# dohlee/diffab-pytorch

Measured on AMD Instinct MI355X. Metric: CDR-residue denoise-steps/sec (K=128 patch), higher is better.
Workload: dtype f32 (bf16x6 / fp16x3 split-precision products on the 16-bit matrix cores, fp32 accumulate; fp32-accurate, DESIGN section 4)

## Files before the change

diffab-pytorch_amd/csrc/api.hip:

```cpp
#include <atomic>
#include <cstring>
#include <mutex>
#include <vector>

#include "common.h"
#include "denoiser_internal.h"
#include "mlp_chain_tile.h"

namespace diffab {

static thread_local char g_err[512] = "";

void set_error(const char* fmt, ...) {
  va_list ap;
  va_start(ap, fmt);
  vsnprintf(g_err, sizeof(g_err), fmt, ap);
  va_end(ap);
}

namespace {
struct OrderState {
  std::recursive_mutex mu;
  hipStream_t last = nullptr;
  bool have = false;
// ... 20 lines not shown
  o.have = true;
}
StreamOrder::~StreamOrder() {
  if (dev_ < 0) return;
  OrderState& o = g_order[dev_ & 31];
  --o.depth;
  o.mu.unlock();
}
void set_stream_order(bool on) { g_order_on.store(on); }

struct KernelTimer {
  bool on = false;
  std::vector<hipEvent_t> ev;
  size_t used = 0;
};
static KernelTimer g_timer;

void timer_begin(hipStream_t st) {
  if (!g_timer.on) return;
  if (g_timer.used + 2 > g_timer.ev.size()) {
    for (int i = 0; i < 2; ++i) {
      hipEvent_t e;
      if (hipEventCreate(&e) != hipSuccess) return;
      g_timer.ev.push_back(e);
    }
  }
  (void)hipEventRecord(g_timer.ev[g_timer.used], st);
}
bool kernel_timer_enabled() { return g_timer.on; }
void timer_end(hipStream_t st) {
  if (!g_timer.on || g_timer.used + 2 > g_timer.ev.size()) return;
  (void)hipEventRecord(g_timer.ev[g_timer.used + 1], st);
  g_timer.used += 2;
}

static int check_dims(const diffab_dims* d, const char* who) {
  DIFFAB_REQUIRE(d != nullptr, DIFFAB_ERR_ARG, "%s: dims is null", who);
  DIFFAB_REQUIRE(d->B > 0 && d->K > 0 && d->D > 0 && d->C >= 0 && d->H > 0 && d->DS > 0 && d->PQ > 0 && d->PV > 0 && d->NL >= 0 && d->V > 0,
                 DIFFAB_ERR_ARG, "%s: non-positive dimension (B=%d K=%d D=%d C=%d H=%d DS=%d PQ=%d PV=%d NL=%d V=%d)", who, d->B, d->K, d->D,
                 d->C, d->H, d->DS, d->PQ, d->PV, d->NL, d->V);
  DIFFAB_REQUIRE(static_cast<int64_t>(d->B) * d->K < (1ll << 31), DIFFAB_ERR_UNSUPPORTED, "%s: B*K must be < 2^31", who);
  return DIFFAB_OK;
}

struct StepBuffers {
  float *cat2, *h1, *hA, *hB, *cat3, *t1, *t2, *vbuf, *logits, *ipa, *emb_tab, *beta_tab;
  char* planes;
  float* pair;
  size_t bytes;
};
static size_t mlp_planes_bytes() { return (rowgemm128_b6_scratch_bytes(128) + 255) & ~static_cast<size_t>(255); }

static StepBuffers carve_step(const diffab_dims* d, void* ws, int n_pair = 0) {
  Carver c(ws);
  const size_t rows = static_cast<size_t>(d->B) * d->K;
  StepBuffers b;
  b.cat2 = c.take<float>(rows * 2 * d->D);
  b.h1 = c.take<float>(rows * d->D);
  b.hA = c.take<float>(rows * d->D);
  b.hB = c.take<float>(rows * d->D);
  b.cat3 = c.take<float>(rows * (d->D + 3));
  b.t1 = c.take<float>(rows * d->D);
  b.t2 = c.take<float>(rows * d->D);
  b.vbuf = c.take<float>(rows * 3);
  b.logits = c.take<float>(rows * d->V);
  b.emb_tab = c.take<float>(static_cast<size_t>(25) * d->D);
  b.beta_tab = c.take<float>(static_cast<size_t>(3) * d->B * d->D);
  size_t ipa_floats = ipa_generic_workspace_floats(d);
  if (fast_path_supported(d)) ipa_floats = ipa_floats > ipa_fast_workspace_floats(d) ? ipa_floats : ipa_fast_workspace_floats(d);
  b.ipa = c.take<float>(ipa_floats);
  b.planes = fast_path_supported(d) ? c.take<char>(d->NL * ipa_layer_planes_bytes() + 11 * mlp_planes_bytes()) : nullptr;
  b.pair = pair_planes_supported(d) ? c.take<float>(pair_planes_floats(d, n_pair)) : nullptr;
  b.bytes = c.bytes();
  return b;
}

static bool ipa_layer_weights_ok(const diffab_dims* d, const diffab_ipa_layer_weights* w) {
  return w && w->gamma && w->wq_s && w->wk_s && w->wv_s && (w->w_bias || d->C == 0) && w->wq_p && w->wk_p && w->wv_p && w->w_out && w->b_out;
}

static int ipa_layer_dispatch(const diffab_dims* d, const diffab_ipa_layer_weights* w, const float* x, const float* e, const float* R,
                              const float* t, float* y, float* ws, uint32_t flags, hipStream_t st, float* sp_keep = nullptr,
                              float* d2_keep = nullptr, const void* planes = nullptr, const float* pair_planes = nullptr,
                              bool taped = false,
                              const unsigned char* tile_needed = nullptr, const int* ctx_of_row = nullptr, int n_ctx = 0) {
  DIFFAB_REQUIRE(ipa_layer_weights_ok(d, w), DIFFAB_ERR_ARG, "ipa layer: null weight pointer");
  if (!(flags & DIFFAB_FLAG_FORCE_GENERIC) && fast_path_supported(d))
    return ipa_layer_fast(d, w, x, e, R, t, y, ws, st, sp_keep, d2_keep, planes, pair_planes, (flags & DIFFAB_FLAG_FP32_GEMM) != 0,
                          taped, tile_needed, ctx_of_row, n_ctx);
  return ipa_layer_generic(d, w, x, e, R, t, y, ws, st, ctx_of_row);
}

static int check_denoiser_weights(const diffab_dims* d, const diffab_denoiser_weights* w) {
  DIFFAB_REQUIRE(w && w->seq_emb && w->res_w0 && w->res_b0 && w->res_w2 && w->res_b2 && (d->NL == 0 || w->layers), DIFFAB_ERR_ARG,
                 "denoiser: null weight pointer");
  DIFFAB_REQUIRE(d->C > 0, DIFFAB_ERR_ARG, "denoiser: C must be positive (the Denoiser's IPA layers use the pair bias, :478-492)");
  for (const diffab_mlp3_weights* h : {&w->coord, &w->orient, &w->seq})
    DIFFAB_REQUIRE(h->w0 && h->b0 && h->w2 && h->b2 && h->w4 && h->b4, DIFFAB_ERR_ARG, "denoiser head: null weight pointer");
  for (int l = 0; l < d->NL; ++l)
    DIFFAB_REQUIRE(ipa_layer_weights_ok(d, &w->layers[l]), DIFFAB_ERR_ARG, "denoiser: null weight pointer in IPA layer %d", l);
  return DIFFAB_OK;
}

static bool use_pair_planes(const diffab_dims* d, uint32_t flags, const float* pair_ctx, const StepBuffers& b) {
  const uint32_t other = DIFFAB_FLAG_FORCE_GENERIC | DIFFAB_FLAG_PAIR_F32;
  return (flags & DIFFAB_FLAG_PAIR_PLANES) && !(flags & other) && b.pair != nullptr && pair_planes_supported(d) &&
         (reinterpret_cast<uintptr_t>(pair_ctx) & 15) == 0;
}

static bool module_launch_fills_chip(const diffab_dims* d) {
  if (!ipa_module_persistent_supported(d)) return false;
  int dev = 0, ncu = 256;
  if (hipGetDevice(&dev) == hipSuccess) (void)hipDeviceGetAttribute(&ncu, hipDeviceAttributeMultiprocessorCount, dev);
  const int rounds = (d->B + ncu - 1) / ncu;
  return d->K == 128 && d->B >= ncu && static_cast<double>(d->B) >= 0.85 * rounds * ncu;
}

struct ForwardPlan {
  uint32_t flags;
  bool fold;
  bool b6;
  bool chain;
  bool persistent, fused_mlps;
  const float* pair_planes;
  const int* ctx_of_row;
  int n_ctx;
  const unsigned char* last_layer_tiles;
  float* res_emb;
};

static ForwardPlan plan_forward(const diffab_dims* d, uint32_t flags, const StepBuffers& b, const float* res_ctx, const float* pair_ctx,
                                float* res_emb, bool loop, const int* ctx_of_row = nullptr, int n_ctx = 0, unsigned char* tiles = nullptr) {
  const int rows = d->B * d->K, D = d->D;
  if (loop && !(flags & DIFFAB_FLAG_PAIR_F32)) flags |= DIFFAB_FLAG_PAIR_PLANES;
  ForwardPlan p{};
  p.flags = flags;
  p.fold = !(flags & DIFFAB_FLAG_FORCE_GENERIC) && fast_path_supported(d) && rowgemm128_ok(res_ctx, D, b.h1, D, rows, D);
  p.b6 = p.fold && use_b6_gemm(flags) && rowgemm128_b6_ok(res_ctx, D, b.h1, D, rows, D);
  p.chain = p.b6 && d->V <= 128;
  p.pair_planes = use_pair_planes(d, flags, pair_ctx, b) ? b.pair : nullptr;
  p.ctx_of_row = ctx_of_row;
  p.n_ctx = n_ctx;
  p.last_layer_tiles = (flags & DIFFAB_FLAG_SKIP_UNUSED_ROWS) && p.fold && d->K % 16 == 0 ? tiles : nullptr;
  p.res_emb = res_emb;
  p.persistent = p.b6 && p.pair_planes != nullptr && ipa_module_persistent_supported(d) && p.last_layer_tiles == nullptr &&
                 ((flags & DIFFAB_FLAG_PERSISTENT_MODULE) || (loop && !(flags & DIFFAB_FLAG_MULTI_LAUNCH) && module_launch_fills_chip(d)));
  p.fused_mlps = p.persistent && p.chain && D == 128 && res_emb == nullptr;
  return p;
}

struct StepBias {
  const float* beta;
  const float* sched_beta;
  int t;
  const int* t_dev;
  float* beta_traj;
  int traj_rows;
};

static int prepare_forward(const diffab_dims* d, const diffab_denoiser_weights* w, const ForwardPlan& p, const StepBuffers& b,
                           const float* pair_ctx, const StepBias& bias, hipStream_t st) {
  if (p.fold)
    if (int rc = launch_fold_embed_table(d, w, b.emb_tab, st)) return rc;
  if (p.b6) {
    const int D = d->D;
    for (int l = 0; l < d->NL; ++l)
      if (int rc = ipa_layer_split_weights(&w->layers[l], b.planes + l * ipa_layer_planes_bytes(), st)) return rc;
    char* mlp = b.planes + d->NL * ipa_layer_planes_bytes();
    const diffab_mlp3_weights* hw[3] = {&w->coord, &w->orient, &w->seq};
    if (int rc = launch_wsplit128(w->res_w0, 2 * D, D, mlp, st)) return rc;
    if (int rc = launch_wsplit128(w->res_w2, D, D, mlp + mlp_planes_bytes(), st)) return rc;
    for (int hd = 0; hd < 3; ++hd) {
      if (int rc = launch_wsplit128(hw[hd]->w0, D + 3, D, mlp + (2 + 2 * hd) * mlp_planes_bytes(), st)) return rc;
      if (int rc = launch_wsplit128(hw[hd]->w2, D, D, mlp + (3 + 2 * hd) * mlp_planes_bytes(), st)) return rc;
      const int nout = hd == 2 ? d->V : 3;
      if (int rc = launch_wsplit128(hw[hd]->w4, D, D, mlp + (8 + hd) * mlp_planes_bytes(), st, nout)) return rc;
    }
  }
  if (p.pair_planes)
    if (int rc = launch_pair_split(d, pair_ctx, b.pair, st, p.n_ctx)) return rc;
  if (bias.beta_traj) {
    diffab_dims dt = *d;
    dt.B = bias.traj_rows;
    if (int rc = launch_fold_beta_table(&dt, w, bias.sched_beta, bias.beta_traj, st)) return rc;
  }
  return DIFFAB_OK;
}

static int denoise_step(const diffab_dims* d, const diffab_denoiser_weights* w, const ForwardPlan& p, const StepBias& bias,
                        const int64_t* seq_t, const float* x_t, const float* O_t, const float* res_ctx, const float* pair_ctx, float* out_eps,
                        float* out_O0, float* out_post, float* out_logits, const StepBuffers& b, hipStream_t st) {
  const int rows = d->B * d->K, D = d->D;
  if (p.fold && bias.beta_traj == nullptr)
    if (int rc = launch_fold_beta_table(d, w, bias.beta, b.beta_tab, st, bias.sched_beta, bias.t, bias.t_dev)) return rc;
  const char* mlp = p.b6 ? b.planes + d->NL * ipa_layer_planes_bytes() : nullptr;
  auto dense128 = [&](int slot, const float* X, const float* W, int ldw, const float* bvec, const int64_t* bias_idx, int bias_div, float* Y,
                      bool relu) -> int {
    if (p.b6) return launch_rowgemm128_b6p(X, D, mlp + slot * mlp_planes_bytes(), bvec, bias_idx, bias_div, Y, D, rows, D, relu, st);
    return launch_rowgemm128(X, D, W, ldw, bvec, bias_idx, bias_div, Y, D, rows, D, relu, st);
  };
  float* logits = out_logits ? out_logits : b.logits;
  MlpChainSet emb_set{}, head_set{};
  if (p.chain) {
    const void* pl[3] = {mlp, mlp + mlp_planes_bytes(), nullptr};
    const float* bs[3] = {b.emb_tab, w->res_b2, nullptr};
    float* ys[1] = {b.hA};
    const int nout1[1] = {D};
    if (int rc = make_mlp_chain_set(&emb_set, 1, pl, bs, seq_t, 0, 2, nout1, ys, nout1)) return rc;
    if (!p.fused_mlps)
      if (int rc = launch_mlp_chain_b6(res_ctx, D, pl, bs, seq_t, 0, 2, D, b.hA, D, rows, st)) return rc;
  } else if (p.fold) {
    if (int rc = dense128(0, res_ctx, w->res_w0, 2 * D, b.emb_tab, seq_t, 0, b.h1, true)) return rc;
    if (int rc = dense128(1, b.h1, w->res_w2, D, w->res_b2, nullptr, 0, b.hA, false)) return rc;
  } else {
    if (int rc = launch_embed_concat(res_ctx, w->seq_emb, seq_t, D, rows, b.cat2, st)) return rc;
    if (int rc = launch_linear(b.cat2, 2 * D, w->res_w0, w->res_b0, b.h1, D, rows, D, 2 * D, true, st)) return rc;
    if (int rc = launch_linear(b.h1, D, w->res_w2, w->res_b2, b.hA, D, rows, D, D, false, st)) return rc;
  }
  float *cur = b.hA, *nxt = b.hB;
  const diffab_mlp3_weights* hw[3] = {&w->coord, &w->orient, &w->seq};
  float* outs[3] = {out_eps, b.vbuf, logits};
  const int nout[3] = {3, 3, d->V};
  const void* hpl[9];
  const float* hbs[9];
  const int head_div = bias.beta_traj ? rows : d->K;
  if (p.chain) {
    for (int hd = 0; hd < 3; ++hd) {
      hpl[3 * hd] = mlp + (2 + 2 * hd) * mlp_planes_bytes();
      hpl[3 * hd + 1] = mlp + (3 + 2 * hd) * mlp_planes_bytes();
      hpl[3 * hd + 2] = mlp + (8 + hd) * mlp_planes_bytes();
      hbs[3 * hd] = bias.beta_traj ? bias.beta_traj + (static_cast<size_t>(hd) * bias.traj_rows + bias.t) * D
                                   : b.beta_tab + static_cast<size_t>(hd) * d->B * D;
      hbs[3 * hd + 1] = hw[hd]->b2;
      hbs[3 * hd + 2] = hw[hd]->b4;
    }
    if (int rc = make_mlp_chain_set(&head_set, 3, hpl, hbs, nullptr, head_div, 3, nout, outs, nout)) return rc;
  }
  if (p.persistent) {
    if (int rc = launch_ipa_module_persistent(d, b.hA, b.hB, O_t, x_t, b.ipa, b.planes, p.pair_planes, st, p.fused_mlps ? res_ctx : nullptr,
                                              &emb_set, &head_set, p.ctx_of_row, p.n_ctx))
      return rc;
    cur = (d->NL & 1) ? b.hB : b.hA;
  }
  for (int l = 0; l < d->NL && !p.persistent; ++l) {
    const void* planes = p.b6 ? b.planes + l * ipa_layer_planes_bytes() : nullptr;
    if (int rc = ipa_layer_dispatch(d, &w->layers[l], cur, pair_ctx, O_t, x_t, nxt, b.ipa, p.flags, st, nullptr, nullptr, planes, p.pair_planes,
                                    false, l == d->NL - 1 ? p.last_layer_tiles : nullptr, p.ctx_of_row, p.n_ctx))
      return rc;
    float* tmp = cur; cur = nxt; nxt = tmp;
  }
  if (p.res_emb) DIFFAB_HIP_CHECK(hipMemcpyAsync(p.res_emb, cur, sizeof(float) * rows * D, hipMemcpyDeviceToDevice, st));
  if (p.chain) {
    if (!p.fused_mlps)
      if (int rc = launch_mlp_chains_b6(cur, D, 3, hpl, hbs, nullptr, head_div, 3, nout, outs, nout, rows, st)) return rc;
  } else if (p.fold) {
    for (int hd = 0; hd < 3; ++hd) {
      if (int rc = dense128(2 + 2 * hd, cur, hw[hd]->w0, D + 3, b.beta_tab + static_cast<size_t>(hd) * d->B * D, nullptr, d->K, b.t1, true))
        return rc;
      if (int rc = dense128(3 + 2 * hd, b.t1, hw[hd]->w2, D, hw[hd]->b2, nullptr, 0, b.t2, true)) return rc;
      if (int rc = launch_linear(b.t2, D, hw[hd]->w4, hw[hd]->b4, outs[hd], nout[hd], rows, nout[hd], D, false, st)) return rc;
    }
  } else {
    if (int rc = launch_beta_concat(cur, bias.beta, D, d->K, rows, b.cat3, st)) return rc;
    for (int hd = 0; hd < 3; ++hd) {
      if (int rc = launch_linear(b.cat3, D + 3, hw[hd]->w0, hw[hd]->b0, b.t1, D, rows, D, D + 3, true, st)) return rc;
      if (int rc = launch_linear(b.t1, D, hw[hd]->w2, hw[hd]->b2, b.t2, D, rows, D, D, true, st)) return rc;
      if (int rc = launch_linear(b.t2, D, hw[hd]->w4, hw[hd]->b4, outs[hd], nout[hd], rows, nout[hd], D, false, st)) return rc;
    }
  }
  if (out_O0 == nullptr) return DIFFAB_OK;
  return launch_heads_finish(b.vbuf, O_t, logits, d->V, rows, out_O0, out_post, st);
}

static uint32_t taped_flags(uint32_t flags) { return flags & ~(DIFFAB_FLAG_FORCE_GENERIC | DIFFAB_FLAG_PAIR_PLANES); }

static int denoise_step_taped(const diffab_dims* d, const diffab_denoiser_weights* w, const int64_t* seq_t, const float* x_t,
                              const float* O_t, const float* res_ctx, const float* pair_ctx, const float* beta, float* out_eps,
                              float* out_O0, float* out_post, const TrainTape& tp, uint32_t flags, hipStream_t st) {
  const int rows = d->B * d->K, D = d->D;
  if (int rc = launch_embed_concat(res_ctx, w->seq_emb, seq_t, D, rows, tp.cat2, st)) return rc;
  if (int rc = launch_linear(tp.cat2, 2 * D, w->res_w0, w->res_b0, tp.h1, D, rows, D, 2 * D, true, st)) return rc;
  if (int rc = launch_linear(tp.h1, D, w->res_w2, w->res_b2, tp.x[0], D, rows, D, D, false, st)) return rc;
  const bool b6 = tp.planes && use_b6_gemm(flags) && fast_path_supported(d);
  for (int l = 0; l < d->NL; ++l) {
    if (b6)
      if (int rc = ipa_layer_split_weights(&w->layers[l], tp.planes, st)) return rc;
    if (int rc = ipa_layer_dispatch(d, &w->layers[l], tp.x[l], pair_ctx, O_t, x_t, tp.x[l + 1], tp.ipa_ws[l], flags, st, tp.sp[l], tp.d2[l],
                                    b6 ? tp.planes : nullptr, nullptr, true))
      return rc;
  }
  if (int rc = launch_beta_concat(tp.x[d->NL], beta, D, d->K, rows, tp.cat3, st)) return rc;
  const diffab_mlp3_weights* hw[3] = {&w->coord, &w->orient, &w->seq};
  float* outs[3] = {out_eps, tp.vbuf, tp.logits};
  const int nout[3] = {3, 3, d->V};
  for (int hd = 0; hd < 3; ++hd) {
    if (int rc = launch_linear(tp.cat3, D + 3, hw[hd]->w0, hw[hd]->b0, tp.t1[hd], D, rows, D, D + 3, true, st)) return rc;
    if (int rc = launch_linear(tp.t1[hd], D, hw[hd]->w2, hw[hd]->b2, tp.t2[hd], D, rows, D, D, true, st)) return rc;
    if (int rc = launch_linear(tp.t2[hd], D, hw[hd]->w4, hw[hd]->b4, outs[hd], nout[hd], rows, nout[hd], D, false, st)) return rc;
  }
  return launch_heads_finish(tp.vbuf, O_t, tp.logits, d->V, rows, out_O0, out_post, st);
}

constexpr int kTrajRows = 1025;
struct SampleBuffers {
  float *beta, *eps, *O0, *post;
  int* t_dev;
  unsigned char* tiles;
  float* beta_traj;
  int* ctx_of_row;
  float* res_ctx;
  void* step;
  size_t bytes;
};

static SampleBuffers carve_sample(const diffab_dims* d, void* ws, int n_pair = 0, bool mapped = false) {
  Carver c(ws);
  const size_t rows = static_cast<size_t>(d->B) * d->K;
  SampleBuffers s;
  s.beta = c.take<float>(d->B);
  s.eps = c.take<float>(rows * 3);
  s.O0 = c.take<float>(rows * 9);
  s.post = c.take<float>(rows * d->V);
  s.t_dev = c.take<int>(64);
  s.tiles = c.take<unsigned char>(static_cast<size_t>(d->B) * ((d->K + 15) / 16));
  s.beta_traj = c.take<float>(static_cast<size_t>(3) * kTrajRows * d->D);
  s.ctx_of_row = mapped ? c.take<int>(d->B) : nullptr;
  s.res_ctx = mapped ? c.take<float>(rows * d->D) : nullptr;
  const size_t step_bytes = carve_step(d, nullptr, n_pair).bytes;
  s.step = c.take<char>(step_bytes);
  s.bytes = c.bytes();
  return s;
}

struct ScoreBuffers {
  int* t_list;
  float* beta;
  int* ctx_of_row;
  int64_t* seq_t;
  float *x_t, *O_t, *eps, *eps_hat;
  float* res_ctx;
  void* step;
  size_t bytes;
};
static ScoreBuffers carve_score(const diffab_dims* d, void* ws, int n_ctx) {
  Carver c(ws);
  const size_t rows = static_cast<size_t>(d->B) * d->K;
  ScoreBuffers s;
  s.t_list = c.take<int>(kTrajRows);
  s.beta = c.take<float>(d->B);
  s.ctx_of_row = c.take<int>(d->B);
  s.seq_t = c.take<int64_t>(rows);
  s.x_t = c.take<float>(rows * 3);
  s.O_t = c.take<float>(rows * 9);
  s.eps = c.take<float>(rows * 3);
  s.eps_hat = c.take<float>(rows * 3);
  s.res_ctx = c.take<float>(rows * d->D);
  s.step = c.take<char>(carve_step(d, nullptr, n_ctx).bytes);
  s.bytes = c.bytes();
  return s;
}

}

using namespace diffab;

extern "C" {

const char* diffab_version(void) { return "diffab_hip 0.1.0 (gfx950)"; }
const char* diffab_last_error(void) { return g_err; }

int diffab_device_ok(void) {
  int n = 0;
  if (hipGetDeviceCount(&n) != hipSuccess || n <= 0) return 0;
  hipDeviceProp_t p;
  int dev = 0;
  if (hipGetDevice(&dev) != hipSuccess || hipGetDeviceProperties(&p, dev) != hipSuccess) return 0;
  return std::strncmp(p.gcnArchName, "gfx950", 6) == 0 ? 1 : 0;
}

int diffab_debug_linear128(const float* X, const float* W, const float* bias, float* Y, int64_t M, int32_t Kd, int32_t mode, void* scratch,
                           size_t scratch_bytes, void* stream) {
  StreamOrder order_(stream);
  DIFFAB_REQUIRE(X && W && Y && M >= 1 && M < (1LL << 31) && Kd >= 32 && Kd % 32 == 0, DIFFAB_ERR_ARG, "debug_linear128: bad operands");
  hipStream_t st = as_stream(stream);
  if (mode == 0) return launch_linear(X, Kd, W, bias, Y, 128, static_cast<int>(M), 128, Kd, false, st);
  if (mode == 2) {
    const size_t pb = (rowgemm128_h3_planes_bytes(Kd) + 255) & ~static_cast<size_t>(255);
    DIFFAB_REQUIRE(Kd % 64 == 0, DIFFAB_ERR_ARG, "debug_linear128: mode 2 (fp16 x 3) needs Kd %% 64 == 0 (its chunks of 32 k are joined in pairs)");
    DIFFAB_REQUIRE(scratch && scratch_bytes >= pb + 512 && rowgemm128_b6_ok(X, Kd, Y, 128, static_cast<int>(M), Kd) &&
                       (reinterpret_cast<uintptr_t>(scratch) & 15) == 0,
                   DIFFAB_ERR_ARG, "debug_linear128: mode 2 needs 16-byte aligned operands and %zu bytes of scratch", pb + 512);
    float* wis = reinterpret_cast<float*>(static_cast<char*>(scratch) + pb);
    if (int rc = launch_wsplit128_h3(W, Kd, Kd, scratch, wis, st)) return rc;
    return launch_rowgemm128_h3p(X, Kd, scratch, wis, bias, nullptr, 0, Y, 128, static_cast<int>(M), Kd, false, st, nullptr);
  }
  DIFFAB_REQUIRE(mode == 1 && scratch && scratch_bytes >= rowgemm128_b6_scratch_bytes(Kd) && rowgemm128_b6_ok(X, Kd, Y, 128, static_cast<int>(M), Kd),
                 DIFFAB_ERR_ARG, "debug_linear128: mode 1 needs 16-byte aligned operands and %zu bytes of scratch", rowgemm128_b6_scratch_bytes(Kd));
  return launch_rowgemm128_b6(X, Kd, W, Kd, bias, nullptr, 0, Y, 128, static_cast<int>(M), Kd, false, scratch, st);
}

int diffab_debug_xstat128(const float* X, const float* W, float* Y, int64_t M, int32_t N, int32_t mode, void* scratch, size_t scratch_bytes,
                          void* stream) {
  StreamOrder order_(stream);
  DIFFAB_REQUIRE(X && W && Y && scratch && M >= 1 && M < (1LL << 31) && N >= 1 && (mode == 1 || mode == 2), DIFFAB_ERR_ARG,
                 "debug_xstat128: bad operands");
  const size_t need = mode == 1 ? xstat_b6_scratch_bytes(N) : xstat_h3_scratch_bytes(N);
  DIFFAB_REQUIRE(scratch_bytes >= need && (reinterpret_cast<uintptr_t>(scratch) & 15) == 0 && (reinterpret_cast<uintptr_t>(X) & 15) == 0,
                 DIFFAB_ERR_ARG, "debug_xstat128: needs 16-byte aligned X / scratch and %zu bytes of scratch", need);
  hipStream_t st = as_stream(stream);
  if (mode == 1) return launch_xstat_b6(X, W, 1, N, Y, N, static_cast<int>(M), N, scratch, st);
  return launch_xstat_h3(X, W, 1, N, Y, N, static_cast<int>(M), N, scratch, st);
}

int diffab_debug_gemm_tn(const float* A, const float* B, float* C, float* db, int64_t M, int32_t N1, int32_t N2, int32_t mode, void* stream) {
  StreamOrder order_(stream);
  DIFFAB_REQUIRE(A && B && C && M >= 1 && M < (1LL << 31) && N1 >= 1 && N2 >= 1 && (mode == 1 || mode == 2), DIFFAB_ERR_ARG,
                 "debug_gemm_tn: bad operands");
  hipStream_t st = as_stream(stream);
  if (mode == 1) return launch_gemm_tn_b6(A, N1, B, N2, C, N2, static_cast<int>(M), N1, N2, db, nullptr, nullptr, 0, st);
  return launch_gemm_tn_h3(A, N1, B, N2, C, N2, static_cast<int>(M), N1, N2, db, nullptr, nullptr, 0, st);
}

int diffab_set_stream_guard(int on) {
  set_stream_order(on != 0);
  return DIFFAB_OK;
}

int diffab_debug_set_module_stagger(int32_t ticks_10ns, int32_t classes) {
  set_module_stagger(ticks_10ns, classes);
  return DIFFAB_OK;
}

int diffab_debug_set_module_stamps(void* device_buffer) {
  set_module_stamps(device_buffer);
  return DIFFAB_OK;
}

int diffab_debug_set_attn_variant(int32_t v) { return set_attn_variant(v); }

int diffab_debug_set_attn_stamps(void* device_buffer) {
  set_attn_stamps(device_buffer);
  return DIFFAB_OK;
}

int diffab_kernel_timer_enable(int on) {
  g_timer.on = on != 0;
  g_timer.used = 0;
  return DIFFAB_OK;
}

int diffab_kernel_timer_read(int64_t* launches, double* total_ms) {
  DIFFAB_REQUIRE(launches && total_ms, DIFFAB_ERR_ARG, "kernel_timer_read: null pointer");
  double tot = 0.0;
  for (size_t i = 0; i + 1 < g_timer.used; i += 2) {
    DIFFAB_HIP_CHECK(hipEventSynchronize(g_timer.ev[i + 1]));
    float ms = 0.f;
    DIFFAB_HIP_CHECK(hipEventElapsedTime(&ms, g_timer.ev[i], g_timer.ev[i + 1]));
    tot += ms;
  }
  *launches = static_cast<int64_t>(g_timer.used / 2);
  *total_ms = tot;
  g_timer.used = 0;
  return DIFFAB_OK;
}

size_t diffab_denoise_workspace_bytes(const diffab_dims* d) {
  if (check_dims(d, "denoise_workspace_bytes")) return 0;
  return carve_step(d, nullptr).bytes;
}

size_t diffab_sample_workspace_bytes(const diffab_dims* d) {
  if (check_dims(d, "sample_workspace_bytes")) return 0;
  return carve_sample(d, nullptr).bytes;
}

size_t diffab_sample_shared_workspace_bytes(const diffab_dims* d, int32_t n_ctx) {
  if (check_dims(d, "sample_shared_workspace_bytes")) return 0;
  if (n_ctx < 1 || static_cast<int64_t>(n_ctx) * d->K >= (1ll << 31)) {
    set_error("sample_shared_workspace_bytes: need 1 <= n_ctx and n_ctx*K < 2^31 (n_ctx=%d)", n_ctx);
    return 0;
  }
  return carve_sample(d, nullptr, n_ctx, true).bytes;
}

int diffab_ipa_layer_fwd(const diffab_dims* d, const diffab_ipa_layer_weights* w, const float* x, const float* e, const float* R,
                         const float* t, float* y, void* workspace, size_t workspace_bytes, uint32_t flags, void* stream) {
  StreamOrder order_(stream);
  if (int rc = check_dims(d, "ipa_layer_fwd")) return rc;
  DIFFAB_REQUIRE(x && (e || d->C == 0) && R && t && y && workspace, DIFFAB_ERR_ARG, "ipa_layer_fwd: null pointer");
  const StepBuffers b = carve_step(d, workspace);
  DIFFAB_REQUIRE(workspace_bytes >= b.bytes, DIFFAB_ERR_WORKSPACE, "ipa_layer_fwd: workspace %zu < %zu bytes", workspace_bytes, b.bytes);
  const float* pair_planes = nullptr;
  if (use_pair_planes(d, flags, e, b)) {
    if (int rc = launch_pair_split(d, e, b.pair, as_stream(stream))) return rc;
    pair_planes = b.pair;
  }
  return ipa_layer_dispatch(d, w, x, e, R, t, y, b.ipa, flags, as_stream(stream), nullptr, nullptr, nullptr, pair_planes);
}

int diffab_denoise_step_fwd(const diffab_dims* d, const diffab_denoiser_weights* w, const int64_t* seq_t, const float* x_t, const float* O_t,
                            const float* res_ctx, const float* pair_ctx, const float* beta, float* out_eps, float* out_O0,
                            float* out_posterior, float* out_logits, float* out_res_emb, void* workspace, size_t workspace_bytes,
                            uint32_t flags, void* stream) {
  StreamOrder order_(stream);
  if (int rc = check_dims(d, "denoise_step_fwd")) return rc;
  if (int rc = check_denoiser_weights(d, w)) return rc;
  DIFFAB_REQUIRE(seq_t && x_t && O_t && res_ctx && pair_ctx && beta && out_eps && out_O0 && out_posterior && workspace, DIFFAB_ERR_ARG,
                 "denoise_step_fwd: null pointer");
  const StepBuffers b = carve_step(d, workspace);
  DIFFAB_REQUIRE(workspace_bytes >= b.bytes, DIFFAB_ERR_WORKSPACE, "denoise_step_fwd: workspace %zu < %zu bytes", workspace_bytes, b.bytes);
  hipStream_t st = as_stream(stream);
  const ForwardPlan p = plan_forward(d, flags, b, res_ctx, pair_ctx, out_res_emb, false);
  const StepBias bias{beta};
  if (int rc = prepare_forward(d, w, p, b, pair_ctx, bias, st)) return rc;
  return denoise_step(d, w, p, bias, seq_t, x_t, O_t, res_ctx, pair_ctx, out_eps, out_O0, out_posterior, out_logits, b, st);
}

size_t diffab_train_tape_bytes(const diffab_dims* d) {
  if (check_dims(d, "train_tape_bytes") || d->NL > kMaxLayers) return 0;
  return train_tape_floats(d) * sizeof(float);
}

size_t diffab_train_workspace_bytes(const diffab_dims* d) {
  if (check_dims(d, "train_workspace_bytes")) return 0;
  return train_bwd_workspace_floats(d) * sizeof(float);
}

int diffab_train_step_fwd(const diffab_dims* d, const diffab_denoiser_weights* w, const int64_t* seq_t, const float* x_t, const float* O_t,
                          const float* res_ctx, const float* pair_ctx, const float* beta, const float* true_post, const float* true_eps,
                          const float* true_O0, const uint8_t* gen_mask, const uint8_t* res_mask, float* out_eps, float* out_O0,
                          float* out_posterior, float* losses3, void* tape, size_t tape_bytes, uint32_t flags, void* stream) {
  StreamOrder order_(stream);
  if (int rc = check_dims(d, "train_step_fwd")) return rc;
  if (int rc = check_denoiser_weights(d, w)) return rc;
  DIFFAB_REQUIRE(d->NL <= kMaxLayers, DIFFAB_ERR_UNSUPPORTED, "train_step_fwd: at most %d IPA layers", kMaxLayers);
  DIFFAB_REQUIRE(seq_t && x_t && O_t && res_ctx && pair_ctx && beta && true_post && true_eps && true_O0 && gen_mask && res_mask && out_eps &&
                     out_O0 && out_posterior && losses3 && tape,
                 DIFFAB_ERR_ARG, "train_step_fwd: null pointer");
  DIFFAB_REQUIRE(tape_bytes >= train_tape_floats(d) * sizeof(float), DIFFAB_ERR_WORKSPACE, "train_step_fwd: tape %zu < %zu bytes", tape_bytes,
                 train_tape_floats(d) * sizeof(float));
  const TrainTape tp = carve_tape(d, static_cast<float*>(tape));
  hipStream_t st = as_stream(stream);
  flags = taped_flags(flags);
  if (int rc = denoise_step_taped(d, w, seq_t, x_t, O_t, res_ctx, pair_ctx, beta, out_eps, out_O0, out_posterior, tp, flags, st)) return rc;
  return launch_losses_fwd(out_posterior, true_post, out_eps, true_eps, out_O0, true_O0, gen_mask, res_mask, d->B, d->K, d->V, losses3, st,
                           tp.scratch);
}

int diffab_train_step_bwd(const diffab_dims* d, const diffab_denoiser_weights* w, const diffab_denoiser_weights* grads,
                          const int64_t* seq_t, const float* x_t, const float* O_t, const float* pair_ctx, const float* out_eps,
                          const float* out_O0, const float* out_posterior, const float* true_post, const float* true_eps,
                          const float* true_O0, const uint8_t* gen_mask, const uint8_t* res_mask, const float* upstream3, float* d_res_ctx,
                          float* d_pair_ctx, const void* tape, size_t tape_bytes, void* workspace, size_t workspace_bytes, void* stream) {
  StreamOrder order_(stream);
  if (int rc = check_dims(d, "train_step_bwd")) return rc;
  if (int rc = check_denoiser_weights(d, w)) return rc;
  if (int rc = check_denoiser_weights(d, grads)) return rc;
  DIFFAB_REQUIRE(d->NL <= kMaxLayers, DIFFAB_ERR_UNSUPPORTED, "train_step_bwd: at most %d IPA layers", kMaxLayers);
  DIFFAB_REQUIRE(seq_t && x_t && O_t && pair_ctx && out_eps && out_O0 && out_posterior && true_post && true_eps && true_O0 && gen_mask &&
                     res_mask && upstream3 && tape && workspace,
                 DIFFAB_ERR_ARG, "train_step_bwd: null pointer");
  DIFFAB_REQUIRE(tape_bytes >= train_tape_floats(d) * sizeof(float), DIFFAB_ERR_WORKSPACE, "train_step_bwd: tape too small");
  DIFFAB_REQUIRE(workspace_bytes >= train_bwd_workspace_floats(d) * sizeof(float), DIFFAB_ERR_WORKSPACE, "train_step_bwd: workspace %zu < %zu",
                 workspace_bytes, train_bwd_workspace_floats(d) * sizeof(float));
  const TrainTape tp = carve_tape(d, static_cast<float*>(const_cast<void*>(tape)));
  return train_step_bwd(d, w, grads, tp, seq_t, x_t, O_t, pair_ctx, out_eps, out_O0, out_posterior, true_post, true_eps, true_O0, gen_mask,
                        res_mask, upstream3, d_res_ctx, d_pair_ctx, static_cast<float*>(workspace), as_stream(stream));
}

int diffab_denoise_step_fwd_taped(const diffab_dims* d, const diffab_denoiser_weights* w, const int64_t* seq_t, const float* x_t,
                                  const float* O_t, const float* res_ctx, const float* pair_ctx, const float* beta, float* out_eps,
                                  float* out_O0, float* out_posterior, void* tape, size_t tape_bytes, uint32_t flags, void* stream) {
  StreamOrder order_(stream);
  if (int rc = check_dims(d, "denoise_step_fwd_taped")) return rc;
  if (int rc = check_denoiser_weights(d, w)) return rc;
  DIFFAB_REQUIRE(d->NL <= kMaxLayers, DIFFAB_ERR_UNSUPPORTED, "denoise_step_fwd_taped: at most %d IPA layers", kMaxLayers);
  DIFFAB_REQUIRE(seq_t && x_t && O_t && res_ctx && pair_ctx && beta && out_eps && out_O0 && out_posterior && tape, DIFFAB_ERR_ARG,
                 "denoise_step_fwd_taped: null pointer");
  DIFFAB_REQUIRE(tape_bytes >= train_tape_floats(d) * sizeof(float), DIFFAB_ERR_WORKSPACE, "denoise_step_fwd_taped: tape %zu < %zu bytes",
                 tape_bytes, train_tape_floats(d) * sizeof(float));
  const TrainTape tp = carve_tape(d, static_cast<float*>(tape));
  return denoise_step_taped(d, w, seq_t, x_t, O_t, res_ctx, pair_ctx, beta, out_eps, out_O0, out_posterior, tp, taped_flags(flags), as_stream(stream));
}

int diffab_denoise_step_bwd(const diffab_dims* d, const diffab_denoiser_weights* w, const diffab_denoiser_weights* grads,
                            const int64_t* seq_t, const float* x_t, const float* O_t, const float* pair_ctx, const float* out_posterior,
                            const float* d_eps, const float* d_O0, const float* d_posterior, float* d_res_ctx, float* d_pair_ctx,
                            float* d_x_t, float* d_O_t, const void* tape, size_t tape_bytes, void* workspace, size_t workspace_bytes,
                            void* stream) {
  StreamOrder order_(stream);
  if (int rc = check_dims(d, "denoise_step_bwd")) return rc;
  if (int rc = check_denoiser_weights(d, w)) return rc;
  if (int rc = check_denoiser_weights(d, grads)) return rc;
  DIFFAB_REQUIRE(d->NL <= kMaxLayers, DIFFAB_ERR_UNSUPPORTED, "denoise_step_bwd: at most %d IPA layers", kMaxLayers);
  DIFFAB_REQUIRE(seq_t && x_t && O_t && pair_ctx && out_posterior && d_res_ctx && tape && workspace, DIFFAB_ERR_ARG,
                 "denoise_step_bwd: null pointer");
  DIFFAB_REQUIRE(tape_bytes >= train_tape_floats(d) * sizeof(float), DIFFAB_ERR_WORKSPACE, "denoise_step_bwd: tape too small");
  DIFFAB_REQUIRE(workspace_bytes >= train_bwd_workspace_floats(d) * sizeof(float), DIFFAB_ERR_WORKSPACE, "denoise_step_bwd: workspace %zu < %zu",
                 workspace_bytes, train_bwd_workspace_floats(d) * sizeof(float));
  const TrainTape tp = carve_tape(d, static_cast<float*>(const_cast<void*>(tape)));
  return denoise_step_bwd(d, w, grads, tp, seq_t, x_t, O_t, pair_ctx, out_posterior, d_eps, d_O0, d_posterior, d_res_ctx, d_pair_ctx,
                          static_cast<float*>(workspace), as_stream(stream), d_x_t, d_O_t);
}

static diffab_dims one_layer(const diffab_dims* d) {
  diffab_dims d1 = *d;
  d1.NL = 1;
  return d1;
}
size_t diffab_ipa_layer_tape_bytes(const diffab_dims* d) {
  if (check_dims(d, "ipa_layer_tape_bytes")) return 0;
  const diffab_dims d1 = one_layer(d);
  return train_tape_floats(&d1) * sizeof(float);
}
size_t diffab_ipa_layer_bwd_workspace_bytes(const diffab_dims* d) {
  if (check_dims(d, "ipa_layer_bwd_workspace_bytes")) return 0;
  const diffab_dims d1 = one_layer(d);
  return train_bwd_workspace_floats(&d1) * sizeof(float);
}

int diffab_ipa_layer_fwd_taped(const diffab_dims* d, const diffab_ipa_layer_weights* w, const float* x, const float* e, const float* R,
                               const float* t, float* y, void* tape, size_t tape_bytes, uint32_t flags, void* stream) {
  StreamOrder order_(stream);
  if (int rc = check_dims(d, "ipa_layer_fwd_taped")) return rc;
  DIFFAB_REQUIRE(x && (e || d->C == 0) && R && t && y && tape, DIFFAB_ERR_ARG, "ipa_layer_fwd_taped: null pointer");
  const diffab_dims d1 = one_layer(d);
  DIFFAB_REQUIRE(tape_bytes >= train_tape_floats(&d1) * sizeof(float), DIFFAB_ERR_WORKSPACE, "ipa_layer_fwd_taped: tape %zu < %zu bytes", tape_bytes,
                 train_tape_floats(&d1) * sizeof(float));
  const TrainTape tp = carve_tape(&d1, static_cast<float*>(tape));
  hipStream_t st = as_stream(stream);
  const size_t nb = sizeof(float) * static_cast<size_t>(d->B) * d->K * d->D;
  DIFFAB_HIP_CHECK(hipMemcpyAsync(tp.x[0], x, nb, hipMemcpyDeviceToDevice, st));
  flags = taped_flags(flags);
  const bool b6 = tp.planes && use_b6_gemm(flags) && fast_path_supported(&d1);
  if (b6)
    if (int rc = ipa_layer_split_weights(w, tp.planes, st)) return rc;
  if (int rc = ipa_layer_dispatch(&d1, w, tp.x[0], e, R, t, tp.x[1], tp.ipa_ws[0], flags, st, tp.sp[0], tp.d2[0], b6 ? tp.planes : nullptr,
                                  nullptr, true))
    return rc;
  DIFFAB_HIP_CHECK(hipMemcpyAsync(y, tp.x[1], nb, hipMemcpyDeviceToDevice, st));
  return DIFFAB_OK;
}

int diffab_ipa_layer_bwd(const diffab_dims* d, const diffab_ipa_layer_weights* w, const diffab_ipa_layer_weights* grads, const float* e,
                         const float* R, const float* t, const float* dy, float* dx, float* d_e, float* d_R, float* d_t, const void* tape,
                         size_t tape_bytes, void* workspace, size_t workspace_bytes, void* stream) {
  StreamOrder order_(stream);
  if (int rc = check_dims(d, "ipa_layer_bwd")) return rc;
  DIFFAB_REQUIRE(w && grads && (e || d->C == 0) && R && t && dy && dx && tape && workspace, DIFFAB_ERR_ARG, "ipa_layer_bwd: null pointer");
  const diffab_dims d1 = one_layer(d);
  DIFFAB_REQUIRE(tape_bytes >= train_tape_floats(&d1) * sizeof(float), DIFFAB_ERR_WORKSPACE, "ipa_layer_bwd: tape too small");
  DIFFAB_REQUIRE(workspace_bytes >= train_bwd_workspace_floats(&d1) * sizeof(float), DIFFAB_ERR_WORKSPACE, "ipa_layer_bwd: workspace %zu < %zu",
                 workspace_bytes, train_bwd_workspace_floats(&d1) * sizeof(float));
  const TrainTape tp = carve_tape(&d1, static_cast<float*>(const_cast<void*>(tape)));
  return ipa_layer_bwd(&d1, w, grads, tp, R, t, e, dy, dx, d_e, static_cast<float*>(workspace), as_stream(stream), d_R, d_t);
}

int diffab_sample_loop(const diffab_dims* d, const diffab_denoiser_weights* w, const diffab_sched* s, const diffab_igso3* rev_tab,
                       int64_t* seq, float* x, float* O, const float* res_ctx, const float* pair_ctx, const uint8_t* gen_mask, uint64_t seed,
                       int64_t first_patch, int32_t t_start, int32_t t_stop, void* workspace, size_t workspace_bytes, uint32_t flags,
                       void* stream) {
  if (int rc = check_dims(d, "sample_loop")) return rc;
  return diffab_sample_loop_shared(d, w, s, rev_tab, seq, x, O, res_ctx, pair_ctx, d->B, nullptr, gen_mask, seed, first_patch, t_start, t_stop,
                                   workspace, workspace_bytes, flags, stream);
}

int diffab_sample_loop_shared(const diffab_dims* d, const diffab_denoiser_weights* w, const diffab_sched* s, const diffab_igso3* rev_tab,
                              int64_t* seq, float* x, float* O, const float* res_ctx, const float* pair_ctx, int32_t n_ctx,
                              const int32_t* ctx_of_row, const uint8_t* gen_mask, uint64_t seed, int64_t first_patch, int32_t t_start,
                              int32_t t_stop, void* workspace, size_t workspace_bytes, uint32_t flags, void* stream) {
  return diffab_sample_loop_aa(d, w, s, rev_tab, seq, x, O, res_ctx, pair_ctx, n_ctx, ctx_of_row, gen_mask, seed, first_patch, t_start, t_stop,
                               workspace, workspace_bytes, flags, nullptr, stream);
}

int diffab_sample_loop_aa(const diffab_dims* d, const diffab_denoiser_weights* w, const diffab_sched* s, const diffab_igso3* rev_tab,
                          int64_t* seq, float* x, float* O, const float* res_ctx, const float* pair_ctx, int32_t n_ctx, const int32_t* ctx_of_row,
                          const uint8_t* gen_mask, uint64_t seed, int64_t first_patch, int32_t t_start, int32_t t_stop, void* workspace,
                          size_t workspace_bytes, uint32_t flags, const uint32_t* allowed, void* stream) {
  return diffab_sample_loop_rec(d, w, s, rev_tab, seq, x, O, res_ctx, pair_ctx, n_ctx, ctx_of_row, gen_mask, seed, first_patch, t_start, t_stop,
                                workspace, workspace_bytes, flags, allowed, nullptr, stream);
}

int diffab_sample_loop_rec(const diffab_dims* d, const diffab_denoiser_weights* w, const diffab_sched* s, const diffab_igso3* rev_tab,
                           int64_t* seq, float* x, float* O, const float* res_ctx, const float* pair_ctx, int32_t n_ctx,
                           const int32_t* ctx_of_row, const uint8_t* gen_mask, uint64_t seed, int64_t first_patch, int32_t t_start,
                           int32_t t_stop, void* workspace, size_t workspace_bytes, uint32_t flags, const uint32_t* allowed,
                           const diffab_sample_record* rec, void* stream) {
  StreamOrder order_(stream);
  if (int rc = check_dims(d, "sample_loop")) return rc;
  if (int rc = check_denoiser_weights(d, w)) return rc;
  DIFFAB_REQUIRE(s && s->T > 0 && s->alpha && s->beta && s->one_minus_alpha_bar_sqrt, DIFFAB_ERR_ARG, "sample_loop: bad schedule");
  DIFFAB_REQUIRE(rev_tab && rev_tab->sigmas && rev_tab->cdf && rev_tab->n_sigmas >= s->T + 1 && rev_tab->n_bins > 0, DIFFAB_ERR_ARG,
                 "sample_loop: reverse IGSO3 table must have T+1 rows");
  DIFFAB_REQUIRE(seq && x && O && res_ctx && pair_ctx && gen_mask && workspace, DIFFAB_ERR_ARG, "sample_loop: null pointer");
  DIFFAB_REQUIRE(t_start <= s->T && t_stop >= 0 && t_stop <= t_start, DIFFAB_ERR_ARG, "sample_loop: need T >= t_start >= t_stop >= 0");
  const uint32_t keep = flags & (DIFFAB_FLAG_KEEP_STRUCTURE | DIFFAB_FLAG_KEEP_SEQUENCE);
  DIFFAB_REQUIRE(keep != (DIFFAB_FLAG_KEEP_STRUCTURE | DIFFAB_FLAG_KEEP_SEQUENCE), DIFFAB_ERR_ARG,
                 "sample_loop: DIFFAB_FLAG_KEEP_STRUCTURE and DIFFAB_FLAG_KEEP_SEQUENCE together leave nothing to sample");
  flags &= ~keep;
  DIFFAB_REQUIRE(!(allowed && (keep & DIFFAB_FLAG_KEEP_SEQUENCE)), DIFFAB_ERR_ARG,
                 "sample_loop: allowed classes constrain a sequence that DIFFAB_FLAG_KEEP_SEQUENCE does not sample");
  DIFFAB_REQUIRE(!allowed || d->V <= 32, DIFFAB_ERR_ARG, "sample_loop: allowed classes are one 32-bit word per residue; V = %d > 32", d->V);
  SampleRecordDev rdev;
  if (rec != nullptr) {
    DIFFAB_REQUIRE(rec->n_slots >= 1, DIFFAB_ERR_ARG, "sample_loop: record n_slots = %d < 1", rec->n_slots);
    DIFFAB_REQUIRE(rec->slot_of_step && rec->slot_dev && rec->seq && rec->x && rec->O, DIFFAB_ERR_ARG,
                   "sample_loop: record needs slot_of_step, slot_dev, seq, x and O");
    const int n_pred = (rec->pred_x != nullptr) + (rec->pred_O != nullptr) + (rec->seq_probs != nullptr);
    DIFFAB_REQUIRE(n_pred == 0 || n_pred == 3, DIFFAB_ERR_ARG, "sample_loop: record predictions are pred_x, pred_O and seq_probs, all or none");
    DIFFAB_REQUIRE(n_pred == 0 || s->alpha_bar_sqrt, DIFFAB_ERR_ARG, "sample_loop: record predictions need the schedule's alpha_bar_sqrt");
    std::vector<int> used(rec->n_slots, 0);
    for (int t = 0; t <= s->T; ++t) {
      const int j = rec->slot_of_step[t];
      if (j == -1) continue;
      DIFFAB_REQUIRE(j >= 0 && j < rec->n_slots, DIFFAB_ERR_ARG, "sample_loop: record slot_of_step[%d] = %d outside -1, [0, %d)", t, j,
                     rec->n_slots);
      DIFFAB_REQUIRE(t > t_stop && t <= t_start, DIFFAB_ERR_ARG,
                     "sample_loop: record slot_of_step[%d] = %d, but the call runs steps [%d, %d] only (the slot would never be written)", t, j,
                     t_stop + 1, t_start);
      DIFFAB_REQUIRE(used[j]++ == 0, DIFFAB_ERR_ARG, "sample_loop: record slot %d is given to two steps", j);
    }
// ... 162 lines not shown
```

diffab-pytorch_amd/csrc/denoiser_fast.hip:

```cpp
#include <cstdlib>
#include <type_traits>

#include "common.h"
#include "denoiser_internal.h"
#include "rowgemm_b6_tile.h"
#include "ipa_attn_tile.h"

namespace diffab {


constexpr int LBM = 128, LBK = 32, LLD = LBK + 4;

struct LinearSegs {
  const float* W[6];
  int n_end[6];
  int nseg;
};

template <int BN, bool RELU, bool VEC>
__global__ __launch_bounds__(256) void linear_mfma_kernel(const float* __restrict__ X, int ldx, LinearSegs segs,
                                                          const float* __restrict__ bias, float* __restrict__ Y, int ldy, int M, int N,
                                                          int Kd) {
  __shared__ __attribute__((aligned(16))) float As[LBM * LLD];
  __shared__ __attribute__((aligned(16))) float Bs[BN * LLD];
// ... 197 lines not shown
  };

  load_w(0);
  load_a(aA, 0);
  store_w(0);
  __syncthreads();
  for (int ch = 0; ch < nchunk; ch += 2 * AW) {
    load_a(aB, ch / AW + 1);
#pragma unroll
    for (int p = 0; p < AW; ++p) {
      load_w(ch + p + 1);
      MEM_FENCE();
      compute(aA, p, p & 1);
      store_w((p + 1) & 1);
      __syncthreads();
    }
    load_a(aA, ch / AW + 2);
#pragma unroll
    for (int p = 0; p < AW; ++p) {
      load_w(ch + AW + p + 1);
      MEM_FENCE();
      compute(aB, p, (AW + p) & 1);
      store_w((AW + p + 1) & 1);
      __syncthreads();
    }
  }
  const int col = 64 * cw + 4 * l15;
  const bool table = bias_idx != nullptr || bias_div > 0;
  f32x4 bv = {0.f, 0.f, 0.f, 0.f};
  if (bias && !table) bv = *reinterpret_cast<const f32x4*>(bias + col);
#pragma unroll
  for (int mt = 0; mt < MT; ++mt)
#pragma unroll
    for (int r = 0; r < 4; ++r) {
      const int row = m0 + 16 * MT * rw + 16 * mt + 4 * g + r;
      if (row >= M) continue;
      if (table) {
        const int64_t bi = bias_idx ? bias_idx[row] : row / bias_div;
        bv = *reinterpret_cast<const f32x4*>(bias + bi * 128 + col);
      }
      f32x4 o = {acc[mt][0][r] + bv[0], acc[mt][1][r] + bv[1], acc[mt][2][r] + bv[2], acc[mt][3][r] + bv[3]};
      if (RELU) { o[0] = fmaxf(o[0], 0.f); o[1] = fmaxf(o[1], 0.f); o[2] = fmaxf(o[2], 0.f); o[3] = fmaxf(o[3], 0.f); }
      *reinterpret_cast<f32x4*>(Y + static_cast<int64_t>(row) * ldy + col) = o;
    }
}

bool rowgemm128_ok(const float* X, int ldx, const float* Y, int ldy, int M, int Kd) {
  return Kd % (2 * RG_KC) == 0 && ldx % 4 == 0 && ldy % 4 == 0 && aligned16(X) && aligned16(Y) && M >= RG_ROWS;
}
int launch_rowgemm128(const float* X, int ldx, const float* W, int ldw, const float* bias, const int64_t* bias_idx, int bias_div, float* Y,
                      int ldy, int M, int Kd, bool relu, hipStream_t st) {
  DIFFAB_REQUIRE(rowgemm128_ok(X, ldx, Y, ldy, M, Kd) && (!bias || aligned16(bias)), DIFFAB_ERR_ARG, "rowgemm128: unsupported operands");
  const dim3 grid((M + RG_ROWS - 1) / RG_ROWS);
#define RG_LAUNCH(R, AW_) \
  hipLaunchKernelGGL((rowgemm128_kernel<R, AW_>), grid, dim3(512), 0, st, X, ldx, W, ldw, bias, bias_idx, bias_div, Y, ldy, M, Kd)
  if (RG_DEEP_A && Kd % (4 * RG_KC) == 0) { if (relu) RG_LAUNCH(true, 2); else RG_LAUNCH(false, 2); }
  else                                    { if (relu) RG_LAUNCH(true, 1); else RG_LAUNCH(false, 1); }
#undef RG_LAUNCH
  DIFFAB_LAUNCH_CHECK();
  return DIFFAB_OK;
}

int launch_linear(const float* X, int ldx, const float* W, const float* bias, float* Y, int ldy, int M, int N, int Kd, bool relu,
                  hipStream_t st) {
  LinearSegs segs{};
  segs.W[0] = W;
  segs.n_end[0] = N;
  segs.nseg = 1;
  const bool vec = (ldx % 4 == 0) && (Kd % 4 == 0) && aligned16(X) && aligned16(W);
  if (N == 128 && vec && rowgemm128_ok(X, ldx, Y, ldy, M, Kd) && (!bias || aligned16(bias)))
    return launch_rowgemm128(X, ldx, W, Kd, bias, nullptr, 0, Y, ldy, M, Kd, relu, st);
  if (N > 64) return launch_linear_bn<128>(X, ldx, segs, bias, Y, ldy, M, N, Kd, relu, vec, st);
  return launch_linear_bn<64>(X, ldx, segs, bias, Y, ldy, M, N, Kd, relu, vec, st);
}

template <int NT, bool MULTI, bool PLANES = false, bool TAPE = false>
__global__ __launch_bounds__(512) void ipa_attn_fast_kernel(const float* __restrict__ proj, const float* __restrict__ e,
                                                            const float* __restrict__ R, const float* __restrict__ t,
                                                            const float* __restrict__ Wb, const float* __restrict__ gamma,
                                                            float* __restrict__ feat, int B, int NC_arg,
                                                            unsigned long long* __restrict__ stamps, const float* __restrict__ esc = nullptr,
                                                            float* __restrict__ tape_p = nullptr, float* __restrict__ tape_d2 = nullptr,
                                                            const unsigned char* __restrict__ tile_needed = nullptr,
                                                            const int* __restrict__ ctx_of_row = nullptr) {
  extern __shared__ __attribute__((aligned(16))) float S[];
  const int ntile = (MULTI ? NC_arg : 1) * NT;
  int b, tile;
  const unsigned bid = blockIdx.x;
  if ((B & 7) == 0) {
    const int xcd = bid & 7, slot = bid >> 3;
    b = (slot / ntile) * 8 + xcd;
    tile = slot % ntile;
  } else {
    b = bid / ntile;
    tile = bid % ntile;
  }
  if (tile_needed != nullptr && !tile_needed[b * ntile + tile]) return;
  ipa_attn_tile<NT, MULTI, PLANES, TAPE>(S, b, tile, bid, proj, e, R, t, Wb, gamma, feat, NC_arg, stamps, esc, tape_p, tape_d2, ctx_of_row);
}

static unsigned long long* g_attn_stamps = nullptr;
static bool g_pair_chain_off = false;
void set_pair_embed_fused(bool on);
int set_attn_variant(int v) {
  DIFFAB_REQUIRE((v & ~(4 | 64)) == 0, DIFFAB_ERR_ARG, "debug_set_attn_variant: %d has bits other than 4 and 64", v);
  set_pair_embed_fused(!(v & 4));
  g_pair_chain_off = (v & 64) != 0;
  return DIFFAB_OK;
}
bool pair_chain_bwd_enabled() { return !g_pair_chain_off; }
void set_attn_stamps(void* p) {
  g_attn_stamps = static_cast<unsigned long long*>(p);
}

__global__ void points_to_global_fast_kernel(float* __restrict__ proj, const float* __restrict__ R, const float* __restrict__ t, int rows) {
  const int gid = blockIdx.x * blockDim.x + threadIdx.x;
  if (gid >= rows * 192) return;
  const int r = gid / 192, p = gid % 192;
  float* qv = proj + static_cast<int64_t>(r) * ANP + OFF_GQ + p * 3;
  const float* Rr = R + static_cast<int64_t>(r) * 9;
  const float x = qv[0], y = qv[1], z = qv[2];
  qv[0] = (x * Rr[0] + y * Rr[3] + z * Rr[6]) + t[r * 3 + 0];
  qv[1] = (x * Rr[1] + y * Rr[4] + z * Rr[7]) + t[r * 3 + 1];
  qv[2] = (x * Rr[2] + y * Rr[5] + z * Rr[8]) + t[r * 3 + 2];
}

__global__ __launch_bounds__(64) void fold_embed_table_kernel(const float* __restrict__ emb, const float* __restrict__ W0,
                                                              const float* __restrict__ b0, int D, int n_types, float* __restrict__ tab) {
  const int s_ = blockIdx.x, n0 = blockIdx.y * 8, lane = threadIdx.x;
  if (s_ >= n_types) return;
  float acc[8];
#pragma unroll
  for (int i = 0; i < 8; ++i) {
    acc[i] = 0.f;
    const int n = n0 + i;
    if (n < D)
      for (int k = lane; k < D; k += 64) acc[i] += emb[s_ * D + k] * W0[n * 2 * D + D + k];
  }
#pragma unroll
  for (int i = 0; i < 8; ++i) {
    for (int o = 32; o > 0; o >>= 1) acc[i] += __shfl_xor(acc[i], o);
    if (lane == 0 && n0 + i < D) tab[s_ * D + n0 + i] = acc[i] + b0[n0 + i];
  }
}
__global__ void fold_beta_table_kernel(const float* __restrict__ beta, const float* __restrict__ Wa, const float* __restrict__ ba,
                                       const float* __restrict__ Wb_, const float* __restrict__ bb, const float* __restrict__ Wc,
                                       const float* __restrict__ bc, int D, int B, float* __restrict__ tab,
                                       const float* __restrict__ sched_beta, int t, const int* __restrict__ t_dev) {
  const int b = blockIdx.x, hd = blockIdx.y, n = threadIdx.x;
  if (b >= B || n >= D) return;
  const float* W = hd == 0 ? Wa : (hd == 1 ? Wb_ : Wc);
  const float* bias = hd == 0 ? ba : (hd == 1 ? bb : bc);
  const float be = sched_beta ? sched_beta[t_dev ? *t_dev : t] : beta[b];
  const float* wr = W + n * (D + 3) + D;
  tab[(static_cast<int64_t>(hd) * B + b) * D + n] = ((be * wr[0] + sinf(be) * wr[1]) + cosf(be) * wr[2]) + bias[n];
}
int launch_fold_embed_table(const diffab_dims* d, const diffab_denoiser_weights* w, float* emb_tab, hipStream_t st) {
  hipLaunchKernelGGL(fold_embed_table_kernel, dim3(25, (d->D + 7) / 8), dim3(64), 0, st, w->seq_emb, w->res_w0, w->res_b0, d->D, 25, emb_tab);
  DIFFAB_LAUNCH_CHECK();
  return DIFFAB_OK;
}
int launch_fold_beta_table(const diffab_dims* d, const diffab_denoiser_weights* w, const float* beta, float* beta_tab, hipStream_t st,
                           const float* sched_beta, int t, const int* t_dev) {
  hipLaunchKernelGGL(fold_beta_table_kernel, dim3(d->B, 3), dim3(d->D), 0, st, beta, w->coord.w0, w->coord.b0, w->orient.w0, w->orient.b0,
                     w->seq.w0, w->seq.b0, d->D, d->B, beta_tab, sched_beta, t, t_dev);
  DIFFAB_LAUNCH_CHECK();
  return DIFFAB_OK;
}

bool fast_path_supported(const diffab_dims* d) {
  return d->D == 128 && d->C == AC && d->H == AH && d->DS == ADS && d->PQ == AP && d->PV == AP && d->K % 64 == 0 && d->K >= 64 &&
         d->K <= 1024;
}

__global__ __launch_bounds__(256) void pair_rowscale_kernel(const float* __restrict__ e, int row_f4, float* __restrict__ rs) {
  const int64_t row = blockIdx.x;
  const f32x4* p = reinterpret_cast<const f32x4*>(e) + row * row_f4;
  float m = 0.f;
  for (int i = threadIdx.x; i < row_f4; i += 256) {
    const f32x4 v = p[i];
    m = fmaxf(fmaxf(m, fmaxf(fabsf(v[0]), fabsf(v[1]))), fmaxf(fabsf(v[2]), fabsf(v[3])));
  }
#pragma unroll
  for (int o = 1; o < 64; o <<= 1) m = fmaxf(m, __shfl_xor(m, o));
  __shared__ float wm[4];
  if ((threadIdx.x & 63) == 0) wm[threadIdx.x >> 6] = m;
  __syncthreads();
  if (threadIdx.x == 0) {
    const unsigned b = __float_as_uint(fmaxf(fmaxf(wm[0], wm[1]), fmaxf(wm[2], wm[3])));
    const int ex = static_cast<int>((b >> 23) & 255u);
    const bool ok = ex >= 8 && ex < 231 && b < 0x7f800000u;
    rs[2 * row] = ok ? __uint_as_float(static_cast<unsigned>(127 + 7 + 127 - ex) << 23) : 1.0f;
    rs[2 * row + 1] = ok ? __uint_as_float(static_cast<unsigned>(ex - 7) << 23) : 1.0f;
  }
}
__global__ void pair_split_kernel(const float* __restrict__ e, const float* __restrict__ rs, int K, int64_t n_groups,
                                  _Float16* __restrict__ out) {
  const int64_t gid = blockIdx.x * static_cast<int64_t>(blockDim.x) + threadIdx.x;
  if (gid >= n_groups) return;
  const int cg = static_cast<int>(gid & 7);
  const int64_t rj = gid >> 3;
  const int j = static_cast<int>(rj % K);
  const int64_t row = rj / K;
  const float s = rs[2 * row];
  const f32x4 v0 = reinterpret_cast<const f32x4*>(e)[gid * 2], v1 = reinterpret_cast<const f32x4*>(e)[gid * 2 + 1];
  f16x8 h1, h2;
#pragma unroll
  for (int c = 0; c < 8; ++c) {
    const float x = (c < 4 ? v0[c & 3] : v1[c & 3]) * s;
    const _Float16 a = static_cast<_Float16>(x);
    h1[c] = a;
    h2[c] = static_cast<_Float16>(x - static_cast<float>(a));
  }
  const int jt = j >> 4, l15 = j & 15, ks = cg >> 2, g = cg & 3;
  _Float16* base = out + (row * K) * 128 + static_cast<int64_t>(jt) * 2048 + ks * 512 + (l15 + 16 * g) * 8;
  *reinterpret_cast<f16x8*>(base) = h1;
  *reinterpret_cast<f16x8*>(base + 1024) = h2;
}
bool pair_planes_supported(const diffab_dims* d) { return fast_path_supported(d); }
static size_t pair_patches(const diffab_dims* d, int n_pair) { return static_cast<size_t>(n_pair > 0 ? n_pair : d->B); }
size_t pair_planes_floats(const diffab_dims* d, int n_pair) {
  const size_t np = pair_patches(d, n_pair);
  return pair_planes_supported(d) ? np * d->K * d->K * AC + 64 + 2 * np * d->K + 64 : 0;
}
const float* pair_row_scales(const diffab_dims* d, const float* planes, int n_pair) {
  return planes + 64 + pair_patches(d, n_pair) * d->K * d->K * AC;
}
int launch_pair_split(const diffab_dims* d, const float* e, float* planes, hipStream_t st, int n_pair) {
  DIFFAB_REQUIRE(pair_planes_supported(d) && e && planes && (reinterpret_cast<uintptr_t>(planes) & 15) == 0 &&
                     (reinterpret_cast<uintptr_t>(e) & 15) == 0,
                 DIFFAB_ERR_ARG, "pair_split: unsupported operands");
  const int64_t np = static_cast<int64_t>(pair_patches(d, n_pair));
  const int64_t n = np * d->K * d->K * AC;
  float* rs = const_cast<float*>(pair_row_scales(d, planes, n_pair));
  hipLaunchKernelGGL(pair_rowscale_kernel, dim3(static_cast<unsigned>(np * d->K)), dim3(256), 0, st, e, d->K * AC / 4, rs);
  hipLaunchKernelGGL(pair_split_kernel, dim3(static_cast<unsigned>((n / 8 + 255) / 256)), dim3(256), 0, st, e, rs, d->K, n / 8,
                     reinterpret_cast<_Float16*>(planes + 64));
  DIFFAB_LAUNCH_CHECK();
  return DIFFAB_OK;
}


bool use_b6_gemm(uint32_t flags) { return !(flags & DIFFAB_FLAG_FP32_GEMM); }
static size_t round256(size_t b) { return (b + 255) & ~static_cast<size_t>(255); }
constexpr size_t kLayerSmallFloats = AH * AC + 64 + 128;
size_t ipa_layer_small_offset() { return 0; }
size_t ipa_layer_h3_pj_offset() { return ipa_layer_small_offset() + round256(kLayerSmallFloats * sizeof(float)); }
size_t ipa_layer_h3_out_offset() { return ipa_layer_h3_pj_offset() + round256(proj_frames_h3_planes_bytes()); }
size_t ipa_layer_h3_wis_offset() { return ipa_layer_h3_out_offset() + round256(rowgemm128_h3_planes_bytes(AF)); }
size_t ipa_layer_planes_bytes() { return ipa_layer_h3_wis_offset() + round256((ANP + 128) * sizeof(float)); }
__global__ void layer_small_copy_kernel(const float* __restrict__ w_bias, const float* __restrict__ gamma, const float* __restrict__ b_out,
                                        float* __restrict__ out) {
  const int i = blockIdx.x * blockDim.x + threadIdx.x;
  if (i < AH * AC) out[i] = w_bias[i];
  else if (i < AH * AC + 64) out[i] = i - AH * AC < AH ? gamma[i - AH * AC] : 0.0f;
  else if (i < static_cast<int>(kLayerSmallFloats)) out[i] = b_out[i - AH * AC - 64];
}
int ipa_layer_split_weights(const diffab_ipa_layer_weights* w, void* planes, hipStream_t st) {
  DIFFAB_REQUIRE(w && w->wq_s && w->wk_s && w->wv_s && w->wq_p && w->wk_p && w->wv_p && w->w_out, DIFFAB_ERR_ARG, "ipa layer: null weight pointer");
  const float* W6[6] = {w->wq_s, w->wk_s, w->wv_s, w->wq_p, w->wk_p, w->wv_p};
  if (w->w_bias && w->gamma && w->b_out) {
    hipLaunchKernelGGL(layer_small_copy_kernel, dim3((kLayerSmallFloats + 255) / 256), dim3(256), 0, st, w->w_bias, w->gamma, w->b_out,
                       reinterpret_cast<float*>(static_cast<char*>(planes) + ipa_layer_small_offset()));
    DIFFAB_LAUNCH_CHECK();
  }
  char* pl = static_cast<char*>(planes);
  float* wis = reinterpret_cast<float*>(pl + ipa_layer_h3_wis_offset());
  if (int rc = launch_pjsplit_h3(W6, pl + ipa_layer_h3_pj_offset(), wis, st)) return rc;
  return launch_wsplit128_h3(w->w_out, AF, AF, pl + ipa_layer_h3_out_offset(), wis + ANP, st);
}
static size_t b6_scratch_floats() { return (ipa_layer_planes_bytes() + 256) / sizeof(float); }

static size_t ipa_ws_parts_offset(const diffab_dims* d) {
  const size_t rows = static_cast<size_t>(d->B) * d->K;
  const size_t o = rows * (ANP + AF) + 128 + (attention_split_supported(d) ? attention_split_workspace_floats(d) : 0) + b6_scratch_floats();
  return (o + 63) & ~static_cast<size_t>(63);
}
size_t ipa_fast_workspace_floats(const diffab_dims* d) { return ipa_ws_parts_offset(d) + rowgemm128_h3_parts_floats(d->B * d->K, AF) + 64; }

int ipa_layer_fast(const diffab_dims* d, const diffab_ipa_layer_weights* w, const float* x, const float* e, const float* R, const float* t,
                   float* y, float* ws, hipStream_t st, float* sp_keep, float* d2_keep, const void* planes, const float* pair_planes,
                   bool fp32_gemm, bool taped, const unsigned char* tile_needed, const int* ctx_of_row, int n_ctx) {
  const int rows = d->B * d->K, D = d->D;
  DIFFAB_REQUIRE(ctx_of_row == nullptr || sp_keep == nullptr, DIFFAB_ERR_ARG, "ipa_layer_fast: shared contexts are an inference form");
  float* proj = ws;
  float* feat = ws + static_cast<size_t>(rows) * ANP;
  const bool h3 = use_b6_gemm(fp32_gemm ? DIFFAB_FLAG_FP32_GEMM : 0u) && (planes != nullptr || sp_keep == nullptr);
  if (h3 && planes == nullptr) {
    float* tail = ws + static_cast<size_t>(rows) * (ANP + AF) + 128 + (attention_split_supported(d) ? attention_split_workspace_floats(d) : 0);
    void* own = reinterpret_cast<void*>((reinterpret_cast<uintptr_t>(tail) + 255) & ~static_cast<uintptr_t>(255));
    if (int rc = ipa_layer_split_weights(w, own, st)) return rc;
    planes = own;
  }
  const char* plc = static_cast<const char*>(planes);
  const float* wis = h3 ? reinterpret_cast<const float*>(plc + ipa_layer_h3_wis_offset()) : nullptr;
  auto to_out = [&]() -> int {
    if (h3 && rowgemm128_b6_ok(feat, AF, y, D, rows, AF))
      return launch_rowgemm128_h3p(feat, AF, plc + ipa_layer_h3_out_offset(), wis + ANP, w->b_out, nullptr, 0, y, D, rows, AF, false, st,
                                   taped ? nullptr : ws + ipa_ws_parts_offset(d));
    return launch_linear(feat, AF, w->w_out, w->b_out, y, D, rows, D, AF, false, st);
  };
  LinearSegs segs{};
  segs.W[0] = w->wq_s; segs.W[1] = w->wk_s; segs.W[2] = w->wv_s; segs.W[3] = w->wq_p; segs.W[4] = w->wk_p; segs.W[5] = w->wv_p;
  segs.n_end[0] = 256; segs.n_end[1] = 512; segs.n_end[2] = 768; segs.n_end[3] = 960; segs.n_end[4] = 1152; segs.n_end[5] = 1344;
  segs.nseg = 6;
  bool vec = aligned16(x);
  for (int s = 0; s < 6; ++s) vec = vec && aligned16(segs.W[s]);
  DIFFAB_REQUIRE(vec, DIFFAB_ERR_ARG, "ipa_layer_fast: x and the projection weights must be 16-byte aligned");
  if (h3) {
    if (int rc = launch_proj_frames_h3p(x, plc + ipa_layer_h3_pj_offset(), wis, R, t, proj, rows, st)) return rc;
  } else {
    if (int rc = launch_proj_frames_f32(x, segs.W, R, t, proj, rows, st)) return rc;
  }
  if (sp_keep != nullptr && attention_split_supported(d) && !(d->K == 128 && d2_keep != nullptr)) {
    if (int rc = launch_attention_split(d, proj, e, R, t, w->w_bias, w->gamma, feat, sp_keep, st, d2_keep)) return rc;
    return to_out();
  }
  const bool tape = sp_keep != nullptr && attention_split_supported(d);
  const int nt = (d->K % 128 == 0) ? 8 : 4;
  const int nc = d->K / (16 * nt);
  const size_t lds = ipa_attn_lds_bytes(nt);
  const dim3 grid(d->B * (d->K / TI));
  const bool use_planes = pair_planes != nullptr && pair_planes_supported(d);
  const float* e_arg = use_planes ? pair_planes + 64 : e;
  const float* esc = use_planes ? pair_row_scales(d, pair_planes, n_ctx) : nullptr;
#define ATTN_LAUNCH(NT_, MULTI_, PLANES_)                                                                                             \
  do {                                                                                                                                \
    DIFFAB_HIP_CHECK(hipFuncSetAttribute(reinterpret_cast<const void*>(ipa_attn_fast_kernel<NT_, MULTI_, PLANES_>),                   \
                                         hipFuncAttributeMaxDynamicSharedMemorySize, static_cast<int>(lds)));                         \
    timer_begin(st);                                                                                                                  \
    hipLaunchKernelGGL((ipa_attn_fast_kernel<NT_, MULTI_, PLANES_>), grid, dim3(512), lds, st, proj, e_arg, R, t, w->w_bias, w->gamma, \
                       feat, d->B, nc, g_attn_stamps, esc, nullptr, nullptr, tile_needed, ctx_of_row);                                \
    timer_end(st);                                                                                                                    \
  } while (0)
  if (tape) {
    DIFFAB_HIP_CHECK(hipFuncSetAttribute(reinterpret_cast<const void*>(ipa_attn_fast_kernel<8, false, false, true>),
                                         hipFuncAttributeMaxDynamicSharedMemorySize, static_cast<int>(lds)));
    hipLaunchKernelGGL((ipa_attn_fast_kernel<8, false, false, true>), grid, dim3(512), lds, st, proj, e, R, t, w->w_bias, w->gamma, feat,
                       d->B, nc, nullptr, nullptr, sp_keep, d2_keep);
  } else if (use_planes) {
    if (nt == 8 && nc == 1) ATTN_LAUNCH(8, false, true);
    else if (nt == 8) ATTN_LAUNCH(8, true, true);
    else if (nc == 1) ATTN_LAUNCH(4, false, true);
    else ATTN_LAUNCH(4, true, true);
  } else if (nt == 8 && nc == 1) ATTN_LAUNCH(8, false, false);
  else if (nt == 8) ATTN_LAUNCH(8, true, false);
  else if (nc == 1) ATTN_LAUNCH(4, false, false);
  else ATTN_LAUNCH(4, true, false);
#undef ATTN_LAUNCH
  DIFFAB_LAUNCH_CHECK();
  return to_out();
}

}
```

diffab-pytorch_amd/csrc/denoiser_internal.h:

```cpp
#pragma once
#include "common.h"

namespace diffab {

int launch_linear_generic(const float* X, int ldx, const float* W, const float* bias, float* Y, int ldy, int M, int N, int Kd, bool relu,
                          hipStream_t st);
size_t ipa_generic_workspace_floats(const diffab_dims* d);
int ipa_layer_generic(const diffab_dims* d, const diffab_ipa_layer_weights* w, const float* x, const float* e, const float* R, const float* t,
                      float* y, float* ws, hipStream_t st, const int* ctx_of_row = nullptr);
int launch_embed_concat(const float* res_ctx, const float* emb, const int64_t* seq, int D, int64_t rows, float* out, hipStream_t st);
int launch_beta_concat(const float* h, const float* beta, int D, int K, int64_t rows, float* out, hipStream_t st);
int launch_heads_finish(const float* v, const float* O_t, const float* logits, int V, int64_t rows, float* O0, float* post, hipStream_t st);
int launch_proj_frames_f32(const float* x, const float* const* W6, const float* R, const float* t, float* proj, int rows, hipStream_t st);
int launch_losses_bwd(const float* post, const float* tpost, const float* eps, const float* teps, const float* O0, const float* tO,
                      const float* O_t, const float* v, const uint8_t* gm, const uint8_t* rm, const float* count, const float* up, int V,
                      int64_t rows, float* d_logits, float* d_eps, float* d_v, hipStream_t st);
int launch_heads_cotangent(const float* post, const float* c_post, const float* c_eps, const float* c_O0, const float* O_t, const float* v,
                           int V, int64_t rows, float* d_logits, float* d_eps, float* d_v, float* d_Ot, hipStream_t st);
int launch_ipa_frames_bwd(const float* proj, const float* dproj, int NP, int pt_col0, int n_pts, const float* feat, const float* dfeat, int F,
                          int ol_col0, int on_col0, int n_vpts, const float* R, const float* t, float* dR, float* dt, int rows,
                          hipStream_t st);

bool fast_path_supported(const diffab_dims* d);
size_t ipa_fast_workspace_floats(const diffab_dims* d);
int ipa_layer_fast(const diffab_dims* d, const diffab_ipa_layer_weights* w, const float* x, const float* e, const float* R, const float* t,
                   float* y, float* ws, hipStream_t st,
                   float* sp_keep = nullptr, float* d2_keep = nullptr,
                   const void* planes = nullptr,
                   const float* pair_planes = nullptr,
                   bool fp32_gemm = false,
                   bool taped = false,
                   const unsigned char* tile_needed = nullptr,
                   const int* ctx_of_row = nullptr, int n_ctx = 0);
bool pair_planes_supported(const diffab_dims* d);
size_t pair_planes_floats(const diffab_dims* d, int n_pair = 0);
int launch_pair_split(const diffab_dims* d, const float* e, float* planes, hipStream_t st, int n_pair = 0);
const float* pair_row_scales(const diffab_dims* d, const float* planes, int n_pair = 0);
int launch_linear(const float* X, int ldx, const float* W, const float* bias, float* Y, int ldy, int M, int N, int Kd, bool relu,
                  hipStream_t st);

bool rowgemm128_ok(const float* X, int ldx, const float* Y, int ldy, int M, int Kd);
int launch_rowgemm128(const float* X, int ldx, const float* W, int ldw, const float* bias, const int64_t* bias_idx, int bias_div, float* Y,
                      int ldy, int M, int Kd, bool relu, hipStream_t st);
size_t rowgemm128_b6_scratch_bytes(int Kd);
bool rowgemm128_b6_ok(const float* X, int ldx, const float* Y, int ldy, int M, int Kd);
int launch_wsplit128(const float* W, int ldw, int Kd, void* planes, hipStream_t st, int nrows = 128);
int launch_mlp_chains_b6(const float* X, int ldx, int nchains, const void* const* planes, const float* const* bias, const int64_t* bias_idx0,
                         int bias_div0, int nlayers, const int* n_out, float* const* Y, const int* ldy, int M, hipStream_t st);
struct MlpChainSet;
int make_mlp_chain_set(MlpChainSet* out, int nchains, const void* const* planes, const float* const* bias, const int64_t* bias_idx0,
                       int bias_div0, int nlayers, const int* n_out, float* const* Y, const int* ldy);
int launch_mlp_chain_b6(const float* X, int ldx, const void* const* planes, const float* const* bias, const int64_t* bias_idx0, int bias_div0,
                        int nlayers, int n_out, float* Y, int ldy, int M, hipStream_t st);
int launch_wsplit128_strided(const float* W, int64_t sn, int64_t sk, int kseg, int k0, void* planes, hipStream_t st);
int launch_wsplit128_segs(const float* const* W, const int* k_end, int nseg, void* planes, hipStream_t st);
int launch_rowgemm128_b6p(const float* X, int ldx, const void* planes, const float* bias, const int64_t* bias_idx, int bias_div, float* Y,
                          int ldy, int M, int Kd, bool relu, hipStream_t st, float* parts = nullptr);
size_t rowgemm128_b6_parts_floats(int M, int Kd);
size_t rowgemm128_h3_parts_floats(int M, int Kd);
int launch_rowgemm128_b6(const float* X, int ldx, const float* W, int ldw, const float* bias, const int64_t* bias_idx, int bias_div, float* Y,
                         int ldy, int M, int Kd, bool relu, void* scratch, hipStream_t st);
bool use_b6_gemm(uint32_t flags = 0);
size_t xstat_b6_scratch_bytes(int N);
int launch_gemm_tn_h3(const float* A, int lda, const float* B, int ldb, float* C, int ldc, int M, int N1, int N2, float* db,
                      float* const* seg_ptrs, const int* seg_ends, int nseg, hipStream_t st);
size_t xstat_h3_scratch_bytes(int N);
int launch_xstat_h3(const float* X, const float* W, int64_t sn, int64_t sk, float* Y, int ldy, int rows, int N, void* scratch, hipStream_t st);
int launch_xstat_b6(const float* X, const float* W, int64_t sn, int64_t sk, float* Y, int ldy, int rows, int N, void* scratch, hipStream_t st);
bool gemm_tn_b6_ok(const float* A, int lda, const float* B, int ldb, int M, int N1, int N2);
int launch_gemm_tn_b6(const float* A, int lda, const float* B, int ldb, float* C, int ldc, int M, int N1, int N2, float* db,
                      float* const* seg_ptrs, const int* seg_ends, int nseg, hipStream_t st);
size_t ipa_layer_planes_bytes();
size_t ipa_layer_small_offset();
size_t ipa_layer_h3_pj_offset();
size_t ipa_layer_h3_out_offset();
size_t ipa_layer_h3_wis_offset();
size_t rowgemm128_h3_planes_bytes(int Kd);
size_t proj_frames_h3_planes_bytes();
int launch_wsplit128_h3(const float* W, int ldw, int Kd, void* planes, float* wis, hipStream_t st, int nrows = 128);
int launch_pjsplit_h3(const float* const* W6, void* planes, float* wis, hipStream_t st);
int launch_rowgemm128_h3p(const float* X, int ldx, const void* planes, const float* wis, const float* bias, const int64_t* bias_idx, int bias_div,
                          float* Y, int ldy, int M, int Kd, bool relu, hipStream_t st, float* parts = nullptr);
int launch_proj_frames_h3p(const float* x, const void* planes, const float* wis, const float* R, const float* t, float* proj, int rows,
                           hipStream_t st);
int ipa_layer_split_weights(const diffab_ipa_layer_weights* w, void* planes, hipStream_t st);
bool ipa_module_persistent_supported(const diffab_dims* d);
int launch_ipa_module_persistent(const diffab_dims* d, float* xa, float* xb, const float* R, const float* t, float* ws, const void* planes,
                                 const float* pair_planes, hipStream_t st, const float* emb_X = nullptr, const MlpChainSet* emb = nullptr,
                                 const MlpChainSet* heads = nullptr, const int* ctx_of_row = nullptr, int n_ctx = 0);
void set_module_stagger(int ticks, int classes);
void set_module_stamps(void* device_buffer);
int launch_fold_embed_table(const diffab_dims* d, const diffab_denoiser_weights* w, float* emb_tab, hipStream_t st);
int launch_fold_beta_table(const diffab_dims* d, const diffab_denoiser_weights* w, const float* beta, float* beta_tab, hipStream_t st,
                           const float* sched_beta = nullptr, int t = 0, const int* t_dev = nullptr);

bool pair_embed_fused_supported(const diffab_ctx_dims* d);
size_t pair_embed_fused_prep_floats(const diffab_ctx_dims* d);
int launch_pair_embed_fused(const diffab_ctx_dims* d, const diffab_pair_emb_weights* w, const int64_t* seq_idx, const float* distmat,
                            const float* xyz, const float* pairwise_dihedrals, const int64_t* residue_idx, int32_t residue_idx_batch_stride,
                            const int64_t* chain_idx, const float* atom_mask, const uint8_t* sequence_context_mask, float* out, float* prep,
                            float* tape_h1, float* tape_df, float* tape_m1, float* tape_m2, int64_t row0, int64_t nrows, hipStream_t st,
                            const float** coef_sp_out = nullptr);
int launch_softplus_table(const float* coefw, int n, float* out, hipStream_t st);

bool attention_split_supported(const diffab_dims* d);
size_t attention_split_workspace_floats(const diffab_dims* d);
int launch_ipa_logits(const diffab_dims* d, const float* proj, const float* gamma, float* SP, hipStream_t st);
int launch_attention_probs(const diffab_dims* d, const float* proj, const float* e, const float* Wb, const float* gamma, float* P,
                           float* D2, hipStream_t st);
constexpr int kDeLayersMax = 6;
int launch_pair_de_layers(const diffab_dims* d, int nl, const float* const* P, const float* const* G, const float* const* doe,
                          const float* const* Wb, float* de, hipStream_t st);
int launch_pair_stream_bwd(const diffab_dims* d, const float* e, const float* P, float* G , const float* D2,
                           const float* dfeat, float* wb_part, const float* Wb, float* de ,
                           hipStream_t st);
int launch_attention_split(const diffab_dims* d, const float* proj, const float* e, const float* R, const float* t, const float* Wb,
                           const float* gamma, float* feat, float* SP, hipStream_t st, float* D2 = nullptr);

void set_stream_order(bool on);
int set_attn_variant(int v);
// ... 107 lines not shown
```

diffab-pytorch_amd/csrc/ipa_attn_tile.h:

```cpp
#pragma once
#include <hip/hip_runtime.h>
#include <cmath>
#include <cstdint>

namespace diffab {

typedef float f32x4 __attribute__((ext_vector_type(4)));
typedef float f32x16 __attribute__((ext_vector_type(16)));
typedef float f32x2 __attribute__((ext_vector_type(2)));

#ifndef MEM_FENCE
#define MEM_FENCE() asm volatile("" ::: "memory")
#endif

constexpr int AH = 8, ADS = 32, AP = 8, AC = 64;
constexpr int ANP = 3 * AH * ADS + 3 * AH * AP * 3;
constexpr int AF = AH * ADS + AH * AC + AH * AP * 3 + AH * AP;
constexpr int OFF_QS = 0, OFF_KS = 256, OFF_VS = 512, OFF_GQ = 768, OFF_GK = 960, OFF_GV = 1152;
constexpr int FOFF_OS = 0, FOFF_OE = 256, FOFF_OL = 768, FOFF_ON = 960;
constexpr int TI = 16;


#define FAST_EXP(x) __expf(x)

typedef _Float16 f16x8 __attribute__((ext_vector_type(8)));
typedef short s16x4_t __attribute__((ext_vector_type(4)));
typedef short s16x8_t __attribute__((ext_vector_type(8)));
template <int SD>
struct AttnP1Pre {
  f32x4 st[SD][4];
  f32x4 qa[2];
  f32x4 gqr[2];
};
struct AttnLaneOff { int s, p0, p1; };
__device__ __forceinline__ AttnLaneOff attn_lane_off(const int lane) {
  const int g0 = lane, g1 = lane + 64 < 96 ? lane + 64 : 95;
  return AttnLaneOff{(lane >> 3) * ANP + 4 * (lane & 7), (g0 / 6) * ANP + 4 * (g0 % 6), (g1 / 6) * ANP + 4 * (g1 % 6)};
}
__device__ __forceinline__ void attn_tile_request(f32x4 (&dst)[4], const float* __restrict__ proj, const int64_t row0, const int off_s,
                                                  const int off_p, const AttnLaneOff lo, const int h) {
  const float* us = proj + row0 * ANP + (off_s + h * ADS);
  const float* up = proj + row0 * ANP + (off_p + h * 24);
  dst[0] = *reinterpret_cast<const f32x4*>(us + lo.s);
  dst[1] = *reinterpret_cast<const f32x4*>(us + 8 * ANP + lo.s);
  dst[2] = *reinterpret_cast<const f32x4*>(up + lo.p0);
  dst[3] = *reinterpret_cast<const f32x4*>(up + lo.p1);
}
template <int SD>
__device__ __forceinline__ void attn_p1_request(AttnP1Pre<SD>& pre, const int piece, const float* __restrict__ proj, const int64_t prow0,
                                                const int64_t krow0, const int i0, const int lane, const AttnLaneOff lo, const int h) {
  if (piece < SD) {
    attn_tile_request(pre.st[piece], proj, krow0 + 16 * piece, OFF_KS, OFF_GK, lo, h);
    return;
  }
  const int l15 = lane & 15, q = lane >> 4;
  const float* uq = proj + (prow0 + i0) * ANP + h * ADS;
  pre.qa[0] = *reinterpret_cast<const f32x4*>(uq + OFF_QS + l15 * ANP + 4 * q);
  pre.qa[1] = *reinterpret_cast<const f32x4*>(uq + OFF_QS + 16 + l15 * ANP + 4 * q);
  const float* ug = proj + (prow0 + i0) * ANP + (OFF_GQ + h * 24);
  pre.gqr[0] = *reinterpret_cast<const f32x4*>(ug + lo.p0);
  pre.gqr[1] = *reinterpret_cast<const f32x4*>(ug + lo.p1);
}

template <bool PLANES, typename FP>
__device__ __forceinline__ void attn_shift_pair_rows(FP& e, FP& esc, const int* __restrict__ ctx_of_row, const int b, const int K) {
  if (ctx_of_row == nullptr) return;
  int c;
  asm volatile("s_load_dword %0, %1, 0x0\n\ts_waitcnt lgkmcnt(0)" : "=s"(c) : "s"(ctx_of_row + b) : "memory");
  const int64_t shift = static_cast<int64_t>(c - b) * K;
  e += shift * K * AC;
  if constexpr (PLANES) esc += 2 * shift;
}

template <int NT, bool MULTI, bool PLANES = false, bool TAPE = false>
__device__ __forceinline__ void ipa_attn_tile(float* __restrict__ S, const int b, const int tile, const unsigned stamp_id,
                                              const float* __restrict__ proj, const float* __restrict__ e,
                                              const float* __restrict__ R, const float* __restrict__ t,
                                              const float* __restrict__ Wb, const float* __restrict__ gamma,
                                              float* __restrict__ feat, int NC_arg,
                                              unsigned long long* __restrict__ stamps, const float* __restrict__ esc = nullptr,
                                              float* __restrict__ tape_p = nullptr, float* __restrict__ tape_d2 = nullptr,
                                              const int* __restrict__ ctx_of_row = nullptr) {
  static_assert(!PLANES || NT % 2 == 0, "the o_e product takes key tiles in pairs");
  static_assert(!TAPE || (!MULTI && !PLANES), "the tape form is the single-chunk fp32-pair kernel");
  const int NC = MULTI ? NC_arg : 1;
  constexpr int KC = NT * 16;
  const int K = NC * KC;
  auto stamp = [&](int k) {
    if (stamps != nullptr) {
      __builtin_amdgcn_sched_barrier(0);
#ifdef AT_STAMP_REALTIME
      const unsigned long long tnow = __builtin_amdgcn_s_memrealtime();
#else
      const unsigned long long tnow = __builtin_amdgcn_s_memtime();
#endif
      if ((threadIdx.x & 63) == 0) stamps[(static_cast<size_t>(stamp_id) * 8 + (threadIdx.x >> 6)) * 8 + k] = tnow;
      __builtin_amdgcn_sched_barrier(0);
    }
  };
  stamp(0);
  const int i0 = tile * TI;
  const int tid = threadIdx.x, lane0 = tid & 63, wv = __builtin_amdgcn_readfirstlane(tid >> 6);
  constexpr int HS = KC + 8, IS = AH * (KC + 8) + 8;
  const int64_t prow0 = static_cast<int64_t>(b) * K;
  attn_shift_pair_rows<PLANES>(e, esc, ctx_of_row, b, K);
  const float scale_t = 0.57735026918962576f;

  constexpr int KLD = 40, GLD = 28;
  constexpr int P1_TILE = 16 * KLD + 16 * GLD;
  constexpr int ELD = 72;
  constexpr int SCR_FLOATS = 2 * 16 * ELD;
  constexpr int E_LAG = MULTI ? 2 : 0;
  constexpr int E_EARLY = MULTI ? 1 : 2;
  float* scr = S + TI * IS + wv * SCR_FLOATS;
  float* st_fac = S + TI * IS + 8 * SCR_FLOATS;
  float* st_inv = st_fac + TI * AH;
  float* wb_lds = st_inv + TI * AH;
  float* gq_lds = wb_lds + (PLANES ? 0 : 4 * 64 * 4) + wv * (TI * 24);
  if (wv == 0 && !PLANES) {
    const int l15_ = lane0 & 15, q_ = lane0 >> 4;
#pragma unroll
    for (int sg = 0; sg < 4; ++sg) {
      f32x4 v = *reinterpret_cast<const f32x4*>(Wb + (l15_ & 7) * AC + 16 * sg + 4 * q_);
#pragma unroll
      for (int s_ = 0; s_ < 4; ++s_) v[s_] = l15_ < 8 ? v[s_] : 0.0f;
      *reinterpret_cast<f32x4*>(wb_lds + (sg * 64 + lane0) * 4) = v;
    }
  }

  const float* erow[2];
  float Mrun[2], Lrun[2];
#pragma unroll
  for (int ii = 0; ii < 2; ++ii) {
    erow[ii] = e + ((prow0 + i0 + 2 * wv + ii) * K) * AC;
    Mrun[ii] = -INFINITY;
    Lrun[ii] = 0.f;
  }
  float inv_s2[2];
#pragma unroll
  for (int ii = 0; ii < 2; ++ii) inv_s2[ii] = 1.0f;
  if constexpr (PLANES) {
    const float* ep = esc + 2 * (prow0 + i0 + 2 * __builtin_amdgcn_readfirstlane(static_cast<int>(threadIdx.x >> 6)));
#pragma unroll
    for (int ii = 0; ii < 2; ++ii) inv_s2[ii] = ep[2 * ii + 1];
  }

#pragma unroll 1
  for (int c = 0; c < NC; ++c) {
    const bool last = c == NC - 1;
    const int64_t krow0 = prow0 + c * KC;
    int lane = lane0;
    asm volatile("" : "+v"(lane));
    const int l15 = lane & 15, q = lane >> 4;
    f32x4 ev[2][NT][4];
    f32x4 wv4[2][2];
    auto load_e_tile = [&](int ii, int cc_, int jt) {
      if constexpr (PLANES) {
        const f32x4* ep = reinterpret_cast<const f32x4*>(erow[ii]) + (cc_ * NT + jt) * 256 + lane;
#pragma unroll
        for (int r = 0; r < 4; ++r) ev[ii][jt][r] = __builtin_nontemporal_load(ep + r * 64);
      } else {
        const f32x4* ep = reinterpret_cast<const f32x4*>(erow[ii] + (cc_ * KC + jt * 16 + 4 * q) * AC + 4 * l15);
#pragma unroll
        for (int r = 0; r < 4; ++r) ev[ii][jt][r] = __builtin_nontemporal_load(ep + r * (AC / 4));
      }
    };
    {
      const int h = wv;
      const float scale_s = 0.17677669529663687f;
      const float coef_p = -0.5f * 0.16666666666666666f * gamma[h];
      const int ks_dst = (lane >> 3) * KLD + 4 * (lane & 7);
      const int g0 = lane, g1 = lane + 64;
      const int gk_dst0 = 16 * KLD + (g0 / 6) * GLD + 4 * (g0 % 6), gk_dst1 = 16 * KLD + (g1 / 6) * GLD + 4 * (g1 % 6);
      constexpr int SD = MULTI ? 3 : 4;
      static_assert(E_EARLY <= SD, "the early pair tiles are requested in the last E_EARLY iterations, which must not request key tiles any more");
      AttnP1Pre<SD> pre;
      f32x4 (&st)[SD][4] = pre.st;
      const AttnLaneOff lo = attn_lane_off(lane);
      auto load_keys = [&](int sb, int jt) { attn_tile_request(st[sb], proj, krow0 + 16 * jt, OFF_KS, OFF_GK, lo, h); };
      auto stage_keys = [&](int sb, int lb) {
        float* t_ = scr + lb * P1_TILE;
        *reinterpret_cast<f32x4*>(t_ + ks_dst) = st[sb][0];
        *reinterpret_cast<f32x4*>(t_ + ks_dst + 8 * KLD) = st[sb][1];
        *reinterpret_cast<f32x4*>(t_ + gk_dst0) = st[sb][2];
        if (g1 < 96) *reinterpret_cast<f32x4*>(t_ + gk_dst1) = st[sb][3];
      };
      attn_p1_request<SD>(pre, SD, proj, prow0, krow0, i0, lane, lo, h);
#pragma unroll
      for (int piece = 0; piece < SD && piece < NT; ++piece) attn_p1_request<SD>(pre, piece, proj, prow0, krow0, i0, lane, lo, h);
      f32x4 (&qa)[2] = pre.qa;
      MEM_FENCE();
      *reinterpret_cast<f32x4*>(gq_lds + 4 * g0) = pre.gqr[0];
      if (g1 < 96) *reinterpret_cast<f32x4*>(gq_lds + 4 * g1) = pre.gqr[1];
      f32x4 gq[4][6];
#pragma unroll
      for (int r = 0; r < 4; ++r)
#pragma unroll
        for (int cc = 0; cc < 6; ++cc) gq[r][cc] = *reinterpret_cast<const f32x4*>(gq_lds + (4 * q + r) * 24 + 4 * cc);
      struct KeyFrag { f32x4 kb0, kb1, gk[6]; };
      auto read_frags = [&](int jt) {
        KeyFrag f;
        const float* t_ = scr + (jt & 1) * P1_TILE;
        f.kb0 = *reinterpret_cast<const f32x4*>(t_ + l15 * KLD + 4 * q);
        f.kb1 = *reinterpret_cast<const f32x4*>(t_ + l15 * KLD + 16 + 4 * q);
#pragma unroll
        for (int cc = 0; cc < 6; ++cc) f.gk[cc] = *reinterpret_cast<const f32x4*>(t_ + 16 * KLD + l15 * GLD + 4 * cc);
        return f;
      };
      stage_keys(0, 0);
      KeyFrag cur = read_frags(0);
      if (NT > 1) stage_keys(1 % SD, 1);
#pragma unroll
      for (int jt = 0; jt < NT; ++jt) {
        if (jt + 2 < NT) stage_keys((jt + 2) % SD, jt & 1);
        KeyFrag nxt = cur;
        if (jt + 1 < NT) nxt = read_frags(jt + 1);
        if (jt + SD < NT) {
          load_keys(jt % SD, jt + SD);
        } else if (jt + E_EARLY >= NT) {
          if constexpr (PLANES) {
            if (jt + E_EARLY == NT) {
              const int hh = lane & 7, qq = lane >> 4;
#pragma unroll
              for (int ks = 0; ks < 2; ++ks)
#pragma unroll
                for (int hf = 0; hf < 2; ++hf) wv4[ks][hf] = *reinterpret_cast<const f32x4*>(Wb + hh * AC + 32 * ks + 8 * qq + 4 * hf);
            }
          }
          load_e_tile(0, c, jt + E_EARLY - NT);
        }
        MEM_FENCE();
        const f32x4 kb0 = cur.kb0, kb1 = cur.kb1;
        f32x4 gk[6];
#pragma unroll
        for (int cc = 0; cc < 6; ++cc) gk[cc] = cur.gk[cc];
        cur = nxt;
        f32x4 acc = {0.f, 0.f, 0.f, 0.f};
#pragma unroll
        for (int s = 0; s < 4; ++s) acc = __builtin_amdgcn_mfma_f32_16x16x4f32(qa[0][s], kb0[s], acc, 0, 0, 0);
#pragma unroll
        for (int s = 0; s < 4; ++s) acc = __builtin_amdgcn_mfma_f32_16x16x4f32(qa[1][s], kb1[s], acc, 0, 0, 0);
#pragma unroll
        for (int r = 0; r < 4; ++r) {
          f32x2 d2v = {0.f, 0.f};
#pragma unroll
          for (int cc = 0; cc < 6; ++cc) {
            f32x2 dlo, dhi;
            asm("v_pk_add_f32 %0, %1, %2 neg_lo:[0,1] neg_hi:[0,1]"
                : "=v"(dlo)
                : "v"(__builtin_shufflevector(gq[r][cc], gq[r][cc], 0, 1)), "v"(__builtin_shufflevector(gk[cc], gk[cc], 0, 1)));
            asm("v_pk_add_f32 %0, %1, %2 neg_lo:[0,1] neg_hi:[0,1]"
                : "=v"(dhi)
                : "v"(__builtin_shufflevector(gq[r][cc], gq[r][cc], 2, 3)), "v"(__builtin_shufflevector(gk[cc], gk[cc], 2, 3)));
            d2v = __builtin_elementwise_fma(dlo, dlo, d2v);
            d2v = __builtin_elementwise_fma(dhi, dhi, d2v);
          }
          const float d2 = d2v[0] + d2v[1];
          S[(4 * q + r) * IS + h * HS + jt * 16 + l15] = scale_t * (acc[r] * scale_s + coef_p * d2);
          if constexpr (TAPE) tape_d2[((static_cast<int64_t>(b) * AH + h) * K + i0 + 4 * q + r) * K + jt * 16 + l15] = d2;
        }
        if (c == 0 && jt == 0) stamp(6);
        if (c == 0 && jt == 3) stamp(7);
      }
    }
    if (c == 0) stamp(1);
    {
      const int h = l15 & 7;
      constexpr int E_DEPTH_FP32 = 3;
      constexpr int RT = NT / 2;
      constexpr int E_DEPTH0 = PLANES ? RT : (E_DEPTH_FP32 < NT ? (E_DEPTH_FP32 > E_EARLY ? E_DEPTH_FP32 : E_EARLY) : NT);
      if constexpr (!PLANES) {
#pragma unroll
        for (int jt = E_EARLY; jt < E_DEPTH0; ++jt) load_e_tile(0, c, jt);
      }
      f32x4 wb[4];
      f16x8 wp[2][2];
      float bscale = scale_t, oscale = 1.0f;
      if constexpr (PLANES) {
        float wmax = 0.f;
#pragma unroll
        for (int ks = 0; ks < 2; ++ks)
#pragma unroll
          for (int hf = 0; hf < 2; ++hf)
#pragma unroll
            for (int s = 0; s < 4; ++s) wmax = fmaxf(wmax, fabsf(wv4[ks][hf][s]));
#pragma unroll
        for (int o = 1; o < 64; o <<= 1) wmax = fmaxf(wmax, __shfl_xor(wmax, o));
        const int ew = static_cast<int>((__float_as_uint(wmax) >> 23) & 255u);
        const float sw = (ew == 0 || ew > 230) ? 1.0f : __uint_as_float(static_cast<unsigned>(127 + 7 + 127 - ew) << 23);
        const float isw = (ew == 0 || ew > 230) ? 1.0f : __uint_as_float(static_cast<unsigned>(ew - 7) << 23);
#pragma unroll
        for (int ks = 0; ks < 2; ++ks)
#pragma unroll
          for (int c8 = 0; c8 < 8; ++c8) {
            const float x = l15 < 8 ? wv4[ks][c8 >> 2][c8 & 3] * sw : 0.0f;
            const _Float16 h1 = static_cast<_Float16>(x);
            wp[0][ks][c8] = h1;
            wp[1][ks][c8] = static_cast<_Float16>(x - static_cast<float>(h1));
          }
        bscale = scale_t * isw;
        oscale = 1.0f / 256.0f;
        asm volatile("" ::"v"(wp[0][0]), "v"(wp[1][0]), "v"(wp[0][1]), "v"(wp[1][1]));
#pragma unroll
        for (int jt = E_EARLY; jt < E_DEPTH0; ++jt) load_e_tile(0, c, jt);
      } else if constexpr (!MULTI) {
#pragma unroll
        for (int sg = 0; sg < 4; ++sg) {
          wb[sg] = *reinterpret_cast<const f32x4*>(Wb + h * AC + 16 * sg + 4 * q);
#pragma unroll
          for (int s = 0; s < 4; ++s) wb[sg][s] = l15 < 8 ? wb[sg][s] : 0.0f;
        }
      }
      MEM_FENCE();
      __syncthreads();
      if (c == 0) stamp(2);
      auto stage_e = [&](int ii, int jt) {
        float* t_ = scr + (jt & 1) * (16 * ELD) + 4 * q * ELD + 4 * l15;
#pragma unroll
        for (int r = 0; r < 4; ++r) *reinterpret_cast<f32x4*>(t_ + r * ELD) = ev[ii][jt][r];
      };

      if constexpr (PLANES) {
        char* trt = reinterpret_cast<char*>(scr);
        const int wr_off = l15 * 128 + 8 * ((2 * q) ^ (4 * ((l15 >> 1) & 3)) ^ (2 * (l15 & 1)));
        const int rrow = 4 * q + (l15 >> 2);
        const int rd_off = rrow * 128 + 8 * ((l15 & 3) ^ (4 * ((rrow >> 1) & 3)) ^ (2 * (rrow & 1)));
#pragma unroll
        for (int ii = 0; ii < 2; ++ii) {
          const int il = 2 * wv + ii;
          float* Srow = S + il * IS + h * HS;
          const float inv_s = inv_s2[ii];
          const float bscale_r = bscale * inv_s, oscale_r = oscale * inv_s;
          float m_run = -INFINITY, l_run = 0.f, m_hist[NT / 2];
          f32x4 oe[4];
#pragma unroll
          for (int ct = 0; ct < 4; ++ct) oe[ct] = f32x4{0.f, 0.f, 0.f, 0.f};
#pragma unroll
          for (int T = 0; T < NT / 2; ++T) {
            f32x4 acc[2][2];
#pragma unroll
            for (int tl = 0; tl < 2; ++tl)
#pragma unroll
              for (int ks = 0; ks < 2; ++ks) {
                const f16x8 a1 = __builtin_bit_cast(f16x8, ev[ii][2 * T + tl][ks]), a2 = __builtin_bit_cast(f16x8, ev[ii][2 * T + tl][2 + ks]);
                f32x4 a_ = {0.f, 0.f, 0.f, 0.f};
                a_ = __builtin_amdgcn_mfma_f32_16x16x32_f16(a2, wp[0][ks], a_, 0, 0, 0);
                a_ = __builtin_amdgcn_mfma_f32_16x16x32_f16(a1, wp[1][ks], a_, 0, 0, 0);
                a_ = __builtin_amdgcn_mfma_f32_16x16x32_f16(a1, wp[0][ks], a_, 0, 0, 0);
                acc[tl][ks] = a_;
              }
            float v[8], smax = -INFINITY;
#pragma unroll
            for (int tl = 0; tl < 2; ++tl) {
              const f32x4 sv = *reinterpret_cast<const f32x4*>(Srow + (2 * T + tl) * 16 + 4 * q);
#pragma unroll
              for (int r = 0; r < 4; ++r) {
                v[4 * tl + r] = sv[r] + bscale_r * (acc[tl][0][r] + acc[tl][1][r]);
                smax = fmaxf(smax, v[4 * tl + r]);
              }
            }
            smax = fmaxf(smax, __shfl_xor(smax, 16));
            smax = fmaxf(smax, __shfl_xor(smax, 32));
            const float m_new = fmaxf(m_run, smax);
            const float alpha = T == 0 ? 0.0f : FAST_EXP(m_run - m_new);
            m_run = m_new;
            m_hist[T] = m_new;
            float psum = 0.f;
#pragma unroll
            for (int tt = 0; tt < 8; ++tt) {
              v[tt] = FAST_EXP(v[tt] - m_new);
              psum += v[tt];
            }
            l_run = l_run * alpha + psum;
            if (T > 0) {
#pragma unroll
              for (int ct = 0; ct < 4; ++ct)
#pragma unroll
                for (int r = 0; r < 4; ++r) oe[ct][r] *= alpha;
            }
            f16x8 p1, p2;
#pragma unroll
            for (int tt = 0; tt < 8; ++tt) {
              const float x = 256.0f * v[tt];
              const _Float16 hh = static_cast<_Float16>(x);
              p1[tt] = hh;
              p2[tt] = static_cast<_Float16>(x - static_cast<float>(hh));
            }
#pragma unroll
            for (int tl = 0; tl < 2; ++tl) {
              if (l15 < 8) *reinterpret_cast<f32x4*>(Srow + (2 * T + tl) * 16 + 4 * q) = f32x4{v[4 * tl], v[4 * tl + 1], v[4 * tl + 2], v[4 * tl + 3]};
#pragma unroll
              for (int pl = 0; pl < 2; ++pl)
#pragma unroll
                for (int ks = 0; ks < 2; ++ks)
                  *reinterpret_cast<f32x4*>(trt + (tl * 2 + pl) * 2048 + (wr_off ^ (64 * ks))) = ev[ii][2 * T + tl][2 * pl + ks];
            }
            {
              constexpr int dummy_ = 0;
              (void)dummy_;
              const int nx = ii * NT + 2 * T + RT;
              if (nx < 2 * NT) {
                load_e_tile(nx / NT, c, nx % NT);
                load_e_tile((nx + 1) / NT, c, (nx + 1) % NT);
                MEM_FENCE();
              }
            }
            f16x8 a[2][4];
#pragma unroll
            for (int pl = 0; pl < 2; ++pl)
#pragma unroll
              for (int ct = 0; ct < 4; ++ct) {
                const int ro = rd_off ^ (32 * ct);
                const s16x4_t lo = __builtin_amdgcn_ds_read_tr16_b64_v4i16((s16x4_t __attribute__((address_space(3)))*)(trt + (0 * 2 + pl) * 2048 + ro));
                const s16x4_t hi = __builtin_amdgcn_ds_read_tr16_b64_v4i16((s16x4_t __attribute__((address_space(3)))*)(trt + (1 * 2 + pl) * 2048 + ro));
                const s16x8_t v8 = {lo[0], lo[1], lo[2], lo[3], hi[0], hi[1], hi[2], hi[3]};
                a[pl][ct] = __builtin_bit_cast(f16x8, v8);
              }
#pragma unroll
            for (int ct = 0; ct < 4; ++ct) oe[ct] = __builtin_amdgcn_mfma_f32_16x16x32_f16(a[1][ct], p1, oe[ct], 0, 0, 0);
#pragma unroll
            for (int ct = 0; ct < 4; ++ct) oe[ct] = __builtin_amdgcn_mfma_f32_16x16x32_f16(a[0][ct], p2, oe[ct], 0, 0, 0);
#pragma unroll
            for (int ct = 0; ct < 4; ++ct) oe[ct] = __builtin_amdgcn_mfma_f32_16x16x32_f16(a[0][ct], p1, oe[ct], 0, 0, 0);
          }
          l_run += __shfl_xor(l_run, 16);
          l_run += __shfl_xor(l_run, 32);
          const float Mnew = MULTI ? fmaxf(Mrun[ii], m_run) : m_run;
          const float fac = (!MULTI || c == 0) ? 0.0f : expf(Mrun[ii] - Mnew);
          const float cf = MULTI ? expf(m_run - Mnew) : 1.0f;
          Mrun[ii] = Mnew;
          Lrun[ii] = Lrun[ii] * fac + l_run * cf;
          const float inv = last ? 1.0f / Lrun[ii] : 1.0f;
#pragma unroll
          for (int T = 0; T < NT / 2 - (MULTI ? 0 : 1); ++T) {
            const float f = FAST_EXP(m_hist[T] - Mnew);
            if (l15 < 8) {
#pragma unroll
              for (int tl = 0; tl < 2; ++tl) {
                f32x4* sp = reinterpret_cast<f32x4*>(Srow + (2 * T + tl) * 16 + 4 * q);
                f32x4 pv = *sp;
#pragma unroll
                for (int r = 0; r < 4; ++r) pv[r] *= f;
                *sp = pv;
              }
            }
          }
          if (l15 < 8) {
            float* fo = feat + (prow0 + i0 + il) * AF + FOFF_OE + h * AC + 4 * q;
            const float sc = cf * oscale_r;
#pragma unroll
            for (int ct = 0; ct < 4; ++ct) {
              f32x4 o = oe[ct];
#pragma unroll
              for (int r = 0; r < 4; ++r) o[r] *= sc;
              if (MULTI && c > 0) {
                const f32x4 old = *reinterpret_cast<const f32x4*>(fo + 16 * ct);
#pragma unroll
                for (int r = 0; r < 4; ++r) o[r] += old[r] * fac;
              }
#pragma unroll
              for (int r = 0; r < 4; ++r) o[r] *= inv;
              *reinterpret_cast<f32x4*>(fo + 16 * ct) = o;
            }
            if (q == 0) {
              st_fac[il * AH + h] = fac;
              st_inv[il * AH + h] = inv;
            }
          }
        }
      } else {
#pragma unroll
      for (int ii = 0; ii < 2; ++ii) {
        const int il = 2 * wv + ii;
        float* Srow = S + il * IS + h * HS;
        float lg[NT][4];
        float mx = -INFINITY;
        stage_e(ii, 0);
#pragma unroll
        for (int jt = 0; jt < NT; ++jt) {
          f32x4 acc = {0.f, 0.f, 0.f, 0.f}, acc2 = {0.f, 0.f, 0.f, 0.f};
          {
            if (jt + 1 < NT) stage_e(ii, jt + 1);
            const float* t_ = scr + (jt & 1) * (16 * ELD) + l15 * ELD + 4 * q;
#pragma unroll
            for (int sg = 0; sg < 4; ++sg) {
              const f32x4 ea = *reinterpret_cast<const f32x4*>(t_ + 16 * sg);
              const f32x4 wbf = MULTI ? *reinterpret_cast<const f32x4*>(wb_lds + (sg * 64 + lane) * 4) : wb[sg];
#pragma unroll
              for (int s = 0; s < 4; ++s) {
                if (sg & 1) acc2 = __builtin_amdgcn_mfma_f32_16x16x4f32(ea[s], wbf[s], acc2, 0, 0, 0);
                else acc = __builtin_amdgcn_mfma_f32_16x16x4f32(ea[s], wbf[s], acc, 0, 0, 0);
              }
            }
          }
          if (ii == 0 && jt + E_DEPTH0 < NT) {
            load_e_tile(0, c, jt + E_DEPTH0);
            MEM_FENCE();
          }
          const f32x4 sv = *reinterpret_cast<const f32x4*>(Srow + jt * 16 + 4 * q);
#pragma unroll
          for (int r = 0; r < 4; ++r) {
            const float v = sv[r] + bscale * (acc[r] + acc2[r]);
            lg[jt][r] = v;
            mx = fmaxf(mx, v);
          }
        }
        mx = fmaxf(mx, __shfl_xor(mx, 16));
        mx = fmaxf(mx, __shfl_xor(mx, 32));
        const float Mnew = fmaxf(Mrun[ii], mx);
        const float fac = c == 0 ? 0.0f : expf(Mrun[ii] - Mnew);
        float sum = 0.f;
#pragma unroll
        for (int jt = 0; jt < NT; ++jt)
#pragma unroll
          for (int r = 0; r < 4; ++r) {
            const float p = FAST_EXP(lg[jt][r] - Mnew);
            lg[jt][r] = p;
            sum += p;
          }
        sum += __shfl_xor(sum, 16);
        sum += __shfl_xor(sum, 32);
        Mrun[ii] = Mnew;
        Lrun[ii] = Lrun[ii] * fac + sum;
        const float inv = last ? 1.0f / Lrun[ii] : 1.0f;
        f32x4 oe[4];
#pragma unroll
        for (int ct = 0; ct < 4; ++ct) oe[ct] = f32x4{0.f, 0.f, 0.f, 0.f};
#pragma unroll
        for (int jt = 0; jt < NT; ++jt) {
          const f32x4 pv = {lg[jt][0], lg[jt][1], lg[jt][2], lg[jt][3]};
          if (l15 < 8) *reinterpret_cast<f32x4*>(Srow + jt * 16 + 4 * q) = pv;
#pragma unroll
          for (int r = 0; r < 4; ++r)
#pragma unroll
            for (int ct = 0; ct < 4; ++ct)
              oe[ct] = __builtin_amdgcn_mfma_f32_16x16x4f32(ev[ii][jt][r][ct], pv[r], oe[ct], 0, 0, 0);
          if (ii == 0 && jt >= E_LAG) {
            load_e_tile(1, c, jt - E_LAG);
            MEM_FENCE();
          }
        }
        if (ii == 0) {
#pragma unroll
          for (int jt = NT - E_LAG; jt < NT; ++jt) load_e_tile(1, c, jt);
          MEM_FENCE();
        }
        if (l15 < 8) {
          float* fo = feat + (prow0 + i0 + il) * AF + FOFF_OE + h * AC + 16 * q;
#pragma unroll
          for (int r = 0; r < 4; ++r) {
            f32x4 v = {oe[0][r], oe[1][r], oe[2][r], oe[3][r]};
            if (c > 0) {
              const f32x4 old = *reinterpret_cast<const f32x4*>(fo + 4 * r);
#pragma unroll
              for (int s = 0; s < 4; ++s) v[s] += old[s] * fac;
            }
#pragma unroll
            for (int s = 0; s < 4; ++s) v[s] *= inv;
            *reinterpret_cast<f32x4*>(fo + 4 * r) = v;
          }
          if (q == 0) {
            st_fac[il * AH + h] = fac;
            st_inv[il * AH + h] = inv;
          }
        }
      }
      }
    }
    if (c == 0) stamp(3);

    {
      const int h = wv;
      const int pp = l15 & 7;
      const int xy = l15 >> 3;
      constexpr int SD3 = NT < 4 ? NT : 4;
      f32x4 sv[SD3][4];
      int lane3 = lane0;
      asm volatile("" : "+v"(lane3));
      const AttnLaneOff lo3 = attn_lane_off(lane3);
      auto load_vals = [&](int sb, int jt) { attn_tile_request(sv[sb], proj, krow0 + 16 * jt, OFF_VS, OFF_GV, lo3, h); };
      const int vs_dst = (lane >> 3) * KLD + 4 * (lane & 7);
      const int g0v = lane, g1v = lane + 64;
      const int gv_dst0 = 16 * KLD + (g0v / 6) * GLD + 4 * (g0v % 6), gv_dst1 = 16 * KLD + (g1v / 6) * GLD + 4 * (g1v % 6);
      auto stage_vals = [&](int sb, int lb) {
        float* t_ = scr + lb * P1_TILE;
// ... 105 lines not shown
```

diffab-pytorch_amd/csrc/ipa_persistent.hip:

```cpp
#include "common.h"
#include "denoiser_internal.h"
#define AT_STAMP_REALTIME 1
#include "ipa_attn_tile.h"
#include "proj_frames_h3_tile.h"
#include "rowgemm_h3_tile.h"
#include "mlp_chain_tile.h"

namespace diffab {

namespace {
constexpr size_t cmax(size_t a, size_t b) { return a > b ? a : b; }
constexpr size_t kModuleLdsBytes = cmax(cmax(ipa_attn_lds_bytes(8), static_cast<size_t>(kChainLdsBytes)),
                                        cmax(static_cast<size_t>(pjh3::PJ_LDS_BYTES), static_cast<size_t>(h3tile::lds_bytes<128>())));

struct ModuleArgs {
  float* xa;
  float* xb;
  float* proj;
  float* feat;
  const float* pair;
  const float* esc;
  const int* ctx_of_row;
  const float* R;
  const float* t;
  const char* planes;
  size_t layer_stride, pj_off, out_off, wis_off, small_off;
  unsigned long long* stamps;
  const float* emb_X;
  MlpChainSet emb, heads;
  int B, NL;
  int stagger_ticks, stagger_classes;
};
}

template <int KRES>
__global__ __launch_bounds__(512) void ipa_module_persistent_kernel(const ModuleArgs a) {
  extern __shared__ __attribute__((aligned(16))) float lds[];
  constexpr int K = KRES, NTILE = K / TI, DT = K / 128;
  static_assert(KRES == 128 || KRES == 256, "patch-resident module: K = 128 or 256");
  const int M = a.B * K;
  if (a.stagger_ticks > 0 && a.stagger_classes > 1) {
    const unsigned long long t0 = __builtin_amdgcn_s_memrealtime();
    const unsigned long long wait = static_cast<unsigned long long>((blockIdx.x >> 3) % a.stagger_classes) * a.stagger_ticks;
    while (__builtin_amdgcn_s_memrealtime() - t0 < wait) __builtin_amdgcn_s_sleep(32);
  }
  unsigned long long* pstamps = a.stamps ? a.stamps + static_cast<size_t>(a.B) * a.NL * NTILE * 64 : nullptr;
  auto pstamp = [&](int b, int l, int k) {
    if (pstamps != nullptr && threadIdx.x == 0) pstamps[(static_cast<size_t>(b) * a.NL + l) * 4 + k] = __builtin_amdgcn_s_memrealtime();
  };
#pragma unroll 1
  for (int b = blockIdx.x; b < a.B; b += gridDim.x) {
    if (a.emb_X != nullptr) {
#pragma unroll 1
      for (int dt = 0; dt < DT; ++dt) {
        int tid = threadIdx.x;
        asm volatile("" : "+v"(tid));
        chaintile::mlp_chain_tile(reinterpret_cast<__bf16*>(lds), tid, b * DT + dt, a.emb_X, 128, a.emb.c[0].planes[0], a.emb.c[0].planes[1],
                                  nullptr, a.emb.c[0].bias[0], a.emb.c[0].bias[1], nullptr, a.emb.c[0].bias_idx0, a.emb.c[0].bias_div0, 2, 128,
                                  a.xa, 128, M);
        asm volatile("s_waitcnt vmcnt(0)" ::: "memory");
        __syncthreads();
      }
    }
#pragma unroll 1
    for (int l = 0; l < a.NL; ++l) {
      const char* lp = a.planes + static_cast<size_t>(l) * a.layer_stride;
      const float* small = reinterpret_cast<const float*>(lp + a.small_off);
      const float* xin = (l & 1) ? a.xb : a.xa;
      float* xout = (l & 1) ? a.xa : a.xb;
      pstamp(b, l, 0);
#pragma unroll 1
      for (int dt = 0; dt < DT; ++dt) {
        int tid = threadIdx.x;
        asm volatile("" : "+v"(tid));
        pjh3::proj_frames_h3_tile<true, false>(reinterpret_cast<_Float16*>(lds), tid, b * DT + dt, 0, 1, xin,
                                               reinterpret_cast<const _Float16*>(lp + a.pj_off), reinterpret_cast<const float*>(lp + a.wis_off),
                                               a.R, a.t, a.proj, M);
        if (dt + 1 < DT) {
          asm volatile("s_waitcnt vmcnt(0)" ::: "memory");
          __syncthreads();
        }
      }
      asm volatile("s_waitcnt vmcnt(0)" ::: "memory");
      __syncthreads();
      pstamp(b, l, 1);
#pragma unroll 1
      for (int tile = 0; tile < NTILE; ++tile) {
        ipa_attn_tile<8, (KRES > 128), true>(lds, b, tile, static_cast<unsigned>((b * a.NL + l) * NTILE + tile), a.proj, a.pair, a.R, a.t, small,
                                             small + 512, a.feat, K / 128, a.stamps, a.esc, nullptr, nullptr, a.ctx_of_row);
        asm volatile("s_waitcnt vmcnt(0)" ::: "memory");
        __syncthreads();
      }
      pstamp(b, l, 2);
#pragma unroll 1
      for (int dt = 0; dt < DT; ++dt) {
        int tid = threadIdx.x;
        asm volatile("" : "+v"(tid));
        h3tile::rowgemm128_h3_tile<false, 128>(reinterpret_cast<_Float16*>(lds), tid, b * DT + dt, a.feat, AF,
                                               reinterpret_cast<const _Float16*>(lp + a.out_off),
                                               reinterpret_cast<const float*>(lp + a.wis_off) + ANP, small + 576, nullptr, 0, xout, 128, M, AF);
        if (dt + 1 < DT) {
          asm volatile("s_waitcnt vmcnt(0)" ::: "memory");
          __syncthreads();
        }
      }
      asm volatile("s_waitcnt vmcnt(0)" ::: "memory");
      __syncthreads();
      pstamp(b, l, 3);
    }
    if (a.emb_X != nullptr) {
      const float* xfin = (a.NL & 1) ? a.xb : a.xa;
#pragma unroll 1
      for (int hdt = 0; hdt < 3 * DT; ++hdt) {
        const int hd = hdt / DT, dt = hdt % DT;
        int tid = threadIdx.x;
        asm volatile("" : "+v"(tid));
#define HSEL(f) (hd == 0 ? a.heads.c[0].f : hd == 1 ? a.heads.c[1].f : a.heads.c[2].f)
        chaintile::mlp_chain_tile(reinterpret_cast<__bf16*>(lds), tid, b * DT + dt, xfin, 128, HSEL(planes[0]), HSEL(planes[1]), HSEL(planes[2]),
                                  HSEL(bias[0]), HSEL(bias[1]), HSEL(bias[2]), HSEL(bias_idx0), HSEL(bias_div0), 3, HSEL(n_out),
                                  hd == 0 ? a.heads.Y[0] : hd == 1 ? a.heads.Y[1] : a.heads.Y[2],
                                  hd == 0 ? a.heads.ldy[0] : hd == 1 ? a.heads.ldy[1] : a.heads.ldy[2], M);
#undef HSEL
        asm volatile("s_waitcnt vmcnt(0)" ::: "memory");
        __syncthreads();
      }
    }
  }
}

namespace {
int g_stagger_ticks = 1000, g_stagger_classes = 8;
unsigned long long* g_module_stamps = nullptr;
}
void set_module_stagger(int ticks, int classes) {
  g_stagger_ticks = ticks;
  g_stagger_classes = classes;
}
void set_module_stamps(void* p) { g_module_stamps = static_cast<unsigned long long*>(p); }

bool ipa_module_persistent_supported(const diffab_dims* d) {
  return fast_path_supported(d) && (d->K == 128 || d->K == 256) && d->NL >= 1;
}

int launch_ipa_module_persistent(const diffab_dims* d, float* xa, float* xb, const float* R, const float* t, float* ws, const void* planes,
                                 const float* pair_planes, hipStream_t st, const float* emb_X, const MlpChainSet* emb,
                                 const MlpChainSet* heads, const int* ctx_of_row, int n_ctx) {
  DIFFAB_REQUIRE(ipa_module_persistent_supported(d) && xa && xb && R && t && ws && planes && pair_planes, DIFFAB_ERR_ARG,
                 "ipa_module_persistent: unsupported operands");
  const size_t rows = static_cast<size_t>(d->B) * d->K;
  ModuleArgs a{};
  a.xa = xa;
  a.xb = xb;
  a.proj = ws;
  a.feat = ws + rows * ANP;
  a.pair = pair_planes + 64;
  a.esc = pair_row_scales(d, pair_planes, n_ctx);
  a.ctx_of_row = ctx_of_row;
  a.R = R;
  a.t = t;
  a.planes = static_cast<const char*>(planes);
  a.layer_stride = ipa_layer_planes_bytes();
  a.pj_off = ipa_layer_h3_pj_offset();
  a.out_off = ipa_layer_h3_out_offset();
  a.wis_off = ipa_layer_h3_wis_offset();
  a.small_off = ipa_layer_small_offset();
  a.stamps = g_module_stamps;
  if (emb_X != nullptr) {
    DIFFAB_REQUIRE(emb && heads && d->D == 128 && (reinterpret_cast<uintptr_t>(emb_X) & 15) == 0, DIFFAB_ERR_ARG,
                   "ipa_module_persistent: the fused MLP phases need both chain sets");
    a.emb_X = emb_X;
    a.emb = *emb;
    a.heads = *heads;
  }
  a.B = d->B;
  a.NL = d->NL;
  a.stagger_ticks = g_stagger_ticks;
  a.stagger_classes = g_stagger_classes;
  int dev = 0, ncu = 256;
  if (hipGetDevice(&dev) == hipSuccess) (void)hipDeviceGetAttribute(&ncu, hipDeviceAttributeMultiprocessorCount, dev);
  const int grid = d->B < ncu ? d->B : ncu;
#define MODULE_LAUNCH(K_)                                                                                                       \
  do {                                                                                                                            \
    DIFFAB_HIP_CHECK(hipFuncSetAttribute(reinterpret_cast<const void*>(ipa_module_persistent_kernel<K_>),                         \
                                         hipFuncAttributeMaxDynamicSharedMemorySize, static_cast<int>(kModuleLdsBytes)));        \
    timer_begin(st);                                                                                                              \
    hipLaunchKernelGGL((ipa_module_persistent_kernel<K_>), dim3(grid), dim3(512), kModuleLdsBytes, st, a);                        \
    timer_end(st);                                                                                                                \
  } while (0)
  if (d->K == 128) MODULE_LAUNCH(128);
  else MODULE_LAUNCH(256);
#undef MODULE_LAUNCH
  DIFFAB_LAUNCH_CHECK();
  return DIFFAB_OK;
}

}
```

diffab-pytorch_amd/diffab_pytorch/_hip.py:

```python
from __future__ import annotations

import ctypes as C
import os
from typing import Dict, Optional, Sequence

import torch

_HERE = os.path.dirname(os.path.abspath(__file__))
LIB_PATH = os.environ.get("DIFFAB_HIP_LIB") or os.path.join(os.path.dirname(_HERE), "lib", "libdiffab_hip.so")

FLAG_FORCE_GENERIC = 1
FLAG_PAIR_F32 = 64
FLAG_FP32_GEMM = 128
FLAG_PAIR_PLANES = 32
FLAG_GRAPH_SAMPLER = 16
FLAG_PERSISTENT_MODULE = 512
FLAG_MULTI_LAUNCH = 1024
FLAG_SKIP_UNUSED_ROWS = 256
FLAG_KEEP_STRUCTURE = 2048
FLAG_KEEP_SEQUENCE = 4096


class HipUnavailable(RuntimeError):
    pass


class DiffabHipError(RuntimeError):
    pass


class Dims(C.Structure):
    _fields_ = [(n, C.c_int32) for n in ("B", "K", "D", "C", "H", "DS", "PQ", "PV", "NL", "V")]


_fp = C.c_void_p


class IpaLayerWeights(C.Structure):
    _fields_ = [(n, _fp) for n in ("gamma", "wq_s", "wk_s", "wv_s", "w_bias", "wq_p", "wk_p", "wv_p", "w_out", "b_out")]


class Mlp3Weights(C.Structure):
    _fields_ = [(n, _fp) for n in ("w0", "b0", "w2", "b2", "w4", "b4")]


class DenoiserWeights(C.Structure):
    _fields_ = [
        ("seq_emb", _fp), ("res_w0", _fp), ("res_b0", _fp), ("res_w2", _fp), ("res_b2", _fp),
        ("layers", C.POINTER(IpaLayerWeights)),
        ("coord", Mlp3Weights), ("orient", Mlp3Weights), ("seq", Mlp3Weights),
    ]


class CtxDims(C.Structure):
    _fields_ = [(n, C.c_int32) for n in ("B", "K", "A", "D", "C", "max_dist")]


class ResidueEmbWeights(C.Structure):
    _fields_ = [(n, _fp) for n in ("aa_emb", "chain_emb", "w0", "b0", "w2", "b2", "w4", "b4", "w6", "b6")]


class PairEmbWeights(C.Structure):
    _fields_ = [(n, _fp) for n in ("aa_pair_emb", "relpos_emb", "pair2distcoef", "dw0", "db0", "dw2", "db2", "mw0", "mb0", "mw2", "mb2",
                                   "mw4", "mb4")]


class Sched(C.Structure):
    _fields_ = [("T", C.c_int32), ("alpha", _fp), ("alpha_bar", _fp), ("alpha_bar_sqrt", _fp),
                ("one_minus_alpha_bar_sqrt", _fp), ("beta", _fp)]


class Igso3(C.Structure):
    _fields_ = [("n_sigmas", C.c_int32), ("n_bins", C.c_int32), ("sigmas", _fp), ("cdf", _fp), ("sigma_threshold", C.c_float)]


class ScoreNoised(C.Structure):
    _fields_ = [(n, _fp) for n in ("seq_t", "x_t", "O_t", "eps")]


class SampleRecord(C.Structure):
    _fields_ = [("n_slots", C.c_int32), ("slot_of_step", C.POINTER(C.c_int32)), ("slot_dev", _fp)] + \
        [(n, _fp) for n in ("seq", "x", "O", "pred_x", "pred_O", "seq_probs")]


_i32, _i64, _u32, _u64, _sz = C.c_int32, C.c_int64, C.c_uint32, C.c_uint64, C.c_size_t
_PD, _PS, _PI = C.POINTER(Dims), C.POINTER(Sched), C.POINTER(Igso3)
SYMBOLS = {
    "diffab_version": (C.c_char_p, []),
    "diffab_last_error": (C.c_char_p, []),
    "diffab_device_ok": (C.c_int, []),
    "diffab_kernel_timer_enable": (C.c_int, [C.c_int]),
    "diffab_debug_set_attn_stamps": (C.c_int, [_fp]),
    "diffab_debug_set_attn_variant": (C.c_int, [_i32]),
    "diffab_debug_set_module_stagger": (C.c_int, [_i32, _i32]),
    "diffab_debug_set_module_stamps": (C.c_int, [_fp]),
    "diffab_set_stream_guard": (C.c_int, [C.c_int]),
    "diffab_debug_linear128": (C.c_int, [_fp, _fp, _fp, _fp, C.c_int64, C.c_int32, C.c_int32, _fp, C.c_size_t, _fp]),
    "diffab_debug_gemm_tn": (C.c_int, [_fp, _fp, _fp, _fp, C.c_int64, C.c_int32, C.c_int32, C.c_int32, _fp]),
    "diffab_debug_xstat128": (C.c_int, [_fp, _fp, _fp, C.c_int64, C.c_int32, C.c_int32, _fp, C.c_size_t, _fp]),
    "diffab_kernel_timer_read": (C.c_int, [C.POINTER(C.c_int64), C.POINTER(C.c_double)]),
    "diffab_so3_log": (C.c_int, [_fp, _fp, _i64, _fp]),
    "diffab_so3_exp": (C.c_int, [_fp, _fp, _i64, _fp]),
    "diffab_so3_matrix_to_rotvec": (C.c_int, [_fp, _fp, _i64, _fp]),
    "diffab_so3_rotvec_to_matrix": (C.c_int, [_fp, _fp, _i64, _fp]),
    "diffab_so3_scale_rot": (C.c_int, [_fp, _fp, _fp, _i64, _i64, _fp]),
    "diffab_igso3_table_build": (C.c_int, [_fp, _i32, _i32, _i32, _fp, _fp]),
    "diffab_igso3_table_build_accurate": (C.c_int, [_fp, _i32, _i32, _i32, _fp, _fp]),
    "diffab_igso3_cdf_build": (C.c_int, [_fp, _i32, _i32, _fp, _fp]),
    "diffab_igso3_sample": (C.c_int, [_PI, _fp, _i32, _i32, _fp, _fp, _fp, _fp, _fp, _fp]),
    "diffab_igso3_bins_without_replacement": (C.c_int, [_fp, _i32, _i32, _fp, _i32, _i32, _fp, _fp, _fp, C.c_float, _fp]),
    "diffab_igso3_sample_bins": (C.c_int, [_PI, _fp, _i32, _i32, _fp, _fp, _fp, _fp, _fp, _fp]),
    "diffab_weighted_multinomial": (C.c_int, [_fp, _fp, _fp, _fp, _i64, _i64, _fp, _fp]),
    "diffab_seq_forward_prob": (C.c_int, [_PS, C.c_int, _fp, _fp, _fp, _i32, _i32, _fp, _fp]),
    "diffab_seq_posterior": (C.c_int, [_PS, _fp, _fp, _fp, _fp, _i32, _i32, _fp, _fp]),
    "diffab_categorical_sample": (C.c_int, [_fp, _fp, _i64, _i32, _fp, _fp]),
    "diffab_coord_forward": (C.c_int, [_PS, _fp, _fp, _fp, _fp, _i32, _i32, _fp, _fp]),
    "diffab_orient_forward": (C.c_int, [_PS, _fp, _fp, _fp, _fp, _i32, _i32, _fp, _fp]),
    "diffab_philox_fill": (C.c_int, [_u64, _i64, _i32, _i32, _i32, _i32, C.c_int, _fp, _fp]),
    "diffab_denoise_workspace_bytes": (_sz, [_PD]),
    "diffab_sample_workspace_bytes": (_sz, [_PD]),
    "diffab_sample_shared_workspace_bytes": (_sz, [_PD, _i32]),
    "diffab_ipa_layer_fwd": (C.c_int, [_PD, C.POINTER(IpaLayerWeights), _fp, _fp, _fp, _fp, _fp, _fp, _sz, _u32, _fp]),
    "diffab_denoise_step_fwd": (C.c_int, [_PD, C.POINTER(DenoiserWeights), _fp, _fp, _fp, _fp, _fp, _fp, _fp, _fp, _fp, _fp, _fp,
                                          _fp, _sz, _u32, _fp]),
    "diffab_losses_fwd": (C.c_int, [_fp, _fp, _fp, _fp, _fp, _fp, _fp, _fp, _i32, _i32, _i32, _fp, _fp]),
    "diffab_train_tape_bytes": (_sz, [_PD]),
    "diffab_train_workspace_bytes": (_sz, [_PD]),
    "diffab_train_step_fwd": (C.c_int, [_PD, C.POINTER(DenoiserWeights)] + [_fp] * 16 + [_sz, _u32, _fp]),
    "diffab_train_step_bwd": (C.c_int, [_PD, C.POINTER(DenoiserWeights), C.POINTER(DenoiserWeights)] + [_fp] * 16 + [_sz, _fp, _sz, _fp]),
    "diffab_residue_embedding_workspace_bytes": (_sz, [C.POINTER(CtxDims)]),
    "diffab_residue_embedding_fwd": (C.c_int, [C.POINTER(CtxDims), C.POINTER(ResidueEmbWeights)] + [_fp] * 10 + [_sz, _fp]),
    "diffab_pair_embedding_workspace_bytes": (_sz, [C.POINTER(CtxDims)]),
    "diffab_pair_embedding_fwd": (C.c_int, [C.POINTER(CtxDims), C.POINTER(PairEmbWeights), _fp, _fp, _fp, _fp, _i32, _fp, _fp, _fp, _fp,
                                            _fp, _sz, _fp]),
    "diffab_pair_embedding_xyz_fwd": (C.c_int, [C.POINTER(CtxDims), C.POINTER(PairEmbWeights), _fp, _fp, _fp, _fp, _i32, _fp, _fp, _fp, _fp,
                                                _fp, _sz, _fp]),
    "diffab_residue_embedding_bwd_workspace_bytes": (_sz, [C.POINTER(CtxDims)]),
    "diffab_residue_embedding_bwd": (C.c_int, [C.POINTER(CtxDims), C.POINTER(ResidueEmbWeights), C.POINTER(ResidueEmbWeights)] + [_fp] * 10
                                     + [_sz, _fp]),
    "diffab_pair_embedding_bwd_workspace_bytes": (_sz, [C.POINTER(CtxDims)]),
    "diffab_pair_embedding_bwd": (C.c_int, [C.POINTER(CtxDims), C.POINTER(PairEmbWeights), C.POINTER(PairEmbWeights), _fp, _fp, _fp, _fp, _fp,
                                            _i32, _fp, _fp, _fp, _fp, _fp, _sz, _fp]),
    "diffab_pair_embedding_tape_bytes": (_sz, [C.POINTER(CtxDims)]),
    "diffab_pair_embedding_fwd_taped": (C.c_int, [C.POINTER(CtxDims), C.POINTER(PairEmbWeights), _fp, _fp, _fp, _fp, _fp, _i32, _fp, _fp, _fp,
                                                  _fp, _fp, _sz, _fp, _sz, _fp]),
    "diffab_pair_embedding_bwd_taped": (C.c_int, [C.POINTER(CtxDims), C.POINTER(PairEmbWeights), C.POINTER(PairEmbWeights), _fp, _fp, _fp, _fp,
                                                  _fp, _i32, _fp, _fp, _fp, _fp, _fp, _sz, _fp, _sz, _fp]),
    "diffab_featurize_xyz": (C.c_int, [_fp, _fp, _fp, _i32, _i32, _i32, _fp, _fp, _fp, _fp, _fp]),
    "diffab_orientation_loss": (C.c_int, [_fp, _fp, _i64, _fp, _fp, _fp]),
    "diffab_orientation_loss_bwd": (C.c_int, [_fp, _fp, _i64, _fp, _fp, _fp, _fp, _fp]),
    "diffab_frames_apply": (C.c_int, [_fp, _fp, _fp, _fp, _i32, _i32, _i32, _i32, _fp]),
    "diffab_frames_invert": (C.c_int, [_fp, _fp, _fp, _fp, _i32, _i32, _i32, _i32, _fp]),
    "diffab_frames_bwd": (C.c_int, [_fp, _fp, _fp, _fp, _i32, _fp, _fp, _i32, _i32, _i32, _i32, _fp]),
    "diffab_angular_encoding": (C.c_int, [_fp, _i64, _i32, _fp, _fp]),
    "diffab_angular_encoding_bwd": (C.c_int, [_fp, _fp, _i64, _i32, _fp, _fp]),
    "diffab_denoise_step_fwd_taped": (C.c_int, [_PD, C.POINTER(DenoiserWeights)] + [_fp] * 10 + [_sz, _u32, _fp]),
    "diffab_denoise_step_bwd": (C.c_int, [_PD, C.POINTER(DenoiserWeights), C.POINTER(DenoiserWeights)] + [_fp] * 13 + [_sz, _fp, _sz, _fp]),
    "diffab_ipa_layer_tape_bytes": (_sz, [_PD]),
    "diffab_ipa_layer_bwd_workspace_bytes": (_sz, [_PD]),
    "diffab_ipa_layer_fwd_taped": (C.c_int, [_PD, C.POINTER(IpaLayerWeights), _fp, _fp, _fp, _fp, _fp, _fp, _sz, _u32, _fp]),
    "diffab_ipa_layer_bwd": (C.c_int, [_PD, C.POINTER(IpaLayerWeights), C.POINTER(IpaLayerWeights), _fp, _fp, _fp, _fp, _fp, _fp, _fp, _fp, _fp,
                                       _sz, _fp, _sz, _fp]),
    "diffab_reverse_update": (C.c_int, [_PS, _i32, _fp, _fp, _fp, _fp, _fp, _fp, _fp, _fp, _fp, _fp, _i32, _i32, _i32, _fp]),
    "diffab_sample_loop": (C.c_int, [_PD, C.POINTER(DenoiserWeights), _PS, _PI, _fp, _fp, _fp, _fp, _fp, _fp, _u64, _i64, _i32,
                                     _i32, _fp, _sz, _u32, _fp]),
    "diffab_sample_loop_shared": (C.c_int, [_PD, C.POINTER(DenoiserWeights), _PS, _PI, _fp, _fp, _fp, _fp, _fp, _i32, C.POINTER(_i32), _fp,
                                            _u64, _i64, _i32, _i32, _fp, _sz, _u32, _fp]),
    "diffab_sample_init": (C.c_int, [_fp, _fp, _fp, _fp, _u64, _i64, _i32, _i32, _i32, _fp]),
    "diffab_sample_init_ex": (C.c_int, [_fp, _fp, _fp, _fp, _u64, _i64, _i32, _i32, _i32, _u32, _fp]),
    "diffab_sample_init_noised": (C.c_int, [_PS, _PI, _fp, _fp, _fp, _fp, _u64, _i64, _i32, _i32, _i32, _u32, _fp]),
    "diffab_sample_loop_aa": (C.c_int, [_PD, C.POINTER(DenoiserWeights), _PS, _PI, _fp, _fp, _fp, _fp, _fp, _i32, C.POINTER(_i32), _fp,
                                        _u64, _i64, _i32, _i32, _fp, _sz, _u32, _fp, _fp]),
    "diffab_sample_init_aa": (C.c_int, [_fp, _fp, _fp, _fp, _u64, _i64, _i32, _i32, _i32, _u32, _fp, _fp]),
    "diffab_sample_init_noised_aa": (C.c_int, [_PS, _PI, _fp, _fp, _fp, _fp, _u64, _i64, _i32, _i32, _i32, _u32, _fp, _fp]),
    "diffab_sample_loop_rec": (C.c_int, [_PD, C.POINTER(DenoiserWeights), _PS, _PI, _fp, _fp, _fp, _fp, _fp, _i32, C.POINTER(_i32), _fp,
                                         _u64, _i64, _i32, _i32, _fp, _sz, _u32, _fp, C.POINTER(SampleRecord), _fp]),
    "diffab_score_workspace_bytes": (_sz, [_PD, _i32]),
    "diffab_score_designs": (C.c_int, [_PD, C.POINTER(DenoiserWeights), _PS, _PI, _fp, _fp, _fp, _fp, _fp, _i32, _fp, _fp, _i32,
                                       C.POINTER(_i32), C.POINTER(_i32), _i32, _i32, _u64, _i64, _fp, _fp, C.POINTER(ScoreNoised), _fp, _sz,
                                       _u32, _fp]),
# ... 114 lines not shown
```

include/diffab_hip.h:

```cpp
#ifndef DIFFAB_HIP_H
#define DIFFAB_HIP_H

#include <stddef.h>
#include <stdint.h>

#ifdef __cplusplus
extern "C" {
#endif

#define DIFFAB_OK 0
#define DIFFAB_ERR_ARG (-1)
#define DIFFAB_ERR_UNSUPPORTED (-2)
#define DIFFAB_ERR_HIP (-3)
#define DIFFAB_ERR_WORKSPACE (-4)

#define DIFFAB_FLAG_FORCE_GENERIC 1u

#define DIFFAB_FLAG_PAIR_PLANES 32u

#define DIFFAB_FLAG_PAIR_F32 64u
#define DIFFAB_FLAG_FP32_GEMM 128u

#define DIFFAB_FLAG_GRAPH_SAMPLER 16u
#define DIFFAB_FLAG_PERSISTENT_MODULE 512u
#define DIFFAB_FLAG_MULTI_LAUNCH 1024u
#define DIFFAB_FLAG_SKIP_UNUSED_ROWS 256u
#define DIFFAB_FLAG_KEEP_STRUCTURE 2048u
#define DIFFAB_FLAG_KEEP_SEQUENCE 4096u

typedef struct {
  int32_t B;
  int32_t K;
  int32_t D;
  int32_t C;
  int32_t H;
  int32_t DS;
  int32_t PQ;
  int32_t PV;
  int32_t NL;
  int32_t V;
} diffab_dims;

typedef struct {
  const float* gamma;
  const float* wq_s;
  const float* wk_s;
  const float* wv_s;
  const float* w_bias;
  const float* wq_p;
  const float* wk_p;
  const float* wv_p;
  const float* w_out;
  const float* b_out;
} diffab_ipa_layer_weights;

typedef struct {
  const float *w0, *b0;
  const float *w2, *b2;
  const float *w4, *b4;
} diffab_mlp3_weights;

typedef struct {
  const float* seq_emb;
  const float *res_w0, *res_b0;
  const float *res_w2, *res_b2;
  const diffab_ipa_layer_weights* layers;
  diffab_mlp3_weights coord;
  diffab_mlp3_weights orient;
  diffab_mlp3_weights seq;
} diffab_denoiser_weights;

typedef struct {
  int32_t T;
  const float* alpha;
  const float* alpha_bar;
  const float* alpha_bar_sqrt;
  const float* one_minus_alpha_bar_sqrt;
  const float* beta;
} diffab_sched;

typedef struct {
  int32_t n_sigmas;
  int32_t n_bins;
  const float* sigmas;
  const float* cdf;
  float sigma_threshold;
} diffab_igso3;

const char* diffab_version(void);
const char* diffab_last_error(void);
int diffab_device_ok(void);

int diffab_kernel_timer_enable(int on);
int diffab_debug_set_attn_stamps(void* device_buffer);
int diffab_debug_set_attn_variant(int32_t v);
int diffab_debug_set_module_stagger(int32_t ticks_10ns, int32_t classes);
int diffab_debug_set_module_stamps(void* device_buffer);
int diffab_set_stream_guard(int on);
int diffab_debug_linear128(const float* X, const float* W, const float* bias, float* Y, int64_t M, int32_t Kd, int32_t mode, void* scratch,
                           size_t scratch_bytes, void* stream);
int diffab_debug_xstat128(const float* X, const float* W, float* Y, int64_t M, int32_t N, int32_t mode, void* scratch, size_t scratch_bytes,
                          void* stream);
int diffab_debug_gemm_tn(const float* A, const float* B, float* C, float* db, int64_t M, int32_t N1, int32_t N2, int32_t mode, void* stream);
int diffab_kernel_timer_read(int64_t* launches, double* total_ms);
int diffab_so3_log(const float* R, float* S, int64_t n, void* stream);
int diffab_so3_exp(const float* S, float* R, int64_t n, void* stream);
int diffab_so3_matrix_to_rotvec(const float* R, float* v, int64_t n, void* stream);
int diffab_so3_rotvec_to_matrix(const float* v, float* R, int64_t n, void* stream);
int diffab_so3_scale_rot(const float* R, const float* k, float* out, int64_t n, int64_t per_k, void* stream);

int diffab_igso3_table_build(const float* sigmas, int32_t n_sigmas, int32_t n_bins, int32_t num_iters, float* pdf, void* stream);
int diffab_igso3_table_build_accurate(const float* sigmas, int32_t n_sigmas, int32_t n_bins, int32_t num_iters, float* pdf,
                                      void* stream);
int diffab_igso3_cdf_build(const float* pdf, int32_t n_sigmas, int32_t n_bins, float* cdf, void* stream);
int diffab_igso3_sample(const diffab_igso3* tab, const int64_t* sigma_idx, int32_t B, int32_t K, const float* axis_raw,
                        const float* u_bin, const float* u_in, const float* z, float* rotvec, void* stream);

int diffab_igso3_bins_without_replacement(const float* pdf, int32_t n_sigmas, int32_t n_bins, const int64_t* sigma_idx, int32_t B,
                                          int32_t K, const float* race, int32_t* bins, const float* sigmas, float sigma_threshold,
                                          void* stream);
int diffab_igso3_sample_bins(const diffab_igso3* tab, const int64_t* sigma_idx, int32_t B, int32_t K, const float* axis_raw,
                             const int32_t* bins, const float* u_in, const float* z, float* rotvec, void* stream);

int diffab_weighted_multinomial(const float* p1, const float* p2, const float* w1, const float* w2, int64_t n, int64_t per_b,
                                float* out, void* stream);
int diffab_seq_forward_prob(const diffab_sched* s, int mode, const int64_t* seq, const int64_t* t, const uint8_t* mask,
                            int32_t B, int32_t K, float* prob , void* stream);
int diffab_seq_posterior(const diffab_sched* s, const int64_t* seq_t, const int64_t* seq_0, const int64_t* t,
                         const uint8_t* mask, int32_t B, int32_t K, float* post , void* stream);
int diffab_categorical_sample(const float* prob, const float* u, int64_t n_rows, int32_t V, int64_t* out, void* stream);
int diffab_coord_forward(const diffab_sched* s, const float* x0, const int64_t* t, const uint8_t* mask, const float* eps,
                         int32_t B, int32_t K, float* xt, void* stream);
int diffab_orient_forward(const diffab_sched* s, const float* O0, const uint8_t* mask, const int64_t* t,
                          const float* rotvec, int32_t B, int32_t K, float* Ot, void* stream);

int diffab_philox_fill(uint64_t seed, int64_t first_patch, int32_t B, int32_t K, int32_t step, int32_t stream_id, int kind,
                       float* out, void* stream);

size_t diffab_denoise_workspace_bytes(const diffab_dims* d);
size_t diffab_sample_workspace_bytes(const diffab_dims* d);
size_t diffab_sample_shared_workspace_bytes(const diffab_dims* d, int32_t n_ctx);
int diffab_ipa_layer_fwd(const diffab_dims* d, const diffab_ipa_layer_weights* w, const float* x ,
                         const float* e , const float* R , const float* t ,
                         float* y , void* workspace, size_t workspace_bytes, uint32_t flags, void* stream);
int diffab_denoise_step_fwd(const diffab_dims* d, const diffab_denoiser_weights* w, const int64_t* seq_t, const float* x_t,
                            const float* O_t, const float* res_ctx, const float* pair_ctx, const float* beta ,
                            float* out_eps, float* out_O0, float* out_posterior, float* out_logits, float* out_res_emb,
                            void* workspace, size_t workspace_bytes, uint32_t flags, void* stream);

int diffab_losses_fwd(const float* pred_post, const float* true_post, const float* pred_eps, const float* true_eps,
                      const float* pred_O0, const float* true_O0, const uint8_t* gen_mask, const uint8_t* res_mask,
                      int32_t B, int32_t K, int32_t V, float* losses3, void* stream);

size_t diffab_train_tape_bytes(const diffab_dims* d);
size_t diffab_train_workspace_bytes(const diffab_dims* d);
int diffab_train_step_fwd(const diffab_dims* d, const diffab_denoiser_weights* w, const int64_t* seq_t, const float* x_t,
                          const float* O_t, const float* res_ctx, const float* pair_ctx, const float* beta, const float* true_post,
                          const float* true_eps, const float* true_O0, const uint8_t* gen_mask, const uint8_t* res_mask,
                          float* out_eps, float* out_O0, float* out_posterior, float* losses3, void* tape, size_t tape_bytes,
                          uint32_t flags, void* stream);
int diffab_train_step_bwd(const diffab_dims* d, const diffab_denoiser_weights* w, const diffab_denoiser_weights* grads,
                          const int64_t* seq_t, const float* x_t, const float* O_t, const float* pair_ctx, const float* out_eps,
                          const float* out_O0, const float* out_posterior, const float* true_post, const float* true_eps,
                          const float* true_O0, const uint8_t* gen_mask, const uint8_t* res_mask, const float* upstream3,
                          float* d_res_ctx, float* d_pair_ctx, const void* tape, size_t tape_bytes, void* workspace,
                          size_t workspace_bytes, void* stream);

int diffab_orientation_loss(const float* pred, const float* target, int64_t n, float* elems, float* sum1, void* stream);
int diffab_orientation_loss_bwd(const float* pred, const float* target, int64_t n, const float* g_elems, const float* g_total,
                                float* d_pred, float* d_target, void* stream);

int diffab_frames_apply(const float* x, const float* R, const float* t, float* out, int32_t B, int32_t N, int32_t L, int32_t P, void* stream);
int diffab_frames_invert(const float* x, const float* R, const float* t, float* out, int32_t B, int32_t N, int32_t L, int32_t P, void* stream);
int diffab_frames_bwd(const float* x, const float* R, const float* t, const float* g_out, int32_t invert, float* dR, float* dt, int32_t B,
                      int32_t N, int32_t L, int32_t P, void* stream);
int diffab_angular_encoding(const float* x, int64_t n, int32_t num_funcs, float* out, void* stream);
int diffab_angular_encoding_bwd(const float* enc, const float* g_out, int64_t n, int32_t num_funcs, float* dx, void* stream);

int diffab_denoise_step_fwd_taped(const diffab_dims* d, const diffab_denoiser_weights* w, const int64_t* seq_t, const float* x_t,
                                  const float* O_t, const float* res_ctx, const float* pair_ctx, const float* beta, float* out_eps,
                                  float* out_O0, float* out_posterior, void* tape, size_t tape_bytes, uint32_t flags, void* stream);
int diffab_denoise_step_bwd(const diffab_dims* d, const diffab_denoiser_weights* w, const diffab_denoiser_weights* grads,
                            const int64_t* seq_t, const float* x_t, const float* O_t, const float* pair_ctx, const float* out_posterior,
// ... 142 lines not shown
```

Measured before the change: 13.07 million.

## Precompute per-layer pair bias once per context and restructure pair-plane layout

```diff
diff --git a/diffab-pytorch_amd/csrc/api.hip b/diffab-pytorch_amd/csrc/api.hip
--- a/diffab-pytorch_amd/csrc/api.hip
+++ b/diffab-pytorch_amd/csrc/api.hip
@@ -126,11 +126,12 @@
 static int ipa_layer_dispatch(const diffab_dims* d, const diffab_ipa_layer_weights* w, const float* x, const float* e, const float* R,
                               const float* t, float* y, float* ws, uint32_t flags, hipStream_t st, float* sp_keep = nullptr,
                               float* d2_keep = nullptr, const void* planes = nullptr, const float* pair_planes = nullptr,
+                              const float* pair_bias = nullptr,
                               bool taped = false,
                               const unsigned char* tile_needed = nullptr, const int* ctx_of_row = nullptr, int n_ctx = 0) {
   DIFFAB_REQUIRE(ipa_layer_weights_ok(d, w), DIFFAB_ERR_ARG, "ipa layer: null weight pointer");
   if (!(flags & DIFFAB_FLAG_FORCE_GENERIC) && fast_path_supported(d))
-    return ipa_layer_fast(d, w, x, e, R, t, y, ws, st, sp_keep, d2_keep, planes, pair_planes, (flags & DIFFAB_FLAG_FP32_GEMM) != 0,
+    return ipa_layer_fast(d, w, x, e, R, t, y, ws, st, sp_keep, d2_keep, planes, pair_planes, pair_bias, (flags & DIFFAB_FLAG_FP32_GEMM) != 0,
                           taped, tile_needed, ctx_of_row, n_ctx);
   return ipa_layer_generic(d, w, x, e, R, t, y, ws, st, ctx_of_row);
 }
@@ -202,6 +203,14 @@
   int traj_rows;
 };
 
+static int build_pair_operands(const diffab_dims* d, const float* pair_ctx, const diffab_ipa_layer_weights* layers, int nl, float* pair,
+                               hipStream_t st, int n_pair) {
+  if (int rc = launch_pair_split(d, pair_ctx, pair, st, n_pair)) return rc;
+  std::vector<const float*> wb(nl);
+  for (int l = 0; l < nl; ++l) wb[l] = layers[l].w_bias;
+  return launch_pair_bias(d, pair_ctx, wb.data(), nl, const_cast<float*>(pair_bias_of_layer(d, pair, n_pair, 0)), st, n_pair);
+}
+
 static int prepare_forward(const diffab_dims* d, const diffab_denoiser_weights* w, const ForwardPlan& p, const StepBuffers& b,
                            const float* pair_ctx, const StepBias& bias, hipStream_t st) {
   if (p.fold)
@@ -222,7 +231,7 @@
     }
   }
   if (p.pair_planes)
-    if (int rc = launch_pair_split(d, pair_ctx, b.pair, st, p.n_ctx)) return rc;
+    if (int rc = build_pair_operands(d, pair_ctx, w->layers, d->NL, b.pair, st, p.n_ctx)) return rc;
   if (bias.beta_traj) {
     diffab_dims dt = *d;
     dt.B = bias.traj_rows;
@@ -288,8 +297,9 @@
   }
   for (int l = 0; l < d->NL && !p.persistent; ++l) {
     const void* planes = p.b6 ? b.planes + l * ipa_layer_planes_bytes() : nullptr;
+    const float* pair_bias = p.pair_planes ? pair_bias_of_layer(d, p.pair_planes, p.n_ctx, l) : nullptr;
     if (int rc = ipa_layer_dispatch(d, &w->layers[l], cur, pair_ctx, O_t, x_t, nxt, b.ipa, p.flags, st, nullptr, nullptr, planes, p.pair_planes,
-                                    false, l == d->NL - 1 ? p.last_layer_tiles : nullptr, p.ctx_of_row, p.n_ctx))
+                                    pair_bias, false, l == d->NL - 1 ? p.last_layer_tiles : nullptr, p.ctx_of_row, p.n_ctx))
       return rc;
     float* tmp = cur; cur = nxt; nxt = tmp;
   }
@@ -330,7 +340,7 @@
     if (b6)
       if (int rc = ipa_layer_split_weights(&w->layers[l], tp.planes, st)) return rc;
     if (int rc = ipa_layer_dispatch(d, &w->layers[l], tp.x[l], pair_ctx, O_t, x_t, tp.x[l + 1], tp.ipa_ws[l], flags, st, tp.sp[l], tp.d2[l],
-                                    b6 ? tp.planes : nullptr, nullptr, true))
+                                    b6 ? tp.planes : nullptr, nullptr, nullptr, true))
       return rc;
   }
   if (int rc = launch_beta_concat(tp.x[d->NL], beta, D, d->K, rows, tp.cat3, st)) return rc;
@@ -422,6 +432,17 @@
   return std::strncmp(p.gcnArchName, "gfx950", 6) == 0 ? 1 : 0;
 }
 
+int diffab_debug_pair_bias(const diffab_dims* d, const diffab_ipa_layer_weights* layers, int32_t n_layers, const float* e, int32_t n_pair,
+                           float* out, void* stream) {
+  StreamOrder order_(stream);
+  if (int rc = check_dims(d, "debug_pair_bias")) return rc;
+  DIFFAB_REQUIRE(pair_planes_supported(d) && layers && n_layers >= 1 && n_pair >= 1 && e && out, DIFFAB_ERR_ARG,
+                 "debug_pair_bias: bad operands (the MFMA geometry, n_layers >= 1, n_pair >= 1)");
+  std::vector<const float*> wb(n_layers);
+  for (int l = 0; l < n_layers; ++l) wb[l] = layers[l].w_bias;
+  return launch_pair_bias(d, e, wb.data(), n_layers, out, as_stream(stream), n_pair);
+}
+
 int diffab_debug_linear128(const float* X, const float* W, const float* bias, float* Y, int64_t M, int32_t Kd, int32_t mode, void* scratch,
                            size_t scratch_bytes, void* stream) {
   StreamOrder order_(stream);
@@ -536,10 +557,11 @@
   DIFFAB_REQUIRE(workspace_bytes >= b.bytes, DIFFAB_ERR_WORKSPACE, "ipa_layer_fwd: workspace %zu < %zu bytes", workspace_bytes, b.bytes);
   const float* pair_planes = nullptr;
   if (use_pair_planes(d, flags, e, b)) {
-    if (int rc = launch_pair_split(d, e, b.pair, as_stream(stream))) return rc;
+    if (int rc = build_pair_operands(d, e, w, 1, b.pair, as_stream(stream), 0)) return rc;
     pair_planes = b.pair;
   }
-  return ipa_layer_dispatch(d, w, x, e, R, t, y, b.ipa, flags, as_stream(stream), nullptr, nullptr, nullptr, pair_planes);
+  return ipa_layer_dispatch(d, w, x, e, R, t, y, b.ipa, flags, as_stream(stream), nullptr, nullptr, nullptr, pair_planes,
+                            pair_planes ? pair_bias_of_layer(d, pair_planes, 0, 0) : nullptr);
 }
 
 int diffab_denoise_step_fwd(const diffab_dims* d, const diffab_denoiser_weights* w, const int64_t* seq_t, const float* x_t, const float* O_t,
@@ -680,7 +702,7 @@
   if (b6)
     if (int rc = ipa_layer_split_weights(w, tp.planes, st)) return rc;
   if (int rc = ipa_layer_dispatch(&d1, w, tp.x[0], e, R, t, tp.x[1], tp.ipa_ws[0], flags, st, tp.sp[0], tp.d2[0], b6 ? tp.planes : nullptr,
-                                  nullptr, true))
+                                  nullptr, nullptr, true))
     return rc;
   DIFFAB_HIP_CHECK(hipMemcpyAsync(y, tp.x[1], nb, hipMemcpyDeviceToDevice, st));
   return DIFFAB_OK;
diff --git a/diffab-pytorch_amd/csrc/denoiser_fast.hip b/diffab-pytorch_amd/csrc/denoiser_fast.hip
--- a/diffab-pytorch_amd/csrc/denoiser_fast.hip
+++ b/diffab-pytorch_amd/csrc/denoiser_fast.hip
@@ -303,7 +303,8 @@
                                                             unsigned long long* __restrict__ stamps, const float* __restrict__ esc = nullptr,
                                                             float* __restrict__ tape_p = nullptr, float* __restrict__ tape_d2 = nullptr,
                                                             const unsigned char* __restrict__ tile_needed = nullptr,
-                                                            const int* __restrict__ ctx_of_row = nullptr) {
+                                                            const int* __restrict__ ctx_of_row = nullptr,
+                                                            const float* __restrict__ pbias = nullptr) {
   extern __shared__ __attribute__((aligned(16))) float S[];
   const int ntile = (MULTI ? NC_arg : 1) * NT;
   int b, tile;
@@ -317,7 +318,8 @@
     tile = bid % ntile;
   }
   if (tile_needed != nullptr && !tile_needed[b * ntile + tile]) return;
-  ipa_attn_tile<NT, MULTI, PLANES, TAPE>(S, b, tile, bid, proj, e, R, t, Wb, gamma, feat, NC_arg, stamps, esc, tape_p, tape_d2, ctx_of_row);
+  ipa_attn_tile<NT, MULTI, PLANES, TAPE>(S, b, tile, bid, proj, e, R, t, Wb, gamma, feat, NC_arg, stamps, esc, tape_p, tape_d2, ctx_of_row,
+                                         pbias);
 }
 
 static unsigned long long* g_attn_stamps = nullptr;
@@ -415,52 +417,131 @@
     rs[2 * row + 1] = ok ? __uint_as_float(static_cast<unsigned>(ex - 7) << 23) : 1.0f;
   }
 }
-__global__ void pair_split_kernel(const float* __restrict__ e, const float* __restrict__ rs, int K, int64_t n_groups,
-                                  _Float16* __restrict__ out) {
+__global__ __launch_bounds__(256) void pair_split_kernel(const float* __restrict__ e, const float* __restrict__ rs, int K, int64_t n_threads,
+                                                         _Float16* __restrict__ out) {
   const int64_t gid = blockIdx.x * static_cast<int64_t>(blockDim.x) + threadIdx.x;
-  if (gid >= n_groups) return;
-  const int cg = static_cast<int>(gid & 7);
-  const int64_t rj = gid >> 3;
-  const int j = static_cast<int>(rj % K);
-  const int64_t row = rj / K;
+  if (gid >= n_threads) return;
+  const int cg = static_cast<int>(gid & 7), g = static_cast<int>((gid >> 3) & 3);
+  const int64_t rT = gid >> 5;
+  const int T = static_cast<int>(rT % (K / 32));
+  const int64_t row = rT / (K / 32);
   const float s = rs[2 * row];
-  const f32x4 v0 = reinterpret_cast<const f32x4*>(e)[gid * 2], v1 = reinterpret_cast<const f32x4*>(e)[gid * 2 + 1];
-  f16x8 h1, h2;
-#pragma unroll
-  for (int c = 0; c < 8; ++c) {
-    const float x = (c < 4 ? v0[c & 3] : v1[c & 3]) * s;
-    const _Float16 a = static_cast<_Float16>(x);
-    h1[c] = a;
-    h2[c] = static_cast<_Float16>(x - static_cast<float>(a));
-  }
-  const int jt = j >> 4, l15 = j & 15, ks = cg >> 2, g = cg & 3;
-  _Float16* base = out + (row * K) * 128 + static_cast<int64_t>(jt) * 2048 + ks * 512 + (l15 + 16 * g) * 8;
-  *reinterpret_cast<f16x8*>(base) = h1;
-  *reinterpret_cast<f16x8*>(base + 1024) = h2;
-}
+  const float* src = e + (row * K + 32 * T + 8 * g) * AC + 8 * cg;
+  f32x4 v[8][2];
+#pragma unroll
+  for (int k = 0; k < 8; ++k) {
+    v[k][0] = *reinterpret_cast<const f32x4*>(src + k * AC);
+    v[k][1] = *reinterpret_cast<const f32x4*>(src + k * AC + 4);
+  }
+  const int ct = cg >> 1;
+  _Float16* base = out + row * K * 128 + static_cast<int64_t>(T) * 4096 + ct * 1024 + (8 * (cg & 1) + 16 * g) * 8;
+#pragma unroll
+  for (int cc = 0; cc < 8; ++cc) {
+    f16x8 h1, h2;
+#pragma unroll
+    for (int k = 0; k < 8; ++k) {
+      const float x = v[k][cc >> 2][cc & 3] * s;
+      const _Float16 a = static_cast<_Float16>(x);
+      h1[k] = a;
+      h2[k] = static_cast<_Float16>(x - static_cast<float>(a));
+    }
+    *reinterpret_cast<f16x8*>(base + cc * 8) = h1;
+    *reinterpret_cast<f16x8*>(base + 512 + cc * 8) = h2;
+  }
+}
+
+constexpr int kBiasLayersPerLaunch = 8;
+struct PairBiasWeights { const float* w[kBiasLayersPerLaunch]; };
+__global__ __launch_bounds__(256) void pair_bias_kernel(const float* __restrict__ e, const PairBiasWeights wl, int nl, int K,
+                                                        int64_t layer_stride, float* __restrict__ out) {
+  __shared__ __attribute__((aligned(16))) float ws[kBiasLayersPerLaunch * AH * AC];
+  for (int i = threadIdx.x; i < nl * AH * AC; i += 256) ws[i] = wl.w[i / (AH * AC)][i % (AH * AC)];
+  __syncthreads();
+  const int t = threadIdx.x, r = t & 3, l15 = (t >> 2) & 15, q = t >> 6;
+  const int nkt = K / 16;
+  const int64_t pb = blockIdx.x / nkt;
+  const int it = static_cast<int>(blockIdx.x % nkt);
+  const int i = 16 * it + 4 * q + r;
+  const float scale_t = 0.57735026918962576f;
+  const float* erow = e + (pb * K + i) * K * AC;
+  float* orow = out + blockIdx.x * static_cast<int64_t>(AH) * nkt * 256 + 4 * (l15 + 16 * q) + r;
+#pragma unroll 1
+  for (int jt = 0; jt < nkt; jt += 2) {
+    f32x4 x0[16], x1[16];
+    const f32x4* p0 = reinterpret_cast<const f32x4*>(erow + (16 * jt + l15) * AC);
+#pragma unroll
+    for (int k = 0; k < 16; ++k) {
+      x0[k] = p0[k];
+      x1[k] = p0[16 * AC / 4 + k];
+    }
+#pragma unroll 1
+    for (int l = 0; l < nl; ++l) {
+#pragma unroll
+      for (int h = 0; h < AH; ++h) {
+        const f32x4* wr = reinterpret_cast<const f32x4*>(ws + (l * AH + h) * AC);
+        float a0 = 0.f, a1 = 0.f;
+#pragma unroll
+        for (int k = 0; k < 16; ++k) {
+          const f32x4 w4 = wr[k];
+#pragma unroll
+          for (int s = 0; s < 4; ++s) {
+            a0 = fmaf(x0[k][s], w4[s], a0);
+            a1 = fmaf(x1[k][s], w4[s], a1);
+          }
+        }
+        float* o = orow + l * layer_stride + (static_cast<int64_t>(h) * nkt + jt) * 256;
+        o[0] = scale_t * a0;
+        o[256] = scale_t * a1;
+      }
+    }
+  }
+}
+
 bool pair_planes_supported(const diffab_dims* d) { return fast_path_supported(d); }
 static size_t pair_patches(const diffab_dims* d, int n_pair) { return static_cast<size_t>(n_pair > 0 ? n_pair : d->B); }
+static size_t pair_bias_layers(const diffab_dims* d) { return static_cast<size_t>(d->NL > 1 ? d->NL : 1); }
 size_t pair_planes_floats(const diffab_dims* d, int n_pair) {
   const size_t np = pair_patches(d, n_pair);
-  return pair_planes_supported(d) ? np * d->K * d->K * AC + 64 + 2 * np * d->K + 64 : 0;
+  return pair_planes_supported(d) ? np * d->K * d->K * AC + 64 + 2 * np * d->K + 64 + pair_bias_layers(d) * np * d->K * d->K * AH : 0;
 }
 const float* pair_row_scales(const diffab_dims* d, const float* planes, int n_pair) {
   return planes + 64 + pair_patches(d, n_pair) * d->K * d->K * AC;
+}
+const float* pair_bias_of_layer(const diffab_dims* d, const float* planes, int n_pair, int l) {
+  const size_t np = pair_patches(d, n_pair);
+  return pair_row_scales(d, planes, n_pair) + 2 * np * d->K + 64 + static_cast<size_t>(l) * np * d->K * d->K * AH;
 }
 int launch_pair_split(const diffab_dims* d, const float* e, float* planes, hipStream_t st, int n_pair) {
   DIFFAB_REQUIRE(pair_planes_supported(d) && e && planes && (reinterpret_cast<uintptr_t>(planes) & 15) == 0 &&
                      (reinterpret_cast<uintptr_t>(e) & 15) == 0,
                  DIFFAB_ERR_ARG, "pair_split: unsupported operands");
   const int64_t np = static_cast<int64_t>(pair_patches(d, n_pair));
-  const int64_t n = np * d->K * d->K * AC;
+  const int64_t n = np * d->K * (d->K / 32) * 32;
   float* rs = const_cast<float*>(pair_row_scales(d, planes, n_pair));
   hipLaunchKernelGGL(pair_rowscale_kernel, dim3(static_cast<unsigned>(np * d->K)), dim3(256), 0, st, e, d->K * AC / 4, rs);
-  hipLaunchKernelGGL(pair_split_kernel, dim3(static_cast<unsigned>((n / 8 + 255) / 256)), dim3(256), 0, st, e, rs, d->K, n / 8,
+  hipLaunchKernelGGL(pair_split_kernel, dim3(static_cast<unsigned>((n + 255) / 256)), dim3(256), 0, st, e, rs, d->K, n,
                      reinterpret_cast<_Float16*>(planes + 64));
   DIFFAB_LAUNCH_CHECK();
   return DIFFAB_OK;
 }
-
+int launch_pair_bias(const diffab_dims* d, const float* e, const float* const* w_bias, int nl, float* out, hipStream_t st, int n_pair) {
+  DIFFAB_REQUIRE(pair_planes_supported(d) && e && out && nl >= 1 && (reinterpret_cast<uintptr_t>(e) & 15) == 0, DIFFAB_ERR_ARG,
+                 "pair_bias: unsupported operands");
+  const int64_t np = static_cast<int64_t>(pair_patches(d, n_pair));
+  const int64_t layer_stride = np * d->K * d->K * AH;
+  for (int l0 = 0; l0 < nl; l0 += kBiasLayersPerLaunch) {
+    PairBiasWeights wl{};
+    const int n = nl - l0 < kBiasLayersPerLaunch ? nl - l0 : kBiasLayersPerLaunch;
+    for (int l = 0; l < n; ++l) {
+      DIFFAB_REQUIRE(w_bias[l0 + l] != nullptr, DIFFAB_ERR_ARG, "pair_bias: null w_bias of layer %d", l0 + l);
+      wl.w[l] = w_bias[l0 + l];
+    }
+    hipLaunchKernelGGL(pair_bias_kernel, dim3(static_cast<unsigned>(np * (d->K / 16))), dim3(256), 0, st, e, wl, n, d->K, layer_stride,
+                       out + l0 * layer_stride);
+    DIFFAB_LAUNCH_CHECK();
+  }
+  return DIFFAB_OK;
+}
 
 bool use_b6_gemm(uint32_t flags) { return !(flags & DIFFAB_FLAG_FP32_GEMM); }
 static size_t round256(size_t b) { return (b + 255) & ~static_cast<size_t>(255); }
@@ -501,7 +582,7 @@
 
 int ipa_layer_fast(const diffab_dims* d, const diffab_ipa_layer_weights* w, const float* x, const float* e, const float* R, const float* t,
                    float* y, float* ws, hipStream_t st, float* sp_keep, float* d2_keep, const void* planes, const float* pair_planes,
-                   bool fp32_gemm, bool taped, const unsigned char* tile_needed, const int* ctx_of_row, int n_ctx) {
+                   const float* pair_bias, bool fp32_gemm, bool taped, const unsigned char* tile_needed, const int* ctx_of_row, int n_ctx) {
   const int rows = d->B * d->K, D = d->D;
   DIFFAB_REQUIRE(ctx_of_row == nullptr || sp_keep == nullptr, DIFFAB_ERR_ARG, "ipa_layer_fast: shared contexts are an inference form");
   float* proj = ws;
@@ -543,6 +624,7 @@
   const size_t lds = ipa_attn_lds_bytes(nt);
   const dim3 grid(d->B * (d->K / TI));
   const bool use_planes = pair_planes != nullptr && pair_planes_supported(d);
+  DIFFAB_REQUIRE(!use_planes || pair_bias != nullptr, DIFFAB_ERR_ARG, "ipa_layer_fast: pair planes without their pair bias");
   const float* e_arg = use_planes ? pair_planes + 64 : e;
   const float* esc = use_planes ? pair_row_scales(d, pair_planes, n_ctx) : nullptr;
 #define ATTN_LAUNCH(NT_, MULTI_, PLANES_)                                                                                             \
@@ -551,7 +633,7 @@
                                          hipFuncAttributeMaxDynamicSharedMemorySize, static_cast<int>(lds)));                         \
     timer_begin(st);                                                                                                                  \
     hipLaunchKernelGGL((ipa_attn_fast_kernel<NT_, MULTI_, PLANES_>), grid, dim3(512), lds, st, proj, e_arg, R, t, w->w_bias, w->gamma, \
-                       feat, d->B, nc, g_attn_stamps, esc, nullptr, nullptr, tile_needed, ctx_of_row);                                \
+                       feat, d->B, nc, g_attn_stamps, esc, nullptr, nullptr, tile_needed, ctx_of_row, PLANES_ ? pair_bias : nullptr);     \
     timer_end(st);                                                                                                                    \
   } while (0)
   if (tape) {
diff --git a/diffab-pytorch_amd/csrc/denoiser_internal.h b/diffab-pytorch_amd/csrc/denoiser_internal.h
--- a/diffab-pytorch_amd/csrc/denoiser_internal.h
+++ b/diffab-pytorch_amd/csrc/denoiser_internal.h
@@ -28,6 +28,7 @@
                    float* sp_keep = nullptr, float* d2_keep = nullptr,
                    const void* planes = nullptr,
                    const float* pair_planes = nullptr,
+                   const float* pair_bias = nullptr,
                    bool fp32_gemm = false,
                    bool taped = false,
                    const unsigned char* tile_needed = nullptr,
@@ -36,6 +37,8 @@
 size_t pair_planes_floats(const diffab_dims* d, int n_pair = 0);
 int launch_pair_split(const diffab_dims* d, const float* e, float* planes, hipStream_t st, int n_pair = 0);
 const float* pair_row_scales(const diffab_dims* d, const float* planes, int n_pair = 0);
+const float* pair_bias_of_layer(const diffab_dims* d, const float* planes, int n_pair, int l);
+int launch_pair_bias(const diffab_dims* d, const float* e, const float* const* w_bias, int nl, float* out, hipStream_t st, int n_pair = 0);
 int launch_linear(const float* X, int ldx, const float* W, const float* bias, float* Y, int ldy, int M, int N, int Kd, bool relu,
                   hipStream_t st);
 
diff --git a/diffab-pytorch_amd/csrc/ipa_attn_tile.h b/diffab-pytorch_amd/csrc/ipa_attn_tile.h
--- a/diffab-pytorch_amd/csrc/ipa_attn_tile.h
+++ b/diffab-pytorch_amd/csrc/ipa_attn_tile.h
@@ -63,13 +63,17 @@
 }
 
 template <bool PLANES, typename FP>
-__device__ __forceinline__ void attn_shift_pair_rows(FP& e, FP& esc, const int* __restrict__ ctx_of_row, const int b, const int K) {
+__device__ __forceinline__ void attn_shift_pair_rows(FP& e, FP& esc, FP& pbias, const int* __restrict__ ctx_of_row, const int b,
+                                                     const int K) {
   if (ctx_of_row == nullptr) return;
   int c;
   asm volatile("s_load_dword %0, %1, 0x0\n\ts_waitcnt lgkmcnt(0)" : "=s"(c) : "s"(ctx_of_row + b) : "memory");
   const int64_t shift = static_cast<int64_t>(c - b) * K;
   e += shift * K * AC;
-  if constexpr (PLANES) esc += 2 * shift;
+  if constexpr (PLANES) {
+    esc += 2 * shift;
+    pbias += shift * K * AH;
+  }
 }
 
 template <int NT, bool MULTI, bool PLANES = false, bool TAPE = false>
@@ -80,7 +84,7 @@
                                               float* __restrict__ feat, int NC_arg,
                                               unsigned long long* __restrict__ stamps, const float* __restrict__ esc = nullptr,
                                               float* __restrict__ tape_p = nullptr, float* __restrict__ tape_d2 = nullptr,
-                                              const int* __restrict__ ctx_of_row = nullptr) {
+                                              const int* __restrict__ ctx_of_row = nullptr, const float* __restrict__ pbias = nullptr) {
   static_assert(!PLANES || NT % 2 == 0, "the o_e product takes key tiles in pairs");
   static_assert(!TAPE || (!MULTI && !PLANES), "the tape form is the single-chunk fp32-pair kernel");
   const int NC = MULTI ? NC_arg : 1;
@@ -103,7 +107,7 @@
   const int tid = threadIdx.x, lane0 = tid & 63, wv = __builtin_amdgcn_readfirstlane(tid >> 6);
   constexpr int HS = KC + 8, IS = AH * (KC + 8) + 8;
   const int64_t prow0 = static_cast<int64_t>(b) * K;
-  attn_shift_pair_rows<PLANES>(e, esc, ctx_of_row, b, K);
+  attn_shift_pair_rows<PLANES>(e, esc, pbias, ctx_of_row, b, K);
   const float scale_t = 0.57735026918962576f;
 
   constexpr int KLD = 40, GLD = 28;
@@ -136,6 +140,8 @@
     Mrun[ii] = -INFINITY;
     Lrun[ii] = 0.f;
   }
+  float Mrow = -INFINITY, Lrow = 0.f;
+  const float* brow = PLANES ? pbias + ((static_cast<int64_t>(b) * (K / 16) + tile) * AH + wv) * (K * 16) : nullptr;
   float inv_s2[2];
 #pragma unroll
   for (int ii = 0; ii < 2; ++ii) inv_s2[ii] = 1.0f;
@@ -153,7 +159,6 @@
     asm volatile("" : "+v"(lane));
     const int l15 = lane & 15, q = lane >> 4;
     f32x4 ev[2][NT][4];
-    f32x4 wv4[2][2];
     auto load_e_tile = [&](int ii, int cc_, int jt) {
       if constexpr (PLANES) {
         const f32x4* ep = reinterpret_cast<const f32x4*>(erow[ii]) + (cc_ * NT + jt) * 256 + lane;
@@ -172,11 +177,24 @@
       const int ks_dst = (lane >> 3) * KLD + 4 * (lane & 7);
       const int g0 = lane, g1 = lane + 64;
       const int gk_dst0 = 16 * KLD + (g0 / 6) * GLD + 4 * (g0 % 6), gk_dst1 = 16 * KLD + (g1 / 6) * GLD + 4 * (g1 % 6);
+#ifdef ATTN_TMP_SD3
+      constexpr int SD = (MULTI || PLANES) ? 3 : 4;
+#else
       constexpr int SD = MULTI ? 3 : 4;
+#endif
       static_assert(E_EARLY <= SD, "the early pair tiles are requested in the last E_EARLY iterations, which must not request key tiles any more");
       AttnP1Pre<SD> pre;
       f32x4 (&st)[SD][4] = pre.st;
+#ifdef ATTN_TMP_SD3
+      constexpr int BL = 2;
+#else
+      constexpr int BL = SD - 1;
+#endif
+      f32x4 bt[2];
       const AttnLaneOff lo = attn_lane_off(lane);
+      auto load_bias = [&](int m) {
+        if constexpr (PLANES) bt[m % 2] = __builtin_nontemporal_load(reinterpret_cast<const f32x4*>(brow + static_cast<unsigned>(4 * lane + (c * NT + m) * 256)));
+      };
       auto load_keys = [&](int sb, int jt) { attn_tile_request(st[sb], proj, krow0 + 16 * jt, OFF_KS, OFF_GK, lo, h); };
       auto stage_keys = [&](int sb, int lb) {
         float* t_ = scr + lb * P1_TILE;
@@ -187,7 +205,10 @@
       };
       attn_p1_request<SD>(pre, SD, proj, prow0, krow0, i0, lane, lo, h);
 #pragma unroll
-      for (int piece = 0; piece < SD && piece < NT; ++piece) attn_p1_request<SD>(pre, piece, proj, prow0, krow0, i0, lane, lo, h);
+      for (int piece = 0; piece < SD && piece < NT; ++piece) {
+        if (piece >= BL && piece - BL < SD - BL) load_bias(piece - BL);
+        attn_p1_request<SD>(pre, piece, proj, prow0, krow0, i0, lane, lo, h);
+      }
       f32x4 (&qa)[2] = pre.qa;
       MEM_FENCE();
       *reinterpret_cast<f32x4*>(gq_lds + 4 * g0) = pre.gqr[0];
@@ -215,18 +236,11 @@
         if (jt + 2 < NT) stage_keys((jt + 2) % SD, jt & 1);
         KeyFrag nxt = cur;
         if (jt + 1 < NT) nxt = read_frags(jt + 1);
+        const f32x4 bcur = PLANES ? bt[jt % 2] : f32x4{0.f, 0.f, 0.f, 0.f};
+        if (jt + SD - BL < NT) load_bias(jt + SD - BL);
         if (jt + SD < NT) {
           load_keys(jt % SD, jt + SD);
         } else if (jt + E_EARLY >= NT) {
-          if constexpr (PLANES) {
-            if (jt + E_EARLY == NT) {
-              const int hh = lane & 7, qq = lane >> 4;
-#pragma unroll
-              for (int ks = 0; ks < 2; ++ks)
-#pragma unroll
-                for (int hf = 0; hf < 2; ++hf) wv4[ks][hf] = *reinterpret_cast<const f32x4*>(Wb + hh * AC + 32 * ks + 8 * qq + 4 * hf);
-            }
-          }
           load_e_tile(0, c, jt + E_EARLY - NT);
         }
         MEM_FENCE();
@@ -256,11 +270,45 @@
             d2v = __builtin_elementwise_fma(dhi, dhi, d2v);
           }
           const float d2 = d2v[0] + d2v[1];
-          S[(4 * q + r) * IS + h * HS + jt * 16 + l15] = scale_t * (acc[r] * scale_s + coef_p * d2);
+          S[(4 * q + r) * IS + h * HS + jt * 16 + l15] = scale_t * (acc[r] * scale_s + coef_p * d2) + bcur[r];
           if constexpr (TAPE) tape_d2[((static_cast<int64_t>(b) * AH + h) * K + i0 + 4 * q + r) * K + jt * 16 + l15] = d2;
         }
         if (c == 0 && jt == 0) stamp(6);
         if (c == 0 && jt == 3) stamp(7);
+      }
+      if constexpr (PLANES) {
+        const int srow = (lane & 7) + 8 * (lane >> 5);
+        float* sp = S + srow * IS + h * HS + 4 * (2 * ((lane >> 4) & 1) + ((lane >> 3) & 1));
+        f32x4 x[NT];
+#pragma unroll
+        for (int k = 0; k < NT; ++k) x[k] = *reinterpret_cast<const f32x4*>(sp + 16 * k);
+        float mx = x[0][0];
+#pragma unroll
+        for (int k = 0; k < NT; ++k)
+#pragma unroll
+          for (int s_ = 0; s_ < 4; ++s_) mx = fmaxf(mx, x[k][s_]);
+        mx = fmaxf(mx, __shfl_xor(mx, 8));
+        mx = fmaxf(mx, __shfl_xor(mx, 16));
+        const float Mnew = MULTI ? fmaxf(Mrow, mx) : mx;
+        const float fac = (!MULTI || c == 0) ? 0.0f : expf(Mrow - Mnew);
+        float sum = 0.f;
+#pragma unroll
+        for (int k = 0; k < NT; ++k) {
+#pragma unroll
+          for (int s_ = 0; s_ < 4; ++s_) {
+            x[k][s_] = FAST_EXP(x[k][s_] - Mnew);
+            sum += x[k][s_];
+          }
+          *reinterpret_cast<f32x4*>(sp + 16 * k) = x[k];
+        }
+        sum += __shfl_xor(sum, 8);
+        sum += __shfl_xor(sum, 16);
+        Mrow = Mnew;
+        Lrow = Lrow * fac + sum;
+        if (((lane >> 3) & 3) == 0) {
+          st_fac[srow * AH + h] = fac;
+          st_inv[srow * AH + h] = last ? 1.0f / Lrow : 1.0f;
+        }
       }
     }
     if (c == 0) stamp(1);
@@ -269,41 +317,10 @@
       constexpr int E_DEPTH_FP32 = 3;
       constexpr int RT = NT / 2;
       constexpr int E_DEPTH0 = PLANES ? RT : (E_DEPTH_FP32 < NT ? (E_DEPTH_FP32 > E_EARLY ? E_DEPTH_FP32 : E_EARLY) : NT);
-      if constexpr (!PLANES) {
-#pragma unroll
-        for (int jt = E_EARLY; jt < E_DEPTH0; ++jt) load_e_tile(0, c, jt);
-      }
+#pragma unroll
+      for (int jt = E_EARLY; jt < E_DEPTH0; ++jt) load_e_tile(0, c, jt);
       f32x4 wb[4];
-      f16x8 wp[2][2];
-      float bscale = scale_t, oscale = 1.0f;
-      if constexpr (PLANES) {
-        float wmax = 0.f;
-#pragma unroll
-        for (int ks = 0; ks < 2; ++ks)
-#pragma unroll
-          for (int hf = 0; hf < 2; ++hf)
-#pragma unroll
-            for (int s = 0; s < 4; ++s) wmax = fmaxf(wmax, fabsf(wv4[ks][hf][s]));
-#pragma unroll
-        for (int o = 1; o < 64; o <<= 1) wmax = fmaxf(wmax, __shfl_xor(wmax, o));
-        const int ew = static_cast<int>((__float_as_uint(wmax) >> 23) & 255u);
-        const float sw = (ew == 0 || ew > 230) ? 1.0f : __uint_as_float(static_cast<unsigned>(127 + 7 + 127 - ew) << 23);
-        const float isw = (ew == 0 || ew > 230) ? 1.0f : __uint_as_float(static_cast<unsigned>(ew - 7) << 23);
-#pragma unroll
-        for (int ks = 0; ks < 2; ++ks)
-#pragma unroll
-          for (int c8 = 0; c8 < 8; ++c8) {
-            const float x = l15 < 8 ? wv4[ks][c8 >> 2][c8 & 3] * sw : 0.0f;
-            const _Float16 h1 = static_cast<_Float16>(x);
-            wp[0][ks][c8] = h1;
-            wp[1][ks][c8] = static_cast<_Float16>(x - static_cast<float>(h1));
-          }
-        bscale = scale_t * isw;
-        oscale = 1.0f / 256.0f;
-        asm volatile("" ::"v"(wp[0][0]), "v"(wp[1][0]), "v"(wp[0][1]), "v"(wp[1][1]));
-#pragma unroll
-        for (int jt = E_EARLY; jt < E_DEPTH0; ++jt) load_e_tile(0, c, jt);
-      } else if constexpr (!MULTI) {
+      if constexpr (!PLANES && !MULTI) {
 #pragma unroll
         for (int sg = 0; sg < 4; ++sg) {
           wb[sg] = *reinterpret_cast<const f32x4*>(Wb + h * AC + 16 * sg + 4 * q);
@@ -321,133 +338,49 @@
       };
 
       if constexpr (PLANES) {
-        char* trt = reinterpret_cast<char*>(scr);
-        const int wr_off = l15 * 128 + 8 * ((2 * q) ^ (4 * ((l15 >> 1) & 3)) ^ (2 * (l15 & 1)));
-        const int rrow = 4 * q + (l15 >> 2);
-        const int rd_off = rrow * 128 + 8 * ((l15 & 3) ^ (4 * ((rrow >> 1) & 3)) ^ (2 * (rrow & 1)));
+        const float oscale = 1.0f / 256.0f;
 #pragma unroll
         for (int ii = 0; ii < 2; ++ii) {
           const int il = 2 * wv + ii;
-          float* Srow = S + il * IS + h * HS;
-          const float inv_s = inv_s2[ii];
-          const float bscale_r = bscale * inv_s, oscale_r = oscale * inv_s;
-          float m_run = -INFINITY, l_run = 0.f, m_hist[NT / 2];
+          const float* Srow = S + il * IS + h * HS;
           f32x4 oe[4];
 #pragma unroll
           for (int ct = 0; ct < 4; ++ct) oe[ct] = f32x4{0.f, 0.f, 0.f, 0.f};
 #pragma unroll
           for (int T = 0; T < NT / 2; ++T) {
-            f32x4 acc[2][2];
-#pragma unroll
-            for (int tl = 0; tl < 2; ++tl)
-#pragma unroll
-              for (int ks = 0; ks < 2; ++ks) {
-                const f16x8 a1 = __builtin_bit_cast(f16x8, ev[ii][2 * T + tl][ks]), a2 = __builtin_bit_cast(f16x8, ev[ii][2 * T + tl][2 + ks]);
-                f32x4 a_ = {0.f, 0.f, 0.f, 0.f};
-                a_ = __builtin_amdgcn_mfma_f32_16x16x32_f16(a2, wp[0][ks], a_, 0, 0, 0);
-                a_ = __builtin_amdgcn_mfma_f32_16x16x32_f16(a1, wp[1][ks], a_, 0, 0, 0);
-                a_ = __builtin_amdgcn_mfma_f32_16x16x32_f16(a1, wp[0][ks], a_, 0, 0, 0);
-                acc[tl][ks] = a_;
-              }
-            float v[8], smax = -INFINITY;
-#pragma unroll
-            for (int tl = 0; tl < 2; ++tl) {
-              const f32x4 sv = *reinterpret_cast<const f32x4*>(Srow + (2 * T + tl) * 16 + 4 * q);
-#pragma unroll
-              for (int r = 0; r < 4; ++r) {
-                v[4 * tl + r] = sv[r] + bscale_r * (acc[tl][0][r] + acc[tl][1][r]);
-                smax = fmaxf(smax, v[4 * tl + r]);
-              }
-            }
-            smax = fmaxf(smax, __shfl_xor(smax, 16));
-            smax = fmaxf(smax, __shfl_xor(smax, 32));
-            const float m_new = fmaxf(m_run, smax);
-            const float alpha = T == 0 ? 0.0f : FAST_EXP(m_run - m_new);
-            m_run = m_new;
-            m_hist[T] = m_new;
-            float psum = 0.f;
+            const f32x4 pa = *reinterpret_cast<const f32x4*>(Srow + 32 * T + 8 * q);
+            const f32x4 pb = *reinterpret_cast<const f32x4*>(Srow + 32 * T + 8 * q + 4);
+            f16x8 p1, p2;
 #pragma unroll
             for (int tt = 0; tt < 8; ++tt) {
-              v[tt] = FAST_EXP(v[tt] - m_new);
-              psum += v[tt];
-            }
-            l_run = l_run * alpha + psum;
-            if (T > 0) {
-#pragma unroll
-              for (int ct = 0; ct < 4; ++ct)
-#pragma unroll
-                for (int r = 0; r < 4; ++r) oe[ct][r] *= alpha;
-            }
-            f16x8 p1, p2;
-#pragma unroll
-            for (int tt = 0; tt < 8; ++tt) {
-              const float x = 256.0f * v[tt];
+              const float x = 256.0f * (tt < 4 ? pa[tt] : pb[tt - 4]);
               const _Float16 hh = static_cast<_Float16>(x);
               p1[tt] = hh;
               p2[tt] = static_cast<_Float16>(x - static_cast<float>(hh));
             }
 #pragma unroll
-            for (int tl = 0; tl < 2; ++tl) {
-              if (l15 < 8) *reinterpret_cast<f32x4*>(Srow + (2 * T + tl) * 16 + 4 * q) = f32x4{v[4 * tl], v[4 * tl + 1], v[4 * tl + 2], v[4 * tl + 3]};
-#pragma unroll
-              for (int pl = 0; pl < 2; ++pl)
-#pragma unroll
-                for (int ks = 0; ks < 2; ++ks)
-                  *reinterpret_cast<f32x4*>(trt + (tl * 2 + pl) * 2048 + (wr_off ^ (64 * ks))) = ev[ii][2 * T + tl][2 * pl + ks];
-            }
+            for (int ct = 0; ct < 4; ++ct)
+              oe[ct] = __builtin_amdgcn_mfma_f32_16x16x32_f16(__builtin_bit_cast(f16x8, ev[ii][2 * T + (ct >> 1)][2 * (ct & 1) + 1]), p1, oe[ct], 0, 0, 0);
+#pragma unroll
+            for (int ct = 0; ct < 4; ++ct)
+              oe[ct] = __builtin_amdgcn_mfma_f32_16x16x32_f16(__builtin_bit_cast(f16x8, ev[ii][2 * T + (ct >> 1)][2 * (ct & 1)]), p2, oe[ct], 0, 0, 0);
+#pragma unroll
+            for (int ct = 0; ct < 4; ++ct)
+              oe[ct] = __builtin_amdgcn_mfma_f32_16x16x32_f16(__builtin_bit_cast(f16x8, ev[ii][2 * T + (ct >> 1)][2 * (ct & 1)]), p1, oe[ct], 0, 0, 0);
             {
-              constexpr int dummy_ = 0;
-              (void)dummy_;
               const int nx = ii * NT + 2 * T + RT;
               if (nx < 2 * NT) {
+                __builtin_amdgcn_sched_barrier(0);
                 load_e_tile(nx / NT, c, nx % NT);
                 load_e_tile((nx + 1) / NT, c, (nx + 1) % NT);
                 MEM_FENCE();
               }
             }
-            f16x8 a[2][4];
-#pragma unroll
-            for (int pl = 0; pl < 2; ++pl)
-#pragma unroll
-              for (int ct = 0; ct < 4; ++ct) {
-                const int ro = rd_off ^ (32 * ct);
-                const s16x4_t lo = __builtin_amdgcn_ds_read_tr16_b64_v4i16((s16x4_t __attribute__((address_space(3)))*)(trt + (0 * 2 + pl) * 2048 + ro));
-                const s16x4_t hi = __builtin_amdgcn_ds_read_tr16_b64_v4i16((s16x4_t __attribute__((address_space(3)))*)(trt + (1 * 2 + pl) * 2048 + ro));
-                const s16x8_t v8 = {lo[0], lo[1], lo[2], lo[3], hi[0], hi[1], hi[2], hi[3]};
-                a[pl][ct] = __builtin_bit_cast(f16x8, v8);
-              }
-#pragma unroll
-            for (int ct = 0; ct < 4; ++ct) oe[ct] = __builtin_amdgcn_mfma_f32_16x16x32_f16(a[1][ct], p1, oe[ct], 0, 0, 0);
-#pragma unroll
-            for (int ct = 0; ct < 4; ++ct) oe[ct] = __builtin_amdgcn_mfma_f32_16x16x32_f16(a[0][ct], p2, oe[ct], 0, 0, 0);
-#pragma unroll
-            for (int ct = 0; ct < 4; ++ct) oe[ct] = __builtin_amdgcn_mfma_f32_16x16x32_f16(a[0][ct], p1, oe[ct], 0, 0, 0);
-          }
-          l_run += __shfl_xor(l_run, 16);
-          l_run += __shfl_xor(l_run, 32);
-          const float Mnew = MULTI ? fmaxf(Mrun[ii], m_run) : m_run;
-          const float fac = (!MULTI || c == 0) ? 0.0f : expf(Mrun[ii] - Mnew);
-          const float cf = MULTI ? expf(m_run - Mnew) : 1.0f;
-          Mrun[ii] = Mnew;
-          Lrun[ii] = Lrun[ii] * fac + l_run * cf;
-          const float inv = last ? 1.0f / Lrun[ii] : 1.0f;
-#pragma unroll
-          for (int T = 0; T < NT / 2 - (MULTI ? 0 : 1); ++T) {
-            const float f = FAST_EXP(m_hist[T] - Mnew);
-            if (l15 < 8) {
-#pragma unroll
-              for (int tl = 0; tl < 2; ++tl) {
-                f32x4* sp = reinterpret_cast<f32x4*>(Srow + (2 * T + tl) * 16 + 4 * q);
-                f32x4 pv = *sp;
-#pragma unroll
-                for (int r = 0; r < 4; ++r) pv[r] *= f;
-                *sp = pv;
-              }
-            }
           }
           if (l15 < 8) {
             float* fo = feat + (prow0 + i0 + il) * AF + FOFF_OE + h * AC + 4 * q;
-            const float sc = cf * oscale_r;
+            const float sc = oscale * inv_s2[ii];
+            const float fac = st_fac[il * AH + h], inv = st_inv[il * AH + h];
 #pragma unroll
             for (int ct = 0; ct < 4; ++ct) {
               f32x4 o = oe[ct];
@@ -461,10 +394,6 @@
 #pragma unroll
               for (int r = 0; r < 4; ++r) o[r] *= inv;
               *reinterpret_cast<f32x4*>(fo + 16 * ct) = o;
-            }
-            if (q == 0) {
-              st_fac[il * AH + h] = fac;
-              st_inv[il * AH + h] = inv;
             }
           }
         }
@@ -500,7 +429,7 @@
           const f32x4 sv = *reinterpret_cast<const f32x4*>(Srow + jt * 16 + 4 * q);
 #pragma unroll
           for (int r = 0; r < 4; ++r) {
-            const float v = sv[r] + bscale * (acc[r] + acc2[r]);
+            const float v = sv[r] + scale_t * (acc[r] + acc2[r]);
             lg[jt][r] = v;
             mx = fmaxf(mx, v);
           }
diff --git a/diffab-pytorch_amd/csrc/ipa_persistent.hip b/diffab-pytorch_amd/csrc/ipa_persistent.hip
--- a/diffab-pytorch_amd/csrc/ipa_persistent.hip
+++ b/diffab-pytorch_amd/csrc/ipa_persistent.hip
@@ -20,6 +20,8 @@
   float* feat;
   const float* pair;
   const float* esc;
+  const float* bias;
+  size_t bias_stride;
   const int* ctx_of_row;
   const float* R;
   const float* t;
@@ -87,7 +89,8 @@
 #pragma unroll 1
       for (int tile = 0; tile < NTILE; ++tile) {
         ipa_attn_tile<8, (KRES > 128), true>(lds, b, tile, static_cast<unsigned>((b * a.NL + l) * NTILE + tile), a.proj, a.pair, a.R, a.t, small,
-                                             small + 512, a.feat, K / 128, a.stamps, a.esc, nullptr, nullptr, a.ctx_of_row);
+                                             small + 512, a.feat, K / 128, a.stamps, a.esc, nullptr, nullptr, a.ctx_of_row,
+                                             a.bias + l * a.bias_stride);
         asm volatile("s_waitcnt vmcnt(0)" ::: "memory");
         __syncthreads();
       }
@@ -155,6 +158,8 @@
   a.feat = ws + rows * ANP;
   a.pair = pair_planes + 64;
   a.esc = pair_row_scales(d, pair_planes, n_ctx);
+  a.bias = pair_bias_of_layer(d, pair_planes, n_ctx, 0);
+  a.bias_stride = static_cast<size_t>(pair_bias_of_layer(d, pair_planes, n_ctx, 1) - a.bias);
   a.ctx_of_row = ctx_of_row;
   a.R = R;
   a.t = t;
diff --git a/diffab-pytorch_amd/diffab_pytorch/_hip.py b/diffab-pytorch_amd/diffab_pytorch/_hip.py
--- a/diffab-pytorch_amd/diffab_pytorch/_hip.py
+++ b/diffab-pytorch_amd/diffab_pytorch/_hip.py
@@ -96,6 +96,7 @@
     "diffab_debug_set_module_stamps": (C.c_int, [_fp]),
     "diffab_set_stream_guard": (C.c_int, [C.c_int]),
     "diffab_debug_linear128": (C.c_int, [_fp, _fp, _fp, _fp, C.c_int64, C.c_int32, C.c_int32, _fp, C.c_size_t, _fp]),
+    "diffab_debug_pair_bias": (C.c_int, [_PD, C.POINTER(IpaLayerWeights), _i32, _fp, _i32, _fp, _fp]),
     "diffab_debug_gemm_tn": (C.c_int, [_fp, _fp, _fp, _fp, C.c_int64, C.c_int32, C.c_int32, C.c_int32, _fp]),
     "diffab_debug_xstat128": (C.c_int, [_fp, _fp, _fp, C.c_int64, C.c_int32, C.c_int32, _fp, C.c_size_t, _fp]),
     "diffab_kernel_timer_read": (C.c_int, [C.POINTER(C.c_int64), C.POINTER(C.c_double)]),
diff --git a/include/diffab_hip.h b/include/diffab_hip.h
--- a/include/diffab_hip.h
+++ b/include/diffab_hip.h
@@ -99,6 +99,8 @@
 int diffab_set_stream_guard(int on);
 int diffab_debug_linear128(const float* X, const float* W, const float* bias, float* Y, int64_t M, int32_t Kd, int32_t mode, void* scratch,
                            size_t scratch_bytes, void* stream);
+int diffab_debug_pair_bias(const diffab_dims* d, const diffab_ipa_layer_weights* layers, int32_t n_layers, const float* e, int32_t n_pair,
+                           float* out, void* stream);
 int diffab_debug_xstat128(const float* X, const float* W, float* Y, int64_t M, int32_t N, int32_t mode, void* scratch, size_t scratch_bytes,
                           void* stream);
 int diffab_debug_gemm_tn(const float* A, const float* B, float* C, float* db, int64_t M, int32_t N1, int32_t N2, int32_t mode, void* stream);
```

Result: slower. 12.76 million, median of 6 (-2.4%).
